# User-tian/Conan

Hardware: AMD Instinct MI355X
Metric: chunks/sec (80 ms chunk, 16 kHz), all streams summed; p50 per-chunk latency beside it (higher is better)
Workload: dtype f32 (3×bf16-limb products, f32 accumulate)

## Files before the change

### conan_amd/csrc/kernels.h

```cpp
#pragma once
#include <hip/hip_runtime.h>
#include <stdint.h>
#include <stdlib.h>

namespace cnk {

inline const char* dev_getenv(const char* name) {
#ifdef CONAN_DEV_SWITCHES
  return getenv(name);
#else
  (void)name;
  return nullptr;
#endif
}
#define HIP_CHECK(x) ::ch::hip_check((x), #x)


struct TRef {
  float* base;
  long long slot_stride;
  int C;
  int lmask;
  int rate;
  int off;
  int mode;
  int pad_;
};

constexpr int kSlotTablePad = 32;

constexpr int kMegaMaxOps = 80;
constexpr int kMegaDbgGroupWords = 512 + 4 * kMegaMaxOps;
constexpr int kMegaDbgWords = kMegaDbgGroupWords + 64;

enum Act { ACT_NONE = 0, ACT_LRELU = 1, ACT_RELU = 2, ACT_GELU = 3, ACT_TANH = 4 };

constexpr unsigned long long kSpinBudgetTicks = 5000000ull;
constexpr unsigned long long kSpinGapTicks = 100000ull;
enum WaitCode { WAIT_MEGA_BARRIER = 1, WAIT_EMF_CLUSTER = 2, WAIT_PAIR_FLAG = 3, WAIT_PAIR_MAILBOX = 4, WAIT_RETIRED_5 = 5 , WAIT_MEGA_ELECT = 6, WAIT_MEGA_DECIDED = 7, WAIT_MEGA_FLAGS = 8 };
struct SpinGuard { unsigned long long last = 0, acc = 0; unsigned it = 0; };
#if defined(__HIPCC__)
__device__ __forceinline__ bool spin_expired(SpinGuard& g, unsigned* guard, unsigned code) {
  if ((++g.it & 255u) != 0u || guard == nullptr) return false;
  if (__hip_atomic_load(guard, __ATOMIC_RELAXED, __HIP_MEMORY_SCOPE_AGENT) != 0u) return true;
  const unsigned long long now = __builtin_amdgcn_s_memrealtime();
  if (g.last != 0) { const unsigned long long d = now - g.last; g.acc += d < kSpinGapTicks ? d : kSpinGapTicks; }
  g.last = now;
  if (g.acc < kSpinBudgetTicks) return false;
  __hip_atomic_store(guard, code, __ATOMIC_RELAXED, __HIP_MEMORY_SCOPE_AGENT);
  unsigned* host = *reinterpret_cast<unsigned* const*>(guard + 2);
  if (host) __hip_atomic_store(host, code, __ATOMIC_RELAXED, __HIP_MEMORY_SCOPE_SYSTEM);
  return true;
}
#endif

struct ConvArgs {
  TRef x;
  TRef y;
  TRef res;
  TRef m1, m2;
  const float* w;
  const float* bias;
  const float* bvec;
  const int* slots;
  const int* pos;
  const int* lens;
  long long bvec_stride;
  int has_res, has_m1, has_m2;
  int Cin, Cin_pad, Cout, Cout_pad;
  int ktaps, dil, pad_left;
  int T;
  int n;
  int in_act;
  float in_slope;
  int out_act;
  float out_scale, out_slope;
  int shuffle_r;
  int Cin_alloc;
  float* y2_base;
  float y2_slope;
  const unsigned short* wl;
#ifdef CK_STAMPS
  unsigned long long* dbg;
#endif
};

struct ConvGroup {
  ConvArgs p[3];
  int tile_start[4];
  int tiles_n[3];
  int order[3];
  float* slab;
  int* counters;
  const int* assign;
  int assign_per;
  int ksplit;
  int split_from;
  int fenced;
};

enum ConvCfg { CFG_128x64 = 0, CFG_64x64 = 1, CFG_128x32 = 2, CFG_32x64_K2 = 3, CFG_32x32_K4 = 4, CFG_64x32_K2 = 5,
               CFG_64x64_KS64 = 6, CFG_128x32_KS64 = 7, NUM_CFG };
int conv_cfg_ks(int cfg);
bool conv_cfg_splitk(int cfg);
const char* conv_cfg_name(int cfg);
int conv_cfg_tm(int cfg);
int conv_cfg_tn(int cfg);
void launch_conv(const ConvGroup& g, int nprob, int cfg, hipStream_t st, int num_cu = 256);

struct ConvTallArgs {
  ConvArgs p;
  int S, nbps;
  int mtiles, ntiles;
  float* slab;
  int* counters;
};
bool conv_tall_supported(const ConvArgs& a);
bool conv_tall_plan(const ConvArgs& a, int num_cu, int plan_n, ConvTallArgs* out, long long slab_floats, int max_counters, int max_T = 32);
void launch_conv_tall(const ConvTallArgs& g, hipStream_t st);

struct ConvLimbGroup {
  ConvArgs p[3];
  int nprob;
  const int* tiles;
  const int* assign;
  int assign_per;
  int wr_max;
  float* slab; int* counters;
  long long slab_floats; int max_counters;
};
bool conv_limb_supported(const ConvArgs& a);
int conv_limb_shape(const ConvArgs* p, int nprob, int num_cu, int plan_n = 0, bool tail_split = false);
bool launch_conv_limb(const ConvLimbGroup& g, int shape, int num_cu, hipStream_t st);
int conv_limb_tail_slices(const ConvArgs& a, int shape, int num_cu);
const char* conv_limb_name(int shape);

struct RBProb {
  const float* w1; const float* w2;
  const float* b1; const float* b2;
  const unsigned short* w1l; const unsigned short* w2l;
  TRef x;
  TRef y;
  int k, dil;
};
struct RBArgs {
  RBProb p[3];
  const int* slots; const int* pos;
  const int* tiles;
  int ntiles;
  int* sched;
  int nprob, n, T;
  int tiles_per_slot;
  int order[3];
  float slope;
  int merge;
  TRef ymean;
  unsigned long long* dbg;
};
bool resblock_fused_supported(int C, int kmax, int span_max);
int resblock_fused_rows(int C, int T, int n, int ksum, int kmax, int num_cu);
bool launch_resblock_fused(const RBArgs& a, int C, int rows, int num_cu, hipStream_t st);
bool resblock_fused_can_merge(int C, int rows);
const char* resblock_fused_name(int C, int rows, bool merge = false);
const int* resblock_tiles(const RBArgs& a, int ro, int* total_out);
bool resblock_limb_supported(int C, int kmax, int span_max);
constexpr int kResblockLimbMaxSlots = 256;
int resblock_limb_rows(int C, int span_max);
bool launch_resblock_limb(const RBArgs& a, int C, int rows, int num_cu, hipStream_t st);
bool resblock_limb_can_merge(int C, int rows);
const char* resblock_limb_name(int C, int rows, bool merge = false);


struct RPProb {
  const float* w1; const float* w2;
  const float* b1; const float* b2;
  TRef x, y;
  TRef xh;
  int k, dil;
};
struct RPArgs {
  RPProb p[3];
  const int* slots; const int* pos;
  const int* tiles; int ntiles;
  int* sched;
  float* xb;
  unsigned* xflag; unsigned* mbox; unsigned* xcount;
  int nprob, n, T;
  float slope;
  unsigned* guard;
  int fault;
};
bool resblock_pair_supported(int C, int kmax, int span_max, int T);
size_t resblock_pair_xb_floats(int num_cu);
bool launch_resblock_pair(const RPArgs& a, int num_cu, hipStream_t st);
const char* resblock_pair_name(int T);

struct RowConvArgs {
  TRef x;
  TRef hist;
  TRef y, res, m1, m2, lnmask, mask_out;
  const float* w;
  const float* bias;
  const float* bvec; long long bvec_stride;
  const float* gamma; const float* beta; float eps;
  const int* slots; const int* pos;
  int ln, has_res, has_m1, has_m2, has_lnmask, has_mask_out;
  int Cin, Cout, Cout_pad, ktaps, dil, T, n;
  int out_act; float out_scale, out_slope;
  int in_lrelu; float in_slope;
  int wr_max;
  int cw;
  const float* w2;
  float* part; long long part_stride;
  int Cout2, Cout2_pad;
  const float* xp; long long xp_stride; int xparts, xp_ld;
  const float* xbias; TRef xres; int has_xres;
  TRef xm1, xm2; int has_xm1, has_xm2, xstore;
  int hid_overlay;
};
bool rowconv_supported(int Cin, int ktaps, int dil, int T);
void launch_rowconv(const RowConvArgs& a, hipStream_t st, int plan_rows = 0);
const char* rowconv_kernel_name(const RowConvArgs& a, int plan_rows = 0);
int rowconv_plan(RowConvArgs& a, int* nbx, int* nby, int* lds_floats, int plan_rows = 0);

struct LNArgs {
  TRef x, pre, y, post, m1, m2, mask_out;
  const float* gamma;
  const float* beta;
  const int* slots;
  const int* pos;
  const int* lens;
  int has_pre, has_post, has_m1, has_m2, has_mask_out;
  int T, n, C;
  float eps;
  const float* xp; long long xp_stride; int xparts, xp_ld;
  const float* xbias; TRef xres; int has_xres;
};
void launch_layernorm(const LNArgs& a, hipStream_t st);

struct CopyArgs {
  TRef x, y;
  const int* slots; const int* pos; const int* lens;
  int T, n, C;
};
void launch_copy_rows(const CopyArgs& a, hipStream_t st);

struct EmbedArgs {
  TRef y;
  const float* table; const int* idx;
  const int* slots; const int* pos;
  int T, n, C, vocab;
};
void launch_embed(const EmbedArgs& a, hipStream_t st);

struct EmfAttnArgs {
  const float* q;
  const float* kv;
  float* out;
  float* kring; float* vring;
  long long ring_slot_stride;
  const int* slots; const int* past;
  int n, R, U, D, H, LC, lmask;
  float scaling;
  int M, seg;
};
void launch_emf_attn(const EmfAttnArgs& a, hipStream_t st);

struct EmfMemArgs {
  float* ln;
  float* bank;
  const float* mems_in;
  const int* slots; const int* past;
  int n, R, U, D, M, MB, seg;
};
void launch_emf_mem_prep(const EmfMemArgs& a, hipStream_t st);
void launch_emf_seg_mean(const float* x, float* out, int n, int rows, int row0, int U, int D, hipStream_t st);
void launch_emf_mem_out(const float* x, float* out, int n, int rows, int row, int D, int tanh_on_mem, hipStream_t st);

constexpr int EMF_MAX_LAYERS = 12;
struct EmfLayerW {
  const float *wqkv, *wo, *w1, *w2;
  const float* params;
};
struct EmfFusedArgs {
  EmfLayerW layers[EMF_MAX_LAYERS];
  float* kring[EMF_MAX_LAYERS]; float* vring[EMF_MAX_LAYERS];
  long long ring_slot_stride;
  const float* chunk;
  float* out;
  float* logits;
  int* codes;
  const float* wp; const float* bp;
  const int* slots; int* past;
  int n, L, R, U, D, H, LC, lmask, F, K;
#ifdef EF_STAMPS
  unsigned long long* dbg;
#endif
  unsigned magic_per_g;
  float scaling;
  int cs;
  float* xch;
  unsigned* xflag;
  unsigned* xepoch;
  int fenced;
  unsigned* guard;
  unsigned fault;
  int M, MB, tanh_on_mem;
  float* bank_k[EMF_MAX_LAYERS]; float* bank_v[EMF_MAX_LAYERS];
  long long bank_slot_stride;
};
constexpr int EMF_MAX_CLUSTER = 8;
constexpr int EMF_MAX_CHUNKS = 16;
inline size_t emformer_cluster_xch_floats(int max_groups, int D) { return (size_t)max_groups * 2 * EMF_MAX_CHUNKS * 16 * D; }
inline size_t emformer_cluster_flag_words(int max_groups) { return (size_t)max_groups * (EMF_MAX_LAYERS * EMF_MAX_CLUSTER + 1); }
int emformer_fused_streams_per_block(const EmfFusedArgs& a);
bool emformer_fused_supported(const EmfFusedArgs& a);
void launch_emformer_fused(const EmfFusedArgs& a, hipStream_t st);

struct XAttnArgs {
  TRef q;
  TRef out;
  const float* kv;
  long long kv_slot_stride;
  const float* kmask;
  const int* slen;
  float* attn_avg;
  const int* slots; const int* pos;
  int T, n, E, H, S_max;
};
void launch_xattn(const XAttnArgs& a, hipStream_t st);

struct PitchHeadArgs {
  TRef h;
  TRef pitch_inp;
  TRef dec_inp;
  const float* gamma; const float* beta; const float* w; const float* b;
  const float* pitch_embed;
  const int* codes;
  float* uv_pred; float* f0; int* bins;
  const int* slots; const int* pos;
  int T, n, Cp, E, silent_token;
};
void launch_pitch_head(const PitchHeadArgs& a, hipStream_t st);

struct MeanActArgs { TRef x[3]; TRef y; const int* slots; const int* pos; int nsrc, T, n, C; float slope; };
void launch_mean_act(const MeanActArgs& a, hipStream_t st);
struct ConvPostArgs { TRef x[3]; TRef xmean; int nsrc; float slope; const float* w; float bias; float* wav; float* pre; const int* slots; const int* pos; int T, n, C, k;
                      int* adv_pos; int adv_delta; int* adv_ticket; };
void launch_conv_post(const ConvPostArgs& a, hipStream_t st);

enum MegaOpType { MOP_RC111 = 0, MOP_RC114 = 1, MOP_ROWLIN = 2, MOP_LN = 3, MOP_XATTN = 4, MOP_PITCH = 5, MOP_EMBED = 6, MOP_COPY32 = 7, MOP_ADVANCE = 8, MOP_FFN = 9 };
struct MegaCopy { unsigned* dst; const unsigned* src; long long n; };
struct MegaAdvance { int* pos; const int* slots; int n, delta; };
struct MegaOp {
  int type, nbx, nby;
  int barrier;
  float f0, f1;
  int pad_[2];
  union U { RowConvArgs rc; LNArgs ln; XAttnArgs xa; PitchHeadArgs ph; EmbedArgs em; MegaCopy cp; MegaAdvance adv; } u;
};
int decoder_mega_lds_floats(const MegaOp& op, int rc_lds_floats);
int decoder_mega_blocks_per_cu(int lds_bytes, bool wide_regs);
struct MegaLaunch {
  const MegaOp* prog; int nops, njobs, groups, group_size, kw4, lds_bytes;
  const int* slots; const int* pos; int n, T;
  unsigned* gbar; unsigned* bar; unsigned bar_base; unsigned long long* dbg;
  unsigned* guard;
  int wide_regs;
  int xcd; unsigned* xs; unsigned xseq, xdec_base;
};
void launch_decoder_mega(const MegaLaunch& m, hipStream_t st);

struct ArgmaxArgs { const float* x; int* idx; int rows, C; };
void launch_argmax(const ArgmaxArgs& a, hipStream_t st);

void launch_advance(int* pos, const int* slots, int n, int delta, hipStream_t st);
void launch_fill_int(int* p, const int* slots, int n, int value, hipStream_t st);
void launch_copy_int_rows(int* dst, const int* src, int n, int T, int S, hipStream_t st);
void launch_profile_mark(hipStream_t st);
void launch_scatter_int(int* dst, const int* slots, const int* src, int n, hipStream_t st);
void launch_scatter_ids(int* dst, const int* slots, const int* src, const int* lens, int n, int S_max, hipStream_t st);
void launch_gather_ids(int* dst, int* cnt, const int* src, const int* slen, const int* slots, int n, int S_max, hipStream_t st);
void launch_scatter_rows(float* dst, const float* src, const int* slots, int n, int C, hipStream_t st);
void launch_zero_slots(float* base, long long slot_stride, long long count, const int* slots, int n, hipStream_t st);
constexpr int kMelStreamFrames = 4;
struct MelStreamArgs {
  const float* wav;
  float* aring;
  float* mring;
  float* chunk;
  const int* slots;
  const float* win; const double2* tw; const float* fb; const int* lo; const int* hi;
  long long r_prev, total;
  int m, n, f0, nnew, pos, rows, real;
  int LA, LM, nm, n_fft, hop, nb, cmag;
  float eps, vmin, vmax, mag_eps;
  int natural_log;
};
inline size_t mel_stream_lds_bytes(int n_fft, int cmag) { return (size_t)n_fft * kMelStreamFrames * 8 + (size_t)n_fft * 16 + (size_t)kMelStreamFrames * cmag * 4; }
void launch_mel_stream(const MelStreamArgs& a, hipStream_t st);
void launch_mel_stream_copy(const MelStreamArgs& a, hipStream_t st);
enum RaggedField {
  kRgSlot, kRgRecvLo, kRgRecvHi, kRgTotalLo, kRgTotalHi,
  kRgM, kRgF0, kRgNnew, kRgPos, kRgRows, kRgReal,
  kRgChunk,
  kRgJob,
  kRgGroup, kRgIndex, kRgEmit,
  kRaggedWords = 16
};
struct MelRaggedArgs {
  const float* wav;
  float* aring; float* mring; float* chunk;
  const int* tab;
  const float* win; const double2* tw; const float* fb; const int* lo; const int* hi;
  int n, jobs, wstride;
  int LA, LM, nm, n_fft, hop, nb, cmag;
  float eps, vmin, vmax, mag_eps;
  int natural_log;
};
void launch_mel_ragged(const MelRaggedArgs& a, hipStream_t st);
struct WavScatterArgs {
  const int* tab; int n, seg, nm, hop;
  const int* codes_src; const float* mel_src; const float* wav_src;
  int* codes; float* mel; float* wav;
};
void launch_wav_scatter(const WavScatterArgs& a, hipStream_t st);

constexpr int kRsTile = 256;
constexpr int kRsRing = 32768;
constexpr int kRsMaxWindow = 16384;
struct RsFilter {
  const float* taps;
  const int* ph;
  int orig, nph, w, L;
};
struct RsRow {
  long long in0, out0;
  const float* taps; const int* ph;
  int slot, m, h, orig, nph, w, L, copy;
};
static_assert(sizeof(RsRow) == 16 * sizeof(int), "RsRow is uploaded as 16 ints");
struct ResampleArgs { const float* x; float* y; long long samples, nout; RsFilter f; int win; };
void launch_resample(const ResampleArgs& a, int n, hipStream_t st);
struct ResampleStreamArgs {
  const float* wav; long long wav_ld;
  float* ring;
  float* out; long long out_ld;
  const RsRow* rows; int n, tiles, win;
};
void launch_resample_stream(const ResampleStreamArgs& a, hipStream_t st);
struct RsOutRow {
  long long in0, out0;
  const float* taps; const int* ph;
  int slot, m, h, orig, nph, w, L, dst;
};
static_assert(sizeof(RsOutRow) == 16 * sizeof(int), "RsOutRow is uploaded as 16 ints");
struct ResampleOutArgs {
  const float* wav; long long wav_ld;
  float* ring; int ring_len;
  float* out; long long out_ld;
  const RsOutRow* rows; int n, tiles, win;
};
void launch_resample_out(const ResampleOutArgs& a, hipStream_t st);

struct RowMaskArgs { TRef x; TRef m; const int* lens; int T, n, C; int mode; };
void launch_rowmask(const RowMaskArgs& a, hipStream_t st);
struct WNGateArgs { TRef xin; TRef acts; const int* lens; int T, n, H; };
void launch_wn_gate(const WNGateArgs& a, hipStream_t st);
struct WNUpdateArgs { TRef rs; TRef x; TRef out; TRef m; const int* lens; int T, n, H; int last; int first; };
void launch_wn_update(const WNUpdateArgs& a, hipStream_t st);
struct PoolArgs { TRef x; TRef m; TRef y; const int* lens; int T, n, C, group; };
void launch_group_pool(const PoolArgs& a, hipStream_t st);
struct VQArgs {
  TRef x; TRef dots; TRef cat;
  const float* emb; const float* e2; const float* postable;
  int* ids;
  const int* lens; int S, n, E, M, S_max;
};
void launch_vq(const VQArgs& a, hipStream_t st);
struct KMaskArgs { TRef tok; float* kmask; long long kmask_stride; const int* slots; const int* lens; int S, n, S_max; };
void launch_kmask(const KMaskArgs& a, hipStream_t st);
struct MeanArgs { TRef x; TRef m; float* out; long long out_stride; const int* slots; const int* lens; int T, n, C; };
void launch_masked_mean(const MeanArgs& a, hipStream_t st);
struct ScaleMaskArgs { TRef x; TRef m; const int* lens; int T, n, C; };
void launch_mul_mask(const ScaleMaskArgs& a, hipStream_t st);

}
```

### conan_amd/csrc/resblock_limb.hip

```cpp
#include <algorithm>
#include <cstring>
#include <type_traits>

#include "kernels.h"

#define RL_MAX_SLOTS 256

#ifndef RL_HELPER_PRIO
#define RL_HELPER_PRIO 3
#endif
#ifndef RL_MATRIX_PRIO
#define RL_MATRIX_PRIO 0
#endif
#ifndef RL_STAMPS
#define RL_STAMPS 0
#endif

#ifdef RL_ABLATE_W
#define RL_WOFF(x) 0
#define RL_WOFF2(a_, b_) (b_)
#else
#define RL_WOFF(x) (x)
#define RL_WOFF2(a_, b_) (a_)
#endif

namespace cnk {

namespace {

typedef float f32x4 __attribute__((ext_vector_type(4)));
typedef __bf16 bf16x8 __attribute__((ext_vector_type(8)));
typedef unsigned short u16;
typedef const f32x4 __attribute__((address_space(1)))* gcf4;
typedef f32x4 __attribute__((address_space(1)))* gf4;
typedef const float __attribute__((address_space(1)))* gcf1;
typedef const int __attribute__((address_space(1)))* gci;

__device__ __forceinline__ f32x4 rl_gload(const void* p) { return *(gcf4)(p); }
__device__ __forceinline__ float4 rl_gload4(const float* p) { const f32x4 v = *(gcf4)(p); return make_float4(v[0], v[1], v[2], v[3]); }
__device__ __forceinline__ void rl_gstore4(float* p, const float4 v) { *(gf4)(p) = (f32x4){v.x, v.y, v.z, v.w}; }

typedef float f32x2 __attribute__((ext_vector_type(2)));
typedef __bf16 bf16x2 __attribute__((ext_vector_type(2)));
__device__ __forceinline__ void rl_split2(const f32x2 x, unsigned& h, unsigned& m, unsigned& l) {
  h = __builtin_bit_cast(unsigned, __builtin_convertvector(x, bf16x2));
  const f32x2 hf = {__uint_as_float(h << 16), __uint_as_float(h & 0xffff0000u)};
  const f32x2 r1 = x - hf;
  m = __builtin_bit_cast(unsigned, __builtin_convertvector(r1, bf16x2));
  const f32x2 mf = {__uint_as_float(m << 16), __uint_as_float(m & 0xffff0000u)};
  const f32x2 r2 = r1 - mf;
  l = __builtin_bit_cast(unsigned, __builtin_convertvector(r2, bf16x2));
}
__device__ __forceinline__ f32x2 rl_lrelu2(const f32x2 x, const float slope) {
  const f32x2 sx = x * slope;
  return (f32x2){__builtin_fmaxf(x[0], sx[0]), __builtin_fmaxf(x[1], sx[1])};
}

template <int C_, int NR2_, int SPAN_>
struct RLGeom {
  static constexpr int C = C_, NR2 = NR2_;
  static constexpr int NR1 = NR2 + 1;
  static constexpr int RO = 16 * NR2;
  static constexpr int XT_ROWS = 16 * NR1;
  static constexpr int MAXSPAN = SPAN_;
  static constexpr int WR_MAX = XT_ROWS + MAXSPAN;
  static constexpr int LDB = C + 16;
  static constexpr int PLW = WR_MAX * LDB;
  static constexpr int PLX = XT_ROWS * LDB;
  static constexpr int LDA = C + 4;
  static constexpr int LDS_U16 = 3 * (PLW + PLX);
  static constexpr int NCT = C / 16;
  static constexpr int NCW = C == 64 ? 1 : 2;
  static constexpr int RSPLIT = 4 / (NCT / NCW);
  static constexpr int NRW1 = (NR1 + RSPLIT - 1) / RSPLIT;
  static constexpr int NRW2 = (NR2 + RSPLIT - 1) / RSPLIT;
  static constexpr int KB = C / 32;
  static constexpr int RING = 2;
  static constexpr int C4 = C / 4;
  static constexpr int BLK = 3 * 512;
  static_assert(C % 32 == 0 && NCT % NCW == 0 && 4 % (NCT / NCW) == 0 && (KB == 1 || KB % RING == 0), "channel count");
  static_assert(RO * LDA * 4 <= 3 * PLX * 2, "accumulator image inside the xt planes");
  static_assert(LDS_U16 * 2 + 32 + 8 * RL_MAX_SLOTS <= 160 * 1024, "LDS budget");
};

template <int NCW, int RING>
__device__ __forceinline__ void rl_prefetch_w(f32x4 (&bw)[RING][NCW][3], const u16* __restrict__ wl, const long long ct_stride) {
#pragma unroll
  for (int q = 0; q < RING; ++q) {
#pragma unroll
    for (int c = 0; c < NCW; ++c)
#pragma unroll
      for (int p = 0; p < 3; ++p) bw[q][c][p] = rl_gload(wl + c * ct_stride + q * 1536 + p * 512);
    __builtin_amdgcn_sched_barrier(0);
  }
}

template <int NRW, int NCW, int LDB, int KB, int RING>
__device__ __forceinline__ void rl_gemm(const u16* __restrict__ src, const int plane, const int row0, const int tap_stride, const int k,
                                        const u16* __restrict__ wl, const long long ct_stride, const u16* __restrict__ wl_next,
                                        const long long ct_stride_next, f32x4 (&acc)[NRW][NCW], f32x4 (&bw)[RING][NCW][3], const int lane) {
  const u16* abase = src + (row0 + (lane & 15)) * LDB + 8 * (lane >> 4);
  f32x4 af[NRW][3];
#pragma unroll
  for (int r = 0; r < NRW; ++r)
#pragma unroll
    for (int p = 0; p < 3; ++p) af[r][p] = *reinterpret_cast<const f32x4*>(abase + p * plane + r * 16 * LDB);
  const int tstep = tap_stride * LDB;
  if constexpr (KB == 1) {
    static_assert(RING == 2, "ring");
    constexpr int PA[6] = {2, 1, 0, 1, 0, 0}, PB[6] = {0, 1, 2, 0, 1, 0};
    auto block = [&](const int j, auto slot_c) __attribute__((always_inline)) {
      constexpr int SL = decltype(slot_c)::value;
      const u16* anext = abase + (j + 1) * tstep;
#pragma unroll
      for (int s = 0; s < 6; ++s)
#pragma unroll
        for (int r = 0; r < NRW; ++r) {
#pragma unroll
          for (int c = 0; c < NCW; ++c)
            acc[r][c] = __builtin_amdgcn_mfma_f32_16x16x32_bf16(__builtin_bit_cast(bf16x8, bw[SL][c][PB[s]]), __builtin_bit_cast(bf16x8, af[r][PA[s]]), acc[r][c], 0, 0, 0);
#ifndef RL_ABLATE_A
          if (s == 0) af[r][2] = *reinterpret_cast<const f32x4*>(anext + 2 * plane + r * 16 * LDB);
          if (s == 3) af[r][1] = *reinterpret_cast<const f32x4*>(anext + plane + r * 16 * LDB);
          if (s == 5) af[r][0] = *reinterpret_cast<const f32x4*>(anext + r * 16 * LDB);
#endif
        }
      const bool own = j + 2 < k;
      const u16* wsrc = own ? wl + (long long)(j + 2) * 1536 : wl_next + (long long)(j + 2 - k) * 1536;
      const long long cs = own ? ct_stride : ct_stride_next;
#pragma unroll
      for (int c = 0; c < NCW; ++c)
#pragma unroll
        for (int p = 0; p < 3; ++p) bw[SL][c][p] = rl_gload(wsrc + c * cs + p * 512);
#pragma unroll
      for (int s = 0; s < 6; ++s) {
        if (s == 0 || s == 3 || s == 5) {
#pragma unroll
          for (int r = 0; r < NRW; ++r) {
            __builtin_amdgcn_sched_group_barrier(0x008, NCW, 0);
            __builtin_amdgcn_sched_group_barrier(0x100, 1, 0);
          }
        } else {
          __builtin_amdgcn_sched_group_barrier(0x008, NRW * NCW, 0);
        }
      }
      __builtin_amdgcn_sched_group_barrier(0x020, 3 * NCW, 0);
    };
    int j = 0;
    for (; j + 1 < k; j += 2) {
      block(j, std::integral_constant<int, 0>{});
      block(j + 1, std::integral_constant<int, 1>{});
    }
    if (j < k) {
      block(j, std::integral_constant<int, 0>{});
#pragma unroll
      for (int c = 0; c < NCW; ++c)
#pragma unroll
        for (int p = 0; p < 3; ++p) { const f32x4 t = bw[0][c][p]; bw[0][c][p] = bw[1][c][p]; bw[1][c][p] = t; }
    }
    return;
  }
  for (int j = 0; j < k; ++j) {
    const u16* arow = abase + j * tstep;
    const bool last = j + 1 == k;
    const u16* wnext = last ? wl_next : wl + (long long)(j + 1) * KB * 1536;
    const long long cnext = last ? ct_stride_next : ct_stride;
#pragma unroll
    for (int q = 0; q < KB; ++q) {
      const u16* anext = (q + 1 < KB) ? arow + (q + 1) * 32 : arow + tstep;
      constexpr int PA[6] = {2, 1, 0, 1, 0, 0}, PB[6] = {0, 1, 2, 0, 1, 0};
#pragma unroll
      for (int s = 0; s < 6; ++s)
#pragma unroll
        for (int r = 0; r < NRW; ++r) {
#pragma unroll
          for (int c = 0; c < NCW; ++c)
            acc[r][c] = __builtin_amdgcn_mfma_f32_16x16x32_bf16(__builtin_bit_cast(bf16x8, bw[q % RING][c][PB[s]]), __builtin_bit_cast(bf16x8, af[r][PA[s]]),
                                                                acc[r][c], 0, 0, 0);
#ifndef RL_ABLATE_A
          if (s == 0) af[r][2] = *reinterpret_cast<const f32x4*>(anext + 2 * plane + r * 16 * LDB);
          if (s == 3) af[r][1] = *reinterpret_cast<const f32x4*>(anext + plane + r * 16 * LDB);
          if (s == 5) af[r][0] = *reinterpret_cast<const f32x4*>(anext + r * 16 * LDB);
#endif
        }
      if (q + RING < KB) {
#pragma unroll
        for (int c = 0; c < NCW; ++c)
#pragma unroll
          for (int p = 0; p < 3; ++p) bw[q % RING][c][p] = rl_gload(wl + RL_WOFF(((long long)j * KB + q + RING) * 1536) + c * ct_stride + p * 512);
      } else {
#pragma unroll
        for (int c = 0; c < NCW; ++c)
#pragma unroll
          for (int p = 0; p < 3; ++p) bw[q % RING][c][p] = rl_gload(RL_WOFF2(wnext, wl) + (q + RING - KB) * 1536 + c * cnext + p * 512);
      }
#pragma unroll
      for (int s = 0; s < 6; ++s) {
        if (s == 0 || s == 3 || s == 5) {
#pragma unroll
          for (int r = 0; r < NRW; ++r) {
            __builtin_amdgcn_sched_group_barrier(0x008, NCW, 0);
            __builtin_amdgcn_sched_group_barrier(0x100, 1, 0);
          }
        } else {
          __builtin_amdgcn_sched_group_barrier(0x008, NRW * NCW, 0);
        }
      }
      __builtin_amdgcn_sched_group_barrier(0x020, 3 * NCW, 0);
      __builtin_amdgcn_sched_barrier(0);
    }
  }
}

}

#define RL_SEL(br_, f) ((br_) == 0 ? a.p[0].f : ((br_) == 1 ? a.p[1].f : a.p[2].f))

template <int C, int NR2, int SPAN, bool MERGE>
__global__ __launch_bounds__(512, 2) void resblock_limb_kernel(const RBArgs a) {
  using G = RLGeom<C, NR2, SPAN>;
  constexpr int LDB = G::LDB;
  __shared__ __attribute__((aligned(16))) u16 lds[G::LDS_U16 + 16 + 4 * RL_MAX_SLOTS];
  u16* const win = lds;
  u16* const xt = lds + 3 * G::PLW;
  float* const accimg = reinterpret_cast<float*>(xt);
  int* const meta = reinterpret_cast<int*>(lds + G::LDS_U16);
  int* const sptab = meta + 8;
  const int tid = threadIdx.x;
  const int lane = tid & 63;
  const int wave = __builtin_amdgcn_readfirstlane(tid >> 6);
  const int ntiles = a.ntiles;
  const float slope = a.slope;
  const int T = a.T;
  constexpr bool merge = MERGE;
  const int np = a.nprob;

  if (wave >= 4) {
    const int ht = tid - 256;
    __builtin_amdgcn_s_setprio(RL_HELPER_PRIO);
    auto hbar = [&]() __attribute__((always_inline)) { asm volatile("s_waitcnt lgkmcnt(0)\n\ts_barrier" ::: "memory"); };
    constexpr int NIT = (G::WR_MAX * G::C4 + 255) / 256;
    float4 wv[NIT];
    int wtotal = 0, wzr = 0;
    auto win_issue = [&](const int p, const int i, const int t0, const int slot, const int pos) __attribute__((always_inline)) {
      const int k = RL_SEL(p, k), d = RL_SEL(p, dil);
      const int wr = G::XT_ROWS + (k - 1) * d;
      const int tw0 = t0 - (k - 1) - (k - 1) * d;
      const int xmode = a.p[0].x.mode, xrate = a.p[0].x.rate;
      const float* xb = RL_SEL(p, x.base) + (long long)(xmode == 0 ? slot : i) * RL_SEL(p, x.slot_stride);
      const unsigned rbase = (xmode == 0 ? (unsigned)pos * (unsigned)xrate : 0u) + (unsigned)(RL_SEL(p, x.off) + tw0);
      const unsigned rmask = xmode == 0 ? (unsigned)RL_SEL(p, x.lmask) : 0xffffffffu;
      wtotal = wr * G::C4;
#pragma unroll
      for (int u = 0; u < NIT; ++u) {
        const int idx = ht + 256 * u;
        const int w = idx / G::C4, c4 = idx - w * G::C4;
        const unsigned row = (rbase + (unsigned)w) & rmask;
        wv[u] = idx < wtotal ? rl_gload4(xb + (long long)row * C + c4 * 4) : make_float4(0.f, 0.f, 0.f, 0.f);
      }
      const long long abs0 = (xmode == 0 ? (long long)pos * xrate : 0ll) + t0 - (k - 1);
      wzr = abs0 >= 0 ? 0 : (abs0 < -(long long)G::XT_ROWS ? G::XT_ROWS : (int)-abs0);
    };
    auto win_write = [&]() __attribute__((always_inline)) {
#pragma unroll
      for (int u = 0; u < NIT; ++u) {
        const int idx = ht + 256 * u;
        const int w = idx / G::C4, c4 = idx - w * G::C4;
        unsigned h[2], m[2], l[2];
        rl_split2(rl_lrelu2((f32x2){wv[u].x, wv[u].y}, slope), h[0], m[0], l[0]);
        rl_split2(rl_lrelu2((f32x2){wv[u].z, wv[u].w}, slope), h[1], m[1], l[1]);
        if (idx < wtotal) {
          u16* dst = win + w * LDB + c4 * 4;
          *reinterpret_cast<uint2*>(dst) = make_uint2(h[0], h[1]);
          *reinterpret_cast<uint2*>(dst + G::PLW) = make_uint2(m[0], m[1]);
          *reinterpret_cast<uint2*>(dst + 2 * G::PLW) = make_uint2(l[0], l[1]);
        }
      }
      if (ht == 0) meta[0] = wzr;
    };
    constexpr int NOUT = (G::RO * G::C4) / 256;
    static_assert((G::RO * G::C4) % 256 == 0 && 256 % G::C4 == 0, "output tile / helper threads");
    const int oc4 = ht % G::C4;
    float4 oacc[NOUT], ores[NOUT], osum[MERGE ? NOUT : 1], ob2 = make_float4(0.f, 0.f, 0.f, 0.f);
    const float* oxb = nullptr; const float* ob2p = nullptr;
    float* oyb = nullptr;
    unsigned oyr0 = 0, oym = 0, oxr0 = 0, oxm = 0;
    int ot0 = 0, op = 0, oyC = C;
#pragma unroll
    for (int u = 0; u < (MERGE ? NOUT : 1); ++u) osum[u] = make_float4(0.f, 0.f, 0.f, 0.f);
    auto out_fetch = [&](const int p, const int i, const int t0, const int slot, const int pos) __attribute__((always_inline)) {
      const int xmode = a.p[0].x.mode, xrate = a.p[0].x.rate, ymode = a.p[0].y.mode, yrate = a.p[0].y.rate;
      oxb = RL_SEL(p, x.base) + (long long)(xmode == 0 ? slot : i) * RL_SEL(p, x.slot_stride);
      oxr0 = (xmode == 0 ? (unsigned)pos * (unsigned)xrate : 0u) + (unsigned)(RL_SEL(p, x.off) + t0);
      oxm = xmode == 0 ? (unsigned)RL_SEL(p, x.lmask) : 0xffffffffu;
      if (!merge) {
        oyb = RL_SEL(p, y.base) + (long long)(ymode == 0 ? slot : i) * RL_SEL(p, y.slot_stride);
        oyr0 = (ymode == 0 ? (unsigned)pos * (unsigned)yrate : 0u) + (unsigned)(RL_SEL(p, y.off) + t0);
        oym = ymode == 0 ? (unsigned)RL_SEL(p, y.lmask) : 0xffffffffu;
      } else {
        const int mmode = a.ymean.mode;
        oyb = a.ymean.base + (long long)(mmode == 0 ? slot : i) * a.ymean.slot_stride;
        oyr0 = (mmode == 0 ? (unsigned)pos * (unsigned)a.ymean.rate : 0u) + (unsigned)(a.ymean.off + t0);
        oym = mmode == 0 ? (unsigned)a.ymean.lmask : 0xffffffffu;
        oyC = a.ymean.C;
      }
      ot0 = t0; op = p;
      ob2p = RL_SEL(p, b2) + oc4 * 4;
#pragma unroll
      for (int u = 0; u < NOUT; ++u) oacc[u] = *reinterpret_cast<const float4*>(accimg + ((ht + 256 * u) / G::C4) * G::LDA + oc4 * 4);
      ob2 = rl_gload4(ob2p);
#pragma unroll
      for (int u = 0; u < NOUT; ++u) {
        const int r = (ht + 256 * u) / G::C4;
        ores[u] = ot0 + r < T ? rl_gload4(oxb + (long long)((oxr0 + (unsigned)r) & oxm) * C + oc4 * 4) : make_float4(0.f, 0.f, 0.f, 0.f);
      }
    };
    auto out_store = [&]() __attribute__((always_inline)) {
#pragma unroll
      for (int u = 0; u < NOUT; ++u) {
        const int r = (ht + 256 * u) / G::C4;
        if (ot0 + r < T) {
          const float4 v = make_float4((oacc[u].x + ob2.x) + ores[u].x, (oacc[u].y + ob2.y) + ores[u].y, (oacc[u].z + ob2.z) + ores[u].z, (oacc[u].w + ob2.w) + ores[u].w);
          if constexpr (!MERGE) rl_gstore4(oyb + (long long)((oyr0 + (unsigned)r) & oym) * C + oc4 * 4, v);
          else {
            float4 sm = osum[MERGE ? u : 0];
            if (op == 0) sm = v; else { sm.x += v.x; sm.y += v.y; sm.z += v.z; sm.w += v.w; }
            osum[MERGE ? u : 0] = sm;
            if (op == np - 1) {
              const float dn = (float)np;
              if (np > 1) { sm.x /= dn; sm.y /= dn; sm.z /= dn; sm.w /= dn; }
              sm.x = sm.x > 0.f ? sm.x : sm.x * slope; sm.y = sm.y > 0.f ? sm.y : sm.y * slope;
              sm.z = sm.z > 0.f ? sm.z : sm.z * slope; sm.w = sm.w > 0.f ? sm.w : sm.w * slope;
              rl_gstore4(oyb + (long long)((oyr0 + (unsigned)r) & oym) * oyC + oc4 * 4, sm);
            }
          }
        }
      }
    };
#if RL_STAMPS
    const unsigned long long h_t0 = __builtin_amdgcn_s_memtime();
    unsigned long long h_t[6] = {0, 0, 0, 0, 0, 0};
#define RL_HT(i_) h_t[i_] = __builtin_amdgcn_s_memtime() - h_t0
#else
#define RL_HT(i_)
#endif
    int dv0 = 0;
    if (wave == 4 && lane == 0) dv0 = __hip_atomic_fetch_add(a.sched, 1, __ATOMIC_RELAXED, __HIP_MEMORY_SCOPE_AGENT);
    for (int e = ht; e < a.n; e += 256) {
      const int sl = a.slots ? *(gci)(a.slots + e) : e;
      sptab[2 * e] = sl; sptab[2 * e + 1] = a.pos ? *(gci)(a.pos + sl) : 0;
    }
    const int tps = a.tiles_per_slot, per_prob = a.n * tps;
    auto decode = [&](const int e, int& p, int& i, int& t0) __attribute__((always_inline)) {
      if constexpr (!MERGE) {
        const int b = e / per_prob, rem = e - b * per_prob;
        p = b == 0 ? a.order[0] : (b == 1 ? a.order[1] : a.order[2]);
        i = rem / tps; t0 = (rem - i * tps) * G::RO;
      } else {
        const int g = e / np;
        p = e - g * np; i = g / tps; t0 = (g - i * tps) * G::RO;
      }
    };
    int cur = -1, p = -1, i = 0, t0 = 0;
    if (wave == 4) {
      cur = __builtin_amdgcn_readfirstlane(dv0) * (merge ? np : 1);
      if (cur >= ntiles) cur = -1;
      if (cur >= 0) decode(cur, p, i, t0);
      if (lane == 0) { meta[1] = cur; meta[2] = p; meta[3] = 0; }
    }
    RL_HT(0);
    asm volatile("s_waitcnt lgkmcnt(0)\n\ts_barrier" ::: "memory");
    RL_HT(1);
    if (wave != 4) {
      cur = __builtin_amdgcn_readfirstlane(meta[1]);
      if (cur >= 0) decode(cur, p, i, t0);
    }
    if (cur >= 0) {
    int slot = __builtin_amdgcn_readfirstlane(sptab[2 * i]), pos = __builtin_amdgcn_readfirstlane(sptab[2 * i + 1]);
    win_issue(p, i, t0, slot, pos);
    RL_HT(2);
    int gen = 1;
    int dv = 0, dnext = -1;
    auto draw_issue = [&](const int have, const int idx_prev, const int p_prev) __attribute__((always_inline)) {
      if (wave == 4 && lane == 0 && have) {
        if (merge && p_prev != np - 1) dnext = idx_prev + 1;
        else { dnext = -1; dv = __hip_atomic_fetch_add(a.sched, 1, __ATOMIC_RELAXED, __HIP_MEMORY_SCOPE_AGENT); }
      }
    };
    auto draw_take = [&](const int have) __attribute__((always_inline)) {
      int idx = -1;
      if (!have) return idx;
      if (wave == 4) {
        const int drawn = dv * (merge ? np : 1);
        idx = __builtin_amdgcn_readfirstlane(dnext >= 0 ? dnext : drawn);
        if (idx >= ntiles) idx = -1;
        if (lane == 0) {
          meta[1] = idx;
          asm volatile("s_waitcnt lgkmcnt(0)" ::: "memory");
          __hip_atomic_store(&meta[3], gen, __ATOMIC_RELEASE, __HIP_MEMORY_SCOPE_WORKGROUP);
        }
      } else {
        while (__hip_atomic_load(&meta[3], __ATOMIC_ACQUIRE, __HIP_MEMORY_SCOPE_WORKGROUP) != gen) __builtin_amdgcn_s_sleep(4);
        idx = __builtin_amdgcn_readfirstlane(meta[1]);
      }
      ++gen;
      return idx;
    };
    const bool deep = ntiles >= 5 * (int)gridDim.x * (merge ? np : 1);
    auto stage = [&](const int e) __attribute__((always_inline)) {
      int pe, ie, te;
      decode(e, pe, ie, te);
      win_issue(pe, ie, te, __builtin_amdgcn_readfirstlane(sptab[2 * ie]), __builtin_amdgcn_readfirstlane(sptab[2 * ie + 1]));
      return pe;
    };
    int nxt = -1, pn = -1;
    if (deep) {
      draw_issue(1, cur, p);
      nxt = draw_take(1);
    }
    RL_HT(3);
    win_write();
    RL_HT(4);
    hbar();
    RL_HT(5);
#if RL_STAMPS
    if (a.dbg && blockIdx.x == 0 && wave == 4 && lane == 0) { unsigned long long* q = a.dbg + 256 * 4 + 12; for (int e = 0; e < 6; ++e) q[e] = h_t[e]; }
#endif
    bool pending = false;
    for (;;) {
      const bool have = deep ? nxt >= 0 : true;
      if (deep && nxt >= 0) pn = stage(nxt);
      draw_issue(have, deep ? nxt : cur, deep ? pn : p);
      if (pending) out_store();
      int nn = -1;
      if (!deep) {
        nxt = draw_take(have); pn = -1;
        if (nxt >= 0) pn = stage(nxt);
      }
      if (ht == 0) meta[2] = nxt >= 0 ? pn : -1;
      hbar();
      hbar();
      if (nxt >= 0) win_write();
      hbar();
      hbar();
      out_fetch(p, i, t0, slot, pos);
      pending = true;
      if (deep) nn = draw_take(have);
      if (nxt < 0) break;
      cur = nxt;
      decode(cur, p, i, t0);
      slot = __builtin_amdgcn_readfirstlane(sptab[2 * i]); pos = __builtin_amdgcn_readfirstlane(sptab[2 * i + 1]);
      nxt = nn;
    }
    if (pending) out_store();
    }
    if (ht == 0) {
      const int d = __hip_atomic_fetch_add(a.sched + 1, 1, __ATOMIC_RELAXED, __HIP_MEMORY_SCOPE_AGENT);
      if (d == (int)gridDim.x - 1) {
        __hip_atomic_store(a.sched, 0, __ATOMIC_RELAXED, __HIP_MEMORY_SCOPE_AGENT);
        __hip_atomic_store(a.sched + 1, 0, __ATOMIC_RELAXED, __HIP_MEMORY_SCOPE_AGENT);
      }
    }
    return;
  }

  if (RL_MATRIX_PRIO) __builtin_amdgcn_s_setprio(RL_MATRIX_PRIO);
  auto bar = [&]() __attribute__((always_inline)) { asm volatile("s_waitcnt lgkmcnt(0)\n\ts_barrier" ::: "memory"); };
  const int wc = wave % (4 / G::RSPLIT);
  const int wr = wave / (4 / G::RSPLIT);
  const int ct0 = wc * G::NCW;
  const int lr = lane & 15, lg = lane >> 4;
#if RL_STAMPS
  unsigned long long st_gemm = 0, st_t0 = __builtin_amdgcn_s_memtime(), st_r0 = __builtin_amdgcn_s_memrealtime(), st_bar = 0, st_b3 = 0, st_b1 = 0, st_b4 = 0, st_b2 = 0, st_e1 = 0, st_e2 = 0, st_tiles = 0, st_head = 0, st_pre = 0, st_mid = 0;
#define RL_T() __builtin_amdgcn_s_memtime()
#define RL_BAR(acc_) do { const unsigned long long q0_ = RL_T(); bar(); const unsigned long long q1_ = RL_T(); acc_ += q1_ - q0_; st_bar += q1_ - q0_; } while (0)
#define RL_GEMM(...) do { const unsigned long long s0_ = RL_T(); __VA_ARGS__; asm volatile("s_nop 0" ::"v"(acc[0][0][0])); st_gemm += RL_T() - s0_; } while (0)
#else
#define RL_BAR(acc_) bar()
#define RL_GEMM(...) __VA_ARGS__
#endif
  f32x4 bw[G::RING][G::NCW][3];
  bar();
  int p = __builtin_amdgcn_readfirstlane(meta[2]);
  if (p < 0) return;
  {
    const long long cs = (long long)(RL_SEL(p, k) + 1) * G::KB * G::BLK;
    rl_prefetch_w<G::NCW, G::RING>(bw, RL_SEL(p, w1l) + (long long)ct0 * cs + lane * 8, cs);
  }
  bar();
#if RL_STAMPS
  st_head = RL_T() - st_t0;
#endif
  while (p >= 0) {
#if RL_STAMPS
    const unsigned long long top_ = RL_T();
#endif
    const int k = RL_SEL(p, k), d = RL_SEL(p, dil);
    const u16* const w1 = RL_SEL(p, w1l);
    const u16* const w2 = RL_SEL(p, w2l);
    const float* const b1 = RL_SEL(p, b1);
    const long long ct_stride = (long long)(k + 1) * G::KB * G::BLK;
    const int zrows = __builtin_amdgcn_readfirstlane(meta[0]);
    f32x4 b1v[G::NCW];
#pragma unroll
    for (int c = 0; c < G::NCW; ++c) b1v[c] = rl_gload(b1 + (ct0 + c) * 16 + 4 * lg);
    int pn;
    {
      f32x4 acc[G::NRW1][G::NCW];
#pragma unroll
      for (int r = 0; r < G::NRW1; ++r)
#pragma unroll
        for (int c = 0; c < G::NCW; ++c) acc[r][c] = (f32x4){0.f, 0.f, 0.f, 0.f};
      const int rt0 = wr * G::NRW1;
#if RL_STAMPS
      st_pre += RL_T() - top_;
#endif
      RL_GEMM(rl_gemm<G::NRW1, G::NCW, LDB, G::KB, G::RING>(win, G::PLW, rt0 * 16, d, k, w1 + (long long)ct0 * ct_stride + lane * 8, ct_stride,
                                                           w2 + (long long)ct0 * ct_stride + lane * 8, ct_stride, acc, bw, lane));
      RL_BAR(st_b3);
#if RL_STAMPS
      const unsigned long long e1_0 = RL_T();
#endif
      auto epilogue1 = [&](auto zr_c) __attribute__((always_inline)) {
        constexpr bool ZR = decltype(zr_c)::value;
#pragma unroll
        for (int c = 0; c < G::NCW; ++c) {
          const int col = (ct0 + c) * 16 + 4 * lg;
#pragma unroll
          for (int r = 0; r < G::NRW1; ++r) {
            if (rt0 + r < G::NR1) {
              const int m = (rt0 + r) * 16 + lr;
              unsigned h[2], mm[2], l[2];
              const f32x4 v = acc[r][c] + b1v[c];
              rl_split2(rl_lrelu2((f32x2){v[0], v[1]}, slope), h[0], mm[0], l[0]);
              rl_split2(rl_lrelu2((f32x2){v[2], v[3]}, slope), h[1], mm[1], l[1]);
              const bool zr = ZR && m < zrows;
              u16* dst = xt + m * LDB + col;
              *reinterpret_cast<uint2*>(dst) = zr ? make_uint2(0u, 0u) : make_uint2(h[0], h[1]);
              *reinterpret_cast<uint2*>(dst + G::PLX) = zr ? make_uint2(0u, 0u) : make_uint2(mm[0], mm[1]);
              *reinterpret_cast<uint2*>(dst + 2 * G::PLX) = zr ? make_uint2(0u, 0u) : make_uint2(l[0], l[1]);
            }
          }
        }
      };
      if (zrows > 0) epilogue1(std::true_type{}); else epilogue1(std::false_type{});
#if RL_STAMPS
      asm volatile("s_waitcnt lgkmcnt(0)" ::: "memory"); st_e1 += RL_T() - e1_0; ++st_tiles;
#endif
    }
    RL_BAR(st_b1);
#if RL_STAMPS
    const unsigned long long mid_ = RL_T();
#endif
    pn = __builtin_amdgcn_readfirstlane(meta[2]);
    const int pnx = pn >= 0 ? pn : p;
    const long long csn = (long long)(RL_SEL(pnx, k) + 1) * G::KB * G::BLK;
    const u16* const w1n = RL_SEL(pnx, w1l) + (long long)ct0 * csn + lane * 8;
    {
      f32x4 acc[G::NRW2][G::NCW];
#pragma unroll
      for (int r = 0; r < G::NRW2; ++r)
#pragma unroll
        for (int c = 0; c < G::NCW; ++c) acc[r][c] = (f32x4){0.f, 0.f, 0.f, 0.f};
      const int rt0 = wr * G::NRW2;
#if RL_STAMPS
      st_mid += RL_T() - mid_;
#endif
      RL_GEMM(rl_gemm<G::NRW2, G::NCW, LDB, G::KB, G::RING>(xt, G::PLX, rt0 * 16, 1, k, w2 + (long long)ct0 * ct_stride + lane * 8, ct_stride,
                                                           w1n, csn, acc, bw, lane));
      RL_BAR(st_b4);
#if RL_STAMPS
      const unsigned long long e2_0 = RL_T();
#endif
#pragma unroll
      for (int c = 0; c < G::NCW; ++c) {
        const int col = (ct0 + c) * 16 + 4 * lg;
#pragma unroll
        for (int r = 0; r < G::NRW2; ++r) {
          if (rt0 + r < NR2) *reinterpret_cast<f32x4*>(accimg + ((rt0 + r) * 16 + lr) * G::LDA + col) = acc[r][c];
        }
      }
#if RL_STAMPS
      asm volatile("s_waitcnt lgkmcnt(0)" ::: "memory"); st_e2 += RL_T() - e2_0;
#endif
    }
    RL_BAR(st_b2);
    p = pn;
  }
#if RL_STAMPS
  if (a.dbg && tid == 0) {
    unsigned long long* o = a.dbg + blockIdx.x * 4;
    if (blockIdx.x == 0) { unsigned long long* q = a.dbg + 256 * 4; q[0] = st_b3; q[1] = st_b1; q[2] = st_b4; q[3] = st_b2; q[4] = st_e1; q[5] = st_e2; q[6] = st_tiles; q[7] = st_gemm; q[8] = __builtin_amdgcn_s_memtime() - st_t0; q[9] = st_head; q[10] = st_pre; q[11] = st_mid; }
    o[0] = st_gemm; o[1] = __builtin_amdgcn_s_memtime() - st_t0; o[2] = __builtin_amdgcn_s_memrealtime() - st_r0; o[3] = st_bar;
  }
#endif
}


namespace {
struct RLCand { int C, NR2, span; };
const RLCand kLimbCands[] = {{32, 10, 50}, {64, 5, 50}, {128, 2, 50}};
}

bool resblock_limb_supported(int C, int kmax, int span_max) {
  for (const RLCand& c : kLimbCands)
    if (c.C == C && span_max <= c.span) return kmax <= 16;
  return false;
}

int resblock_limb_rows(int C, int span_max) {
  int best = 0;
  for (const RLCand& c : kLimbCands)
    if (c.C == C && span_max <= c.span) best = std::max(best, 16 * c.NR2);
  return best;
}

template <int C, int NR2, int SPAN, bool MERGE = false>
static bool launch_rl(const RBArgs& ain, int num_cu, hipStream_t st) {
  RBArgs a = ain;
  const int ro = 16 * NR2;
  a.tiles_per_slot = (a.T + ro - 1) / ro;
  const int total = a.nprob * a.n * a.tiles_per_slot;
  if (total <= 0) return true;
  if (!a.sched) return false;
  for (int p = 0; p < a.nprob; ++p) if (!a.p[p].w1l || !a.p[p].w2l) return false;
  if (a.n > RL_MAX_SLOTS) return false;
  if (!(a.slope > 0.f && a.slope <= 1.f)) return false;
  for (int p = 0; p < 3; ++p) a.order[p] = p;
  std::stable_sort(a.order, a.order + a.nprob, [&](int x, int y) { return a.p[x].k > a.p[y].k; });
  const int grid = std::min(a.merge ? total / a.nprob : total, num_cu);
  a.tiles = nullptr; a.ntiles = total;
  hipLaunchKernelGGL((resblock_limb_kernel<C, NR2, SPAN, MERGE>), dim3(grid), dim3(512), 0, st, a);
  return true;
}

bool launch_resblock_limb(const RBArgs& a, int C, int rows, int num_cu, hipStream_t st) {
  const int nr2 = rows / 16;
  if (a.merge) {
    if (C == 32 && nr2 == 10) return launch_rl<32, 10, 50, true>(a, num_cu, st);
    if (C == 64 && nr2 == 5) return launch_rl<64, 5, 50, true>(a, num_cu, st);
    if (C == 128 && nr2 == 2) return launch_rl<128, 2, 50, true>(a, num_cu, st);
    return false;
  }
  if (C == 32 && nr2 == 10) return launch_rl<32, 10, 50>(a, num_cu, st);
  if (C == 64 && nr2 == 5) return launch_rl<64, 5, 50>(a, num_cu, st);
  if (C == 128 && nr2 == 2) return launch_rl<128, 2, 50>(a, num_cu, st);
  return false;
}

bool resblock_limb_can_merge(int C, int rows) { return (C == 32 && rows == 160) || (C == 64 && rows == 80) || (C == 128 && rows == 32); }

const char* resblock_limb_name(int C, int rows, bool merge) {
  static thread_local char buf[72];
  const int span = 50;
  snprintf(buf, sizeof(buf), "cnk::resblock_limb_kernel<%d, %d, %d, %s>", C, rows / 16, span, merge ? "true" : "false");
  return buf;
}

}
```

### conan_amd/csrc/streams.h

```cpp
#pragma once
#include "host_common.h"

using ch::Error;
using ch::Lin;
using ch::PackedConv;
using ch::Ring;
using cnk::ConvArgs;
using cnk::ConvGroup;
using cnk::TRef;

constexpr int kMaxBranches = 3;
constexpr int PADR = 16;

struct VocStage {
  Ring up;
  Ring upa;
  Ring xs;
  std::vector<std::vector<Ring>> xt, xo;
  std::vector<std::vector<Ring>> xa;
  int C = 0, rate = 1;
  bool fused = false;
  bool pair = false;
  std::vector<std::vector<Ring>> xh;
};

struct PinRing {
  static constexpr int N = 8;
  int* buf = nullptr;
  size_t cap = 0;
  hipEvent_t ev[N] = {};
  int next = 0, cur = 0;
  void init(size_t ints) {
    cap = ints;
    HIP_CHECK(hipHostMalloc((void**)&buf, cap * N * sizeof(int), hipHostMallocDefault));
    for (int i = 0; i < N; ++i) HIP_CHECK(hipEventCreateWithFlags(&ev[i], hipEventDisableTiming));
  }
  void upload(int* dst, const int* src, size_t n, hipStream_t st) {
    if (n > cap) throw ch::Error(CONAN_ERR_INVALID, "host table larger than the staging buffer");
    cur = next; next = (next + 1) % N;
    HIP_CHECK(hipEventSynchronize(ev[cur]));
    memcpy(buf + (size_t)cur * cap, src, n * sizeof(int));
    HIP_CHECK(hipMemcpyAsync(dst, buf + (size_t)cur * cap, n * sizeof(int), hipMemcpyHostToDevice, st));
    HIP_CHECK(hipEventRecord(ev[cur], st));
  }
  ~PinRing() {
    for (int i = 0; i < N; ++i) if (ev[i]) (void)hipEventDestroy(ev[i]);
    if (buf) (void)hipHostFree(buf);
  }
};

struct conan_streams {
  conan_ctx* ctx = nullptr;
  std::atomic<int>* live = nullptr;
  std::map<std::string, std::string> dev_plan;
  void parse_dev_plan(const char* text);
  const char* dev(const char* name) const {
    if (!dev_plan.empty()) {
      auto it = dev_plan.find(name);
      if (it != dev_plan.end()) return it->second.c_str();
    }
#ifdef CONAN_DEV_SWITCHES
    return getenv((std::string("CONAN_") + name).c_str());
#else
    return nullptr;
#endif
  }
  bool fixed_plan = false;
  bool in_style_pass = false;
  int plan_n(int n) const { return (fixed_plan && !in_style_pass) ? max_slots : n; }
  bool pipe_idle = false;
  bool shared_device = false;
  int max_slots = 0, max_frames = 0, max_ref = 0, S_max = 0;
  std::vector<void*> allocs;
  int64_t state_bytes = 0;
  std::vector<std::pair<float*, long long>> voc_state, dec_state, emf_state;

  int* d_slots = nullptr;
  int* d_ident = nullptr;
  int* d_zero = nullptr;
  int* d_lens = nullptr;
  int* d_lens2 = nullptr;
  int* d_codes = nullptr;
  float* sk_slab[3] = {nullptr, nullptr, nullptr};
  int* sk_counters[3] = {nullptr, nullptr, nullptr};
  int reserve_cus = 0;
  bool fenced = false;
  bool rb_limb = false;
  bool arith_auto = true;
  bool rb_merge = true;
  int* cp_ticket[3] = {nullptr, nullptr, nullptr};
  int* rb_sched[2] = {nullptr, nullptr};
  float* rp_xb[2] = {nullptr, nullptr};
  unsigned* rp_words[2] = {nullptr, nullptr};
  long long sk_slab_floats = 0;
  int sk_max_tiles = 0;
  std::vector<int> h_slots;
  std::vector<int> slot_seen;
  int slot_gen = 0;
  PinRing pin;
  int* pos_emf = nullptr; int* pos_dec = nullptr; int* pos_voc = nullptr;
  unsigned* d_guard = nullptr;
  unsigned* h_guard = nullptr;
  int test_fault = 0;
  void check_fault() const {
    if (!h_guard) return;
    const unsigned code = *(volatile const unsigned*)h_guard;
    if (code == 0) return;
    static const char* what[] = {"?", "decoder_mega_kernel group / grid barrier", "emformer_fused_kernel cluster exchange", "resblock_pair_kernel partner flag", "resblock_pair_kernel tile mailbox",
                                 "(retired)", "decoder_mega_kernel xcd election", "decoder_mega_kernel xcd roll call", "decoder_mega_kernel xcd flag barrier"};
    throw ch::Error(CONAN_ERR_HIP, std::string("a cross-workgroup wait gave up after its 50 ms budget (") + what[code < 9 ? code : 0] +
                                       "): results since then are invalid and this stream-set is unusable - destroy it and create a new one");
  }

  float* fe_audio = nullptr; float* fe_mel = nullptr; float* fe_chunk = nullptr;
  int fe_LA = 0, fe_LM = 0, fe_last_n = 0;
  struct FeSlot { long long recv = 0; int frames = 0, chunks = 0, phase = 0; };
  std::vector<FeSlot> fe_slot;
  static constexpr int NS = 4;
  PinRing fe_pin;
  int* rg_tab[NS] = {}; int* rg_codes[NS] = {}; float* rg_mel[NS] = {}; float* rg_wav[NS] = {};
  hipEvent_t ev_stage[NS] = {};
  long long rg_calls = 0;
  bool fe_last_ragged = false;
  void ragged_init();
  struct RsSlot { const ch::RsTable* f = nullptr; long long in = 0, out = 0; int phase = 0; };
  std::vector<RsSlot> rs_slot;
  float* rs_ring = nullptr;
  PinRing rs_pin;
  cnk::RsRow* rs_rows[NS] = {}; float* rs_wav[NS] = {};
  hipEvent_t ev_rs[NS] = {};
  long long rs_calls = 0;
  void resample_init();
  struct OrSlot { const ch::RsTable* f = nullptr; long long out = 0; int flushed = 0; };
  std::vector<OrSlot> or_slot;
  std::vector<long long> voc_samples;
  float* or_ring = nullptr; int or_ring_len = 0;
  PinRing or_pin;
  cnk::RsOutRow* or_rows[NS] = {}; float* or_wav[NS] = {};
  hipEvent_t ev_or[NS] = {};
  long long or_calls = 0, out_ld = 0;
  std::vector<int32_t> out_counts;
  void out_stage_init();
  struct OutPlan {
    bool active = false;
    std::vector<cnk::RsOutRow> rows;
    std::vector<int32_t> counts;
    std::vector<int> dst;
    float* base = nullptr; long long ld = 0;
    int tiles = 1, win = 0;
    double flops = 0;
  };
  OutPlan out_plan(const int32_t* slots, int n, int frames, float* wav_out, long long natural_ld, const std::vector<int>* dst, const std::string& who) const;
  Ring v_mel, v_pre;
  std::vector<VocStage> v_st;
  std::vector<Ring> e_k, e_v;
  std::vector<float*> e_bank;
  int e_bank_rows = 0;
  float* e_mems[2] = {nullptr, nullptr};
  Lin e_x[2], e_ln, e_q, e_kv, e_att, e_r1, e_ffn, e_h, e_r2, e_logits;
  bool emf_fused = false;
  int emf_cluster = 0;
  cnk::EmfFusedArgs emf_fused_args;
  Ring c_emb, c_pin2, c_lastr;
  std::vector<Ring> c_uvh;
  std::vector<Ring> c_lnrs;
  Lin c_pin, c_q, c_att, c_a1, c_a2, c_ff, c_uv5, c_x[2], c_h, c_post, c_mask_blk, c_mask_blk2, c_mask_out, c_mel, c_part, c_part2;
  float* c_style = nullptr;
  float* c_kv = nullptr;
  float* c_kmask = nullptr;
  int* c_slen = nullptr;
  int* c_vqids = nullptr;
  std::vector<char> has_ref;
  std::vector<char> voc_fresh;
  int sp_batch = 0;
  Lin s_mel, s_np, s_wnm, s_x[2], s_ln, s_h, s_blkm, s_wx, s_wout, s_win, s_acts, s_rs, s_ph, s_pm, s_px[2], s_pln, s_phh,
      s_pblk, s_enc, s_dots, s_cat, s_tok, s_kvtmp;
  int* s_ids = nullptr;

  float* alloc(size_t floats) {
    void* p = nullptr;
    if (floats == 0) floats = 4;
    HIP_CHECK(hipMalloc(&p, floats * sizeof(float)));
    HIP_CHECK(hipMemset(p, 0, floats * sizeof(float)));
    allocs.push_back(p);
    state_bytes += (int64_t)floats * 4;
    return (float*)p;
  }
  Ring mk_ring(int C, int rate, int hist, std::vector<std::pair<float*, long long>>* reg) {
    Ring r; r.C = C; r.rate = rate;
    r.L = ch::next_pow2(hist + max_frames * rate);
    r.slot_stride = (long long)r.L * C;
    r.base = alloc((size_t)max_slots * r.slot_stride);
    if (reg) reg->push_back({r.base, r.slot_stride});
    return r;
  }
  Lin mk_lin(int rows, int C, int nb = -1) {
    Lin l; l.rows = rows; l.C = C;
    l.base = alloc((size_t)(nb < 0 ? max_slots : nb) * rows * C);
    return l;
  }
  hipStream_t st_emf = nullptr, st_front = nullptr, st_voc = nullptr;
  hipEvent_t ev_wide[4] = {};
  hipEvent_t mark_wide = nullptr;
  bool wide_marked[4] = {false, false, false, false};
  static constexpr int NP = 4;
  hipEvent_t ev_in[NP] = {}, ev_emf[NP] = {}, ev_front[NP] = {}, ev_voc[NP] = {};
  hipEvent_t ev_fence[NP] = {};
  hipStream_t fence_stream = nullptr; bool fence_set = false;
  hipEvent_t fence_event = nullptr;
  int* codes_hand[NP] = {};
  int ws_index(hipStream_t st) const { return (st_voc && st == st_voc) ? 1 : ((st_emf && st == st_emf) ? 2 : 0); }
  float* mel_hand[NP] = {};
  long long async_steps = 0;
  std::vector<hipEvent_t> clock_ev;
  bool clock_on = false; int clock_n = 0;
  std::vector<hipEvent_t> tl_ev;
  bool tl_on = false; int tl_n = 0;
  void async_init();
  void join(hipStream_t st);

  void mega_print_stamps();
  ~conan_streams() {
    if (live) live->fetch_sub(1);
    if (mega_dbg) mega_print_stamps();
    if (st_emf) (void)hipStreamDestroy(st_emf);
    if (st_front) (void)hipStreamDestroy(st_front);
    if (st_voc) (void)hipStreamDestroy(st_voc);
    for (int i = 0; i < NP; ++i) { if (ev_in[i]) (void)hipEventDestroy(ev_in[i]); if (ev_fence[i]) (void)hipEventDestroy(ev_fence[i]); }
    for (int i = 0; i < NP; ++i) { if (ev_wide[i]) (void)hipEventDestroy(ev_wide[i]); if (ev_emf[i]) (void)hipEventDestroy(ev_emf[i]); if (ev_front[i]) (void)hipEventDestroy(ev_front[i]); if (ev_voc[i]) (void)hipEventDestroy(ev_voc[i]); }
    for (int i = 0; i < NS; ++i) if (ev_stage[i]) (void)hipEventDestroy(ev_stage[i]);
    for (int i = 0; i < NS; ++i) if (ev_rs[i]) (void)hipEventDestroy(ev_rs[i]);
    for (int i = 0; i < NS; ++i) if (ev_or[i]) (void)hipEventDestroy(ev_or[i]);
    for (void* p : allocs) (void)hipFree(p);
    if (h_guard) (void)hipHostFree(h_guard);
    for (auto& e : prof_ev) { (void)hipEventDestroy(e.first); (void)hipEventDestroy(e.second); }
    for (auto& e : clock_ev) (void)hipEventDestroy(e);
    for (auto& m : mega_cache) { if (m.copied) (void)hipEventDestroy(m.copied); if (m.pinned) (void)hipHostFree(m.pinned); if (m.dev) (void)hipFree(m.dev); }
    for (auto& e : tl_ev) (void)hipEventDestroy(e);
  }

  void build_vocoder();
  void build_emformer();
  void build_decoder();
  void set_slots(const int32_t* slots, int n, hipStream_t st);
  int pick_cfg(int M, int N, int nprob) const;
  bool prof_on = false;
  std::vector<std::pair<hipEvent_t, hipEvent_t>> prof_ev;
  size_t prof_used = 0;
  double prof_flops = 0.0;
  long long prof_launches = 0;
  struct ProfRec { std::string name; double flops; };
  std::vector<ProfRec> prof_rec;
  struct ProfKernel { std::string name; double ms, flops; long long n; };
  std::vector<ProfKernel> prof_kernels;
  void launch_group(const ConvGroup& g, int nprob, int cfg, hipStream_t st);
  bool launch_rb(const cnk::RBArgs& a, int C, hipStream_t st, const TRef* ymean = nullptr);
  void launch_rp(const cnk::RPArgs& a, hipStream_t st);
  bool use_rowconv = true;
  bool rowconv_ok(const PackedConv& pc, int dil, int T) const { return use_rowconv && pc.wf && cnk::rowconv_supported(pc.Cin, pc.k, dil, T); }
  cnk::RowConvArgs mk_rc(const PackedConv& pc, const TRef& x, const TRef& y, int n, int T, int dil = 1) const;
  void rowconv(const cnk::RowConvArgs& a, hipStream_t st);
  template <typename F> void profiled(const std::string& name, double flops, hipStream_t st, F&& launch);
  void conv(const ConvArgs& a, hipStream_t st) { ConvGroup g; g.p[0] = a; launch_group(g, 1, pick_cfg(plan_n(a.n) * a.T, a.Cout, 1), st); }
  ConvArgs mk(const PackedConv& pc, const TRef& x, const TRef& y, int n, int T, const int* pos, int dil = 1, int pad_left = -1) const;

  struct DecExtra { float* mel_out2 = nullptr; int* codes_dst = nullptr; const int* codes_src = nullptr; int codes_words = 0; };
  struct MegaProgram {
    long long key[6] = {0, 0, 0, 0, 0, 0};
    bool ok = false;
    int nops = 0, groups = 0, group_size = 0, njobs = 0, kw4 = 0, lds_bytes = 0, barriers = 0, n = 0, T = 0;
    int lds_need = 0;
    bool xcd = false;
    double flops = 0.0;
    cnk::MegaOp* dev = nullptr;
    cnk::MegaOp* pinned = nullptr;
    hipEvent_t copied = nullptr;
    long long stamp = 0;
  };
  static constexpr int kMegaMaxOps = cnk::kMegaMaxOps, kMegaEntries = 12;
  std::vector<MegaProgram> mega_cache;
  long long mega_clock = 0;
  bool use_mega = true;
  int mega_grid = 128;
  int mega_gs = 8;
  bool mega_narrow_ksplit = true;
  int mega_ffn_gs = 8;
  unsigned* mega_bar = nullptr;
  unsigned mega_bar_count = 0;
  unsigned* mega_x = nullptr;
  unsigned mega_gseq = 0;
  unsigned mega_xseq = 0, mega_xdec = 0;
  int opt_flags = 0;
  bool mega_single = true;
  unsigned long long* mega_dbg = nullptr;
  int mega_dbg_prog = -1;
  std::vector<cnk::MegaOp>* mega_rec = nullptr;
  bool mega_rec_ok = true; int mega_rec_lds = 0; double mega_rec_flops = 0.0;
  void mega_push(cnk::MegaOp& op, int lds_floats);
  bool run_mega(int n, int T, const int32_t* codes, float* mel_out, const DecExtra& ex, hipStream_t st);
  void launch_mega(MegaProgram& e, hipStream_t st);
  void decoder_ops(int n, int frames, const int32_t* codes, float* mel_out, const conan_decoder_taps& taps, hipStream_t st);
  void op_embed(const cnk::EmbedArgs& a, hipStream_t st);
  void op_ln(const cnk::LNArgs& a, hipStream_t st);
  void op_xattn(const cnk::XAttnArgs& a, hipStream_t st);
  void op_pitch(const cnk::PitchHeadArgs& a, hipStream_t st);
  void op_advance(int* pos, int n, int delta, hipStream_t st);

  void hifigan_step(int n, int frames, const float* mel_dev, float* wav_out, float* pre_tanh, hipStream_t st, const conan_hifigan_taps* taps = nullptr,
                    const OutPlan* op = nullptr);
  void emformer_step(int n, const float* chunk, float* out, float* logits, int32_t* codes, hipStream_t st);
  void decoder_step(int n, int frames, const int32_t* codes, float* mel_out, const conan_decoder_taps& taps, hipStream_t st, const DecExtra* extra = nullptr);
  void set_reference(const int32_t* slots, int n, const float* ref, const int32_t* ref_len, int max_len, hipStream_t st);
  void conv_blocks_noncausal(const std::string& name, int nblocks, int k, int C, Lin* x, Lin& ln, Lin& h, Lin& blkm, const TRef& npm,
                             const int* lens, int n, int T, int& cur, hipStream_t st);
};

template <typename F>
inline void conan_streams::profiled(const std::string& name, double flops, hipStream_t st, F&& launch) {
  if (!prof_on) { launch(); return; }
  if (prof_used == prof_ev.size()) {
    hipEvent_t a, b;
    HIP_CHECK(hipEventCreate(&a)); HIP_CHECK(hipEventCreate(&b));
    prof_ev.push_back({a, b});
  }
  auto& ev = prof_ev[prof_used++];
  HIP_CHECK(hipEventRecord(ev.first, st));
  launch();
  HIP_CHECK(hipEventRecord(ev.second, st));
  prof_flops += flops;
  prof_launches += 1;
  prof_rec.push_back({name, flops});
}
```

### conan_amd/csrc/streams.hip

```cpp
#include <climits>

#include "streams.h"


ConvArgs conan_streams::mk(const PackedConv& pc, const TRef& x, const TRef& y, int n, int T, const int* pos, int dil,
                           int pad_left) const {
  ConvArgs a;
  memset(&a, 0, sizeof(a));
  a.x = x;
  a.y = y; a.res = ch::null_ref(); a.m1 = ch::null_ref(); a.m2 = ch::null_ref();
  a.w = pc.w; a.bias = pc.bias; a.bvec = nullptr; a.slots = d_slots; a.pos = pos; a.lens = nullptr;
  a.Cin = pc.Cin; a.Cin_pad = pc.Cin_pad; a.Cin_alloc = pc.Cin_alloc; a.Cout = pc.Cout; a.Cout_pad = pc.Cout_pad;
  a.ktaps = pc.k; a.dil = dil; a.pad_left = pad_left < 0 ? (pc.k - 1) * dil : pad_left;
  a.T = T; a.n = n; a.in_act = cnk::ACT_NONE; a.in_slope = 0.f; a.out_act = cnk::ACT_NONE; a.out_scale = 1.f; a.out_slope = 0.f;
  a.shuffle_r = pc.shuffle_r;
  a.wl = reinterpret_cast<const unsigned short*>(pc.wl);
  if (x.C != pc.Cin && !(x.C > pc.Cin)) throw Error(CONAN_ERR_SHAPE, "conv input width mismatch");
  return a;
}

int conan_streams::pick_cfg(int M, int N, int nprob) const {
  const int wide[] = {cnk::CFG_64x64, cnk::CFG_32x64_K2, cnk::CFG_32x32_K4};
  const int narrow[] = {cnk::CFG_128x32, cnk::CFG_64x32_K2, cnk::CFG_32x32_K4};
  const int* order = N <= 32 ? narrow : wide;
  const int cnt = 3;
  long long need = ctx->num_cu;
  int best = order[cnt - 1];
  for (int k = 0; k < cnt; ++k) {
    int c = order[k];
    long long blocks = (long long)((M + cnk::conv_cfg_tm(c) - 1) / cnk::conv_cfg_tm(c)) * ((N + cnk::conv_cfg_tn(c) - 1) / cnk::conv_cfg_tn(c)) * nprob;
    if (blocks >= need) {
      best = c;
      if (c == cnk::CFG_64x64 && blocks < 2 * need && nprob > 1) best = cnk::CFG_64x64_KS64;
      break;
    }
  }
  return best;
}

void conan_streams::launch_group(const ConvGroup& gin, int nprob, int cfg, hipStream_t st) {
  if (mega_rec) { mega_rec_ok = false; return; }
  for (int p = 0; p < nprob; ++p) {
    const ConvArgs& a = gin.p[p];
    if ((long long)(a.x.mode == 0 ? max_slots : a.n) * a.x.slot_stride * 4 >= (1ll << 32))
      throw Error(CONAN_ERR_UNSUPPORTED, "activation tensor of 4 GiB or more: lower max_slots");
    if (a.y2_base && ((a.Cout & 3) || (a.y.C & 3) || ((a.Cout / a.shuffle_r) & 3))) throw Error(CONAN_ERR_UNSUPPORTED, "activated twin output needs channel counts that are multiples of 4");
  }
  if (rb_limb && nprob == 1 && dev("NO_TALL") == nullptr) {
    const int cus = std::max(8, ctx->num_cu - (ws_index(st) == 1 ? reserve_cus : 0));
    const int wsi = ws_index(st);
    cnk::ConvTallArgs ta;
    if (cnk::conv_tall_plan(gin.p[0], cus, fixed_plan ? plan_n(gin.p[0].n) : 0, &ta, sk_slab_floats, sk_max_tiles, dev("TALL_MAXT") ? atoi(dev("TALL_MAXT")) : 32)) {
      ta.slab = sk_slab[wsi]; ta.counters = sk_counters[wsi];
      const ConvArgs& a = gin.p[0];
      profiled("cnk::conv_tall_kernel", 2.0 * (double)a.n * a.T * a.Cout * a.ktaps * a.Cin, st, [&] { cnk::launch_conv_tall(ta, st); });
      return;
    }
  }
  if (rb_limb && nprob >= 1 && nprob <= 3) {
    bool ok = true;
    for (int p = 0; p < nprob; ++p) ok = ok && cnk::conv_limb_supported(gin.p[p]) && gin.p[p].n == gin.p[0].n && gin.p[p].T == gin.p[0].T && gin.p[p].Cout == gin.p[0].Cout;
    const int cus = std::max(8, ctx->num_cu - (ws_index(st) == 1 ? reserve_cus : 0));
    const int shape = ok ? cnk::conv_limb_shape(gin.p, nprob, cus, fixed_plan ? plan_n(gin.p[0].n) : 0, !fixed_plan) : -1;
    if (shape >= 0) {
      cnk::ConvLimbGroup lg; memset(&lg, 0, sizeof(lg));
      for (int p = 0; p < nprob; ++p) lg.p[p] = gin.p[p];
      lg.nprob = nprob;
      if (!fixed_plan && nprob == 1) {
        const int wsi = ws_index(st);
        lg.slab = sk_slab[wsi]; lg.counters = sk_counters[wsi]; lg.slab_floats = sk_slab_floats; lg.max_counters = sk_max_tiles;
      }
      double fl = 0.0;
      for (int p = 0; p < nprob; ++p) fl += 2.0 * (double)lg.p[p].n * lg.p[p].T * lg.p[p].Cout * lg.p[p].ktaps * lg.p[p].Cin;
      const bool tail = lg.slab && shape == 0 && cnk::conv_limb_tail_slices(lg.p[0], shape, cus) >= 2;
      profiled(tail ? "cnk::conv_limb_sk_kernel<4, 1, 1, 4>" : cnk::conv_limb_name(shape), fl, st, [&] {
        if (!cnk::launch_conv_limb(lg, shape, cus, st)) throw Error(CONAN_ERR_HIP, "conv_limb launch failed");
      });
      return;
    }
  }
  ConvGroup g = gin;
  for (int p = 0; p < nprob; ++p) {
    ConvArgs& a = g.p[p];
    bool ring = a.y.mode == 0 || (a.has_res && a.res.mode == 0) || (a.has_m1 && a.m1.mode == 0) || (a.has_m2 && a.m2.mode == 0) || a.bvec != nullptr;
    ring = ring || a.x.mode == 0;
    if (!ring) { a.slots = nullptr; a.pos = nullptr; }
  }
  const int wsi = ws_index(st);
  g.slab = sk_slab[wsi]; g.counters = sk_counters[wsi]; g.ksplit = 1; g.split_from = 0; g.fenced = fenced ? 1 : 0;
  const int cus_all = std::max(8, ctx->num_cu - (wsi == 1 ? reserve_cus : 0));
  if (cnk::conv_cfg_tm(cfg) != 32 && nprob == 1 && cnk::conv_cfg_splitk(cfg)) {
    static const bool off = ch::dev_getenv("CONAN_NO_TAILSPLIT") != nullptr;
    const ConvArgs& a = g.p[0];
    const int TM = cnk::conv_cfg_tm(cfg), TN = cnk::conv_cfg_tn(cfg), KS = cnk::conv_cfg_ks(cfg);
    const long long tiles = (long long)((a.n * a.T + TM - 1) / TM) * ((a.Cout + TN - 1) / TN);
    const int nks = a.ktaps * ((a.Cin_pad + KS - 1) / KS);
    const long long rem = tiles % cus_all;
    if (!off && !fixed_plan && tiles > cus_all && rem > 0 && tiles <= sk_max_tiles) {
      int S = (int)std::min<long long>(8, cus_all / rem);
      S = std::min(S, nks / 8);
      while (S > 1 && rem * S * TM * TN > sk_slab_floats) --S;
      if (S >= 2) { g.ksplit = S; g.split_from = (int)(tiles - rem); }
    }
  }
  if (cnk::conv_cfg_tm(cfg) == 32) {
    const int TM = cnk::conv_cfg_tm(cfg), TN = cnk::conv_cfg_tn(cfg);
    const int KS = cnk::conv_cfg_ks(cfg);
    long long tiles = 0;
    int nks = 0;
    for (int p = 0; p < nprob; ++p) {
      const ConvArgs& a = g.p[p];
      tiles += (long long)((plan_n(a.n) * a.T + TM - 1) / TM) * ((a.Cout + TN - 1) / TN);
      nks = std::max(nks, a.ktaps * ((a.Cin_pad + KS - 1) / KS));
    }
    int S = tiles > 0 ? (int)(ctx->num_cu / tiles) : 1;
    if (S > nks / 2) S = nks / 2;
    if (S > 16) S = 16;
    while (S > 1 && tiles * S * TM * TN > sk_slab_floats) --S;
    static const int min_saved = ch::dev_getenv("CONAN_SK_MIN") ? atoi(ch::dev_getenv("CONAN_SK_MIN")) : 12;
    if (S >= 2 && tiles <= sk_max_tiles && (nks - nks / S) * (KS / 32) >= min_saved) g.ksplit = S;
  }
  double fl = 0.0;
  for (int p = 0; p < nprob; ++p) fl += 2.0 * (double)g.p[p].n * g.p[p].T * g.p[p].Cout * g.p[p].ktaps * g.p[p].Cin;
  profiled(cnk::conv_cfg_name(cfg), fl, st, [&] { cnk::launch_conv(g, nprob, cfg, st, cus_all); });
}

cnk::RowConvArgs conan_streams::mk_rc(const PackedConv& pc, const TRef& x, const TRef& y, int n, int T, int dil) const {
  cnk::RowConvArgs a; memset(&a, 0, sizeof(a));
  a.x = x; a.hist = ch::null_ref(); a.y = y; a.res = ch::null_ref(); a.m1 = ch::null_ref(); a.m2 = ch::null_ref();
  a.lnmask = ch::null_ref(); a.mask_out = ch::null_ref();
  a.w = pc.wf; a.bias = pc.bias; a.slots = d_slots; a.pos = pos_dec;
  a.Cin = pc.Cin; a.Cout = pc.Cout; a.Cout_pad = pc.wf_cout_pad; a.ktaps = pc.k; a.dil = dil; a.T = T; a.n = n;
  a.out_act = cnk::ACT_NONE; a.out_scale = 1.f; a.out_slope = 0.f; a.eps = 1e-5f;
  return a;
}

void conan_streams::rowconv(const cnk::RowConvArgs& a, hipStream_t st) {
  const double fl = 2.0 * (double)a.n * a.T * a.Cout * a.ktaps * a.Cin;
  if (mega_rec) {
    cnk::MegaOp op; memset(&op, 0, sizeof(op));
    op.u.rc = a;
    int ldsf = 0;
    const int prows = fixed_plan ? plan_n(a.n) * a.T : 0;
    const int v = cnk::rowconv_plan(op.u.rc, &op.nbx, &op.nby, &ldsf, prows);
    op.type = v == 3 ? cnk::MOP_ROWLIN : (v == 2 ? cnk::MOP_RC114 : cnk::MOP_RC111);
    const int strips64 = (op.u.rc.Cout_pad + 63) / 64;
    if (v == 0 && !a.w2 && plan_n(a.n) * a.T > 16 && mega_narrow_ksplit && (strips64 * 4 <= mega_gs || (strips64 * 2 <= mega_gs && a.ktaps >= 3)) && (a.ktaps * (a.Cin >> 4)) % 4 == 0) {
      const int ldsk = (32 + op.u.rc.wr_max * (a.Cin + 8) + 3 * 64 * 4);
      cnk::MegaOp t = op; t.type = cnk::MOP_RC114;
      if (cnk::decoder_mega_lds_floats(t, ldsk) * 4 <= (96 + 32 * 264) * 4) {
        op.type = cnk::MOP_RC114; op.nbx = (op.u.rc.Cout_pad + 15) / 16; ldsf = ldsk;
      }
    }
    if (a.w2) {
      if ((v != 0 && v != 2) || (a.ktaps * (a.Cin >> 4)) % 8 != 0) { mega_rec_ok = false; return; }
      op.type = cnk::MOP_FFN;
      const int hc = a.Cout / mega_ffn_gs;
      op.u.rc.hid_overlay = hc == 64 ? 1 : 0;
      ldsf = op.u.rc.hid_overlay ? std::max(op.u.rc.wr_max * (a.Cin + 8), 16 * (hc + 8)) : op.u.rc.wr_max * (a.Cin + 8) + 16 * (hc + 8);
      mega_rec_flops += 2.0 * (double)a.n * a.T * a.Cout * a.Cout2;
    }
    mega_rec_flops += fl;
    mega_push(op, cnk::decoder_mega_lds_floats(op, ldsf));
    return;
  }
  const int prows = fixed_plan ? plan_n(a.n) * a.T : 0;
  profiled(cnk::rowconv_kernel_name(a, prows), fl, st, [&] { cnk::launch_rowconv(a, st, prows); });
}

bool conan_streams::launch_rb(const cnk::RBArgs& ain, int C, hipStream_t st, const TRef* ymean) {
  cnk::RBArgs a = ain;
  a.sched = rb_sched[ws_index(st) == 1 ? 1 : 0];
  int ksum = 0, kmax = 0;
  double fl = 0.0;
  for (int p = 0; p < a.nprob; ++p) { ksum += a.p[p].k; kmax = std::max(kmax, a.p[p].k); fl += 2.0 * 2.0 * (double)a.n * a.T * C * C * a.p[p].k; }
  const int cus = std::max(8, ctx->num_cu - (ws_index(st) == 1 ? reserve_cus : 0));
  int span = 0;
  bool limb = rb_limb;
  for (int p = 0; p < a.nprob; ++p) { span = std::max(span, (a.p[p].k - 1) * a.p[p].dil); limb = limb && a.p[p].w1l && a.p[p].w2l; }
  limb = limb && plan_n(a.n) <= cnk::kResblockLimbMaxSlots && cnk::resblock_limb_supported(C, kmax, span);
  const int rows = limb ? cnk::resblock_limb_rows(C, span) : cnk::resblock_fused_rows(C, a.T, plan_n(a.n), ksum, kmax, cus);
  const long long groups = (long long)plan_n(a.n) * ((a.T + rows - 1) / rows);
  const long long rounds = (groups + cus - 1) / cus;
  const bool balanced = groups * 10 >= rounds * cus * 9;
  a.merge = (ymean && rb_merge && a.nprob > 1 && groups >= cus && balanced && (limb ? cnk::resblock_limb_can_merge(C, rows) : cnk::resblock_fused_can_merge(C, rows))) ? 1 : 0;
  if (a.merge) a.ymean = *ymean;
  profiled(limb ? cnk::resblock_limb_name(C, rows, a.merge != 0) : cnk::resblock_fused_name(C, rows, a.merge != 0), fl, st, [&] {
    if (!(limb ? cnk::launch_resblock_limb(a, C, rows, cus, st) : cnk::launch_resblock_fused(a, C, rows, cus, st))) throw Error(CONAN_ERR_HIP, "fused resblock launch failed");
  });
  return a.merge != 0;
}

void conan_streams::launch_rp(const cnk::RPArgs& ain, hipStream_t st) {
  cnk::RPArgs a = ain;
  const int w = ws_index(st) == 1 ? 1 : 0;
  const int pairs = ctx->num_cu / 2;
  a.xb = rp_xb[w]; a.xflag = rp_words[w]; a.mbox = rp_words[w] + (size_t)pairs * 8; a.xcount = rp_words[w] + (size_t)pairs * 12;
  a.sched = reinterpret_cast<int*>(rp_words[w] + (size_t)pairs * 14);
  a.guard = d_guard; a.fault = test_fault == 3 ? 1 : 0;
  if (test_fault == 3) test_fault = 0;
  double fl = 0.0;
  for (int p = 0; p < a.nprob; ++p) fl += 2.0 * 2.0 * (double)a.n * a.T * 256.0 * 256.0 * a.p[p].k;
  profiled(cnk::resblock_pair_name(a.T), fl, st, [&] {
    if (!cnk::launch_resblock_pair(a, ctx->num_cu, st)) throw Error(CONAN_ERR_HIP, "resblock pair launch failed");
  });
}

void conan_streams::mega_print_stamps() {
  if (!mega_dbg || mega_dbg_prog < 0 || mega_dbg_prog >= (int)mega_cache.size()) return;
  (void)hipDeviceSynchronize();
  const MegaProgram& e = mega_cache[mega_dbg_prog];
  std::vector<unsigned long long> h(cnk::kMegaDbgWords);
  if (hipMemcpy(h.data(), mega_dbg, h.size() * 8, hipMemcpyDeviceToHost) != hipSuccess) return;
  static const char* names[] = {"rowconv<1,1,1>", "rowconv<1,1,4>", "rowlin", "layernorm", "xattn", "pitch_head", "embed", "copy32", "advance", "ffn"};
  constexpr int nnames = (int)(sizeof(names) / sizeof(names[0]));
  fprintf(stderr, "[decoder_mega] last launch: %d groups x %d workgroups, %d jobs, %d operators, %d group barriers, %.1f us in all (workgroup 0; first job per operator below)\n",
          e.groups, e.group_size, e.njobs, e.nops, e.barriers, (h[e.nops + 1] - h[0]) / 100.0);
  if (!e.xcd) {
    fprintf(stderr, "  groups on one XCD (l2 mode) / XCC masks:");
    for (int g2 = 0; g2 < e.groups && g2 < 32; ++g2) if (h[cnk::kMegaDbgGroupWords + g2]) fprintf(stderr, " %d:%llu/%02llx", g2, h[cnk::kMegaDbgGroupWords + g2] & 1ull, (h[cnk::kMegaDbgGroupWords + g2] >> 16) & 0xffull);
    fprintf(stderr, "\n");
  }
  for (int o = 0; o < e.nops; ++o) {
    const cnk::MegaOp& op = e.pinned[o];
    fprintf(stderr, "  op %2d %-15s strips %4d  barrier %d  %7.2f us", o, (op.type >= 0 && op.type < nnames) ? names[op.type] : "?", op.nbx, op.barrier, (h[o + 1] - h[o]) / 100.0);
    if (op.type <= cnk::MOP_ROWLIN) fprintf(stderr, "   Cin %4d Cout %4d k %d ln %d", op.u.rc.Cin, op.u.rc.Cout, op.u.rc.ktaps, op.u.rc.ln);
    if ((op.type == cnk::MOP_RC114 || op.type == cnk::MOP_RC111) && h[128 + o * 4]) fprintf(stderr, "   [args+warm %.2f stage %.2f strips %.2f barrier %.2f]", (h[128 + o * 4] - h[o]) / 100.0, (h[128 + o * 4 + 1] - h[128 + o * 4]) / 100.0,
                                                               (h[128 + o * 4 + 2] - h[128 + o * 4 + 1]) / 100.0, (h[o + 1] - h[128 + o * 4 + 2]) / 100.0);
    if (op.type == cnk::MOP_RC114 && h[512 + o * 4]) fprintf(stderr, " {stage: sync %.2f issue %.2f return+lds %.2f sync %.2f rest %.2f}", (h[512 + o * 4] - h[128 + o * 4]) / 100.0, (h[512 + o * 4 + 1] - h[512 + o * 4]) / 100.0,
                                                               (h[512 + o * 4 + 2] - h[512 + o * 4 + 1]) / 100.0, (h[512 + o * 4 + 3] - h[512 + o * 4 + 2]) / 100.0, (h[128 + o * 4 + 1] - h[512 + o * 4 + 3]) / 100.0);
    fprintf(stderr, "\n");
  }
}

void conan_streams::launch_mega(MegaProgram& e, hipStream_t st) {
  static const bool stamps = ch::dev_getenv("CONAN_MEGA_STAMPS") != nullptr;
  if (stamps && !mega_dbg) mega_dbg = reinterpret_cast<unsigned long long*>(alloc(2 * (size_t)cnk::kMegaDbgWords));
  if (stamps) HIP_CHECK(hipMemsetAsync(mega_dbg, 0, sizeof(unsigned long long) * cnk::kMegaDbgWords, st));
  if (stamps) mega_dbg_prog = (int)(&e - mega_cache.data());
  cnk::MegaLaunch m; memset(&m, 0, sizeof(m));
  m.prog = e.dev; m.nops = e.nops; m.njobs = e.njobs; m.groups = e.groups; m.group_size = e.group_size; m.kw4 = e.kw4; m.lds_bytes = e.lds_bytes;
  m.slots = d_slots; m.pos = pos_dec; m.n = e.n; m.T = e.T;
  m.gbar = mega_bar + 16; m.bar = mega_bar; m.bar_base = mega_bar_count; m.dbg = mega_dbg; m.guard = d_guard; m.wide_regs = rb_limb ? 1 : 0;
  m.xcd = e.xcd ? 1 : 0;
  const bool pipelined = st_front != nullptr && st == st_front;
  if (e.xcd) {
    static const bool pad_always = ch::dev_getenv("CONAN_MEGA_XCD_PAD") != nullptr;
    if (pipelined && !pad_always) m.lds_bytes = e.lds_need;
    mega_xseq = mega_xseq + 1u;
    m.xs = mega_x; m.xseq = mega_xseq; m.xdec_base = mega_xdec;
    if (test_fault == 1) { m.xseq += 7u; mega_xseq += 7u; test_fault = 0; }
    profiled("cnk::decoder_mega_kernel<4, 2>", e.flops, st, [&] { cnk::launch_decoder_mega(m, st); });
    mega_xdec += (unsigned)(e.groups * e.group_size);
    return;
  }
  if (test_fault == 1) { m.bar_base += 1u; test_fault = 0; }
  mega_gseq = mega_gseq + 1u;
  m.xs = mega_x; m.xseq = mega_gseq;
  { const bool nol2 = dev("MEGA_NOL2") != nullptr;
    const char* lay = dev("MEGA_LAYOUT");
    const bool mfast = lay && lay[0] == 'm';
    m.xdec_base = (nol2 ? 1u : 0u) | (mfast ? 2u : 0u); }
  profiled(rb_limb ? "cnk::decoder_mega_kernel<4, 3>" : "cnk::decoder_mega_kernel<6, 3>", e.flops, st, [&] { cnk::launch_decoder_mega(m, st); });
  mega_bar_count += (unsigned)(e.groups * e.group_size);
}

void conan_streams::parse_dev_plan(const char* text) {
  static const char* known[] = {"RESERVE_CUS", "ROWCONV", "RB_NOMERGE", "RB_NOLIMB", "FENCED", "DEC_MEGA", "MEGA_GRID", "FRONT_CUSTRIDE", "EMF_CUSTRIDE", "MEGA_GS",
                                "MEGA_NARROW", "MEGA_NOL2", "MEGA_LAYOUT", "FRONT_PRIO", "RB_UNFUSED", "RB_FUSED", "RB_PAIR", "RB_NOPAIR", "RP_MIN_SLOTS",
                                "UPS_CFG", "EMF_CLUSTER", "EMF_UNFUSED", "NO_TALL", "TALL_MAXT"};
  dev_plan.clear();
  if (!text) return;
  const std::string t(text);
  size_t p = 0;
  while (p < t.size()) {
    size_t q = t.find(';', p);
    if (q == std::string::npos) q = t.size();
    std::string item = t.substr(p, q - p);
    p = q + 1;
    while (!item.empty() && item.front() == ' ') item.erase(item.begin());
    while (!item.empty() && item.back() == ' ') item.pop_back();
    if (item.empty()) continue;
    const size_t eq = item.find('=');
    const std::string name = item.substr(0, eq), value = eq == std::string::npos ? "1" : item.substr(eq + 1);
    bool ok = false;
    for (const char* k : known) ok = ok || name == k;
    if (!ok) throw Error(CONAN_ERR_INVALID, "conan_streams_opts.dev_plan: unknown switch '" + name + "'");
    dev_plan[name] = value;
  }
}

void conan_streams::set_slots(const int32_t* slots, int n, hipStream_t st) {
  if (n <= 0 || n > max_slots) throw Error(CONAN_ERR_INVALID, "slot count out of range");
  bool same = (int)h_slots.size() == n;
  for (int i = 0; i < n; ++i) {
    if (slots[i] < 0 || slots[i] >= max_slots) throw Error(CONAN_ERR_INVALID, "slot index out of range");
    if (same && h_slots[i] != slots[i]) same = false;
  }
  if (same) return;
  if (++slot_gen == 0x7fffffff) { std::fill(slot_seen.begin(), slot_seen.end(), 0); slot_gen = 1; }
  for (int i = 0; i < n; ++i) {
    if (slot_seen[slots[i]] == slot_gen) throw Error(CONAN_ERR_INVALID, "duplicate slot");
    slot_seen[slots[i]] = slot_gen;
  }
  h_slots.assign(slots, slots + n);
  std::vector<int> up(h_slots); up.resize((size_t)n + cnk::kSlotTablePad, h_slots.back());
  pin.upload(d_slots, up.data(), up.size(), st);
}


void conan_streams::async_init() {
  if (st_front) return;
  {
    int lo = 0, hi = 0;
    HIP_CHECK(hipDeviceGetStreamPriorityRange(&lo, &hi));
    const char* e = dev("FRONT_PRIO");
    const int mode = e ? atoi(e) : 0;
    auto masked = [&](hipStream_t* st, const char* env) {
      const char* v = dev(env);
      const int stride = v ? atoi(v) : 0;
      if (stride < 2) { HIP_CHECK(hipStreamCreateWithFlags(st, hipStreamNonBlocking)); return; }
      std::vector<uint32_t> mask((ctx->num_cu + 31) / 32, 0u);
      for (int i = 0; i < ctx->num_cu; i += stride) mask[i / 32] |= 1u << (i % 32);
      HIP_CHECK(hipExtStreamCreateWithCUMask(st, (uint32_t)mask.size(), mask.data()));
    };
    if (mode == 0) {
      masked(&st_front, "FRONT_CUSTRIDE");
      HIP_CHECK(hipStreamCreateWithFlags(&st_voc, hipStreamNonBlocking));
      masked(&st_emf, "EMF_CUSTRIDE");
    } else {
      HIP_CHECK(hipStreamCreateWithPriority(&st_emf, hipStreamNonBlocking, mode > 0 ? hi : lo));
      HIP_CHECK(hipStreamCreateWithPriority(&st_front, hipStreamNonBlocking, mode > 0 ? hi : lo));
      HIP_CHECK(hipStreamCreateWithPriority(&st_voc, hipStreamNonBlocking, mode > 0 ? lo : hi));
    }
  }
  for (int i = 0; i < NP; ++i) {
    HIP_CHECK(hipEventCreateWithFlags(&ev_in[i], hipEventDisableTiming));
    HIP_CHECK(hipEventCreateWithFlags(&ev_fence[i], hipEventDisableTiming));
    HIP_CHECK(hipEventCreateWithFlags(&ev_emf[i], hipEventDisableTiming));
    codes_hand[i] = (int*)alloc((size_t)max_slots * max_frames);
    HIP_CHECK(hipEventCreateWithFlags(&ev_front[i], hipEventDisableTiming));
    HIP_CHECK(hipEventCreateWithFlags(&ev_voc[i], hipEventDisableTiming));
    mel_hand[i] = alloc((size_t)max_slots * max_frames * ctx->cfg.num_mels);
  }
}

void conan_streams::join(hipStream_t st) {
  if (async_steps == 0) return;
  const int last = (int)((async_steps - 1) % NP);
  HIP_CHECK(hipStreamWaitEvent(st, ev_emf[last], 0));
  HIP_CHECK(hipStreamWaitEvent(st, ev_front[last], 0));
  HIP_CHECK(hipStreamWaitEvent(st, ev_voc[last], 0));
}


void conan_streams::build_vocoder() {
  const conan_cfg& c = ctx->cfg;
  int maxk = 0;
  for (int b = 0; b < c.voc_num_resblocks; ++b) maxk = std::max(maxk, c.voc_rb_kernels[b]);
  v_mel = mk_ring(c.num_mels, 1, 6, &voc_state);
  v_pre = mk_ring(c.voc_initial_channel, 1, c.voc_up_kernels[0] - 1, &voc_state);
  int ch_ = c.voc_initial_channel, rate = 1;
  v_st.resize(c.voc_num_ups);
  for (int i = 0; i < c.voc_num_ups; ++i) {
    VocStage& s = v_st[i];
    rate *= c.voc_up_rates[i];
    ch_ /= 2;
    s.C = ch_; s.rate = rate;
    s.fused = c.voc_resblock != 2 && dev("RB_UNFUSED") == nullptr && (max_slots >= (rb_limb ? 4 : 8) || ch_ <= 32 || dev("RB_FUSED") != nullptr);
    for (int b = 0; b < c.voc_num_resblocks && s.fused; ++b)
      for (int d = 0; d < c.voc_rb_num_dil; ++d)
        s.fused = s.fused && cnk::resblock_fused_supported(ch_, c.voc_rb_kernels[b], (c.voc_rb_kernels[b] - 1) * c.voc_rb_dilations[b][d]);
    const bool limb_groups = rb_limb && max_slots >= 16 && dev("RB_PAIR") == nullptr;
    if (!s.fused && !limb_groups && c.voc_resblock != 2 && dev("RB_UNFUSED") == nullptr && dev("RB_NOPAIR") == nullptr &&
        c.voc_num_resblocks <= kMaxBranches && max_slots >= (dev("RP_MIN_SLOTS") ? atoi(dev("RP_MIN_SLOTS")) : 16) && max_frames * rate <= 32) {
      s.pair = true;
      for (int b = 0; b < c.voc_num_resblocks; ++b)
        for (int d = 0; d < c.voc_rb_num_dil; ++d)
          s.pair = s.pair && cnk::resblock_pair_supported(ch_, c.voc_rb_kernels[b], (c.voc_rb_kernels[b] - 1) * c.voc_rb_dilations[b][d], max_frames * rate);
      s.fused = s.pair;
    }
    int up_hist = (maxk - 1) * c.voc_rb_dilations[0][0];
    if (s.fused) for (int b = 0; b < c.voc_num_resblocks; ++b) up_hist = std::max(up_hist, (c.voc_rb_kernels[b] - 1) * (c.voc_rb_dilations[b][0] + 1));
    s.up = mk_ring(ch_, rate, up_hist, &voc_state);
    const int next_pad = (i + 1 < c.voc_num_ups) ? c.voc_up_kernels[i + 1] - 1 : 6;
    s.xs = mk_ring(ch_, rate, next_pad, &voc_state);
    if (!s.fused) s.upa = mk_ring(ch_, rate, (maxk - 1) * c.voc_rb_dilations[0][0], &voc_state);
    s.xt.resize(c.voc_num_resblocks); s.xo.resize(c.voc_num_resblocks); s.xa.resize(c.voc_num_resblocks);
    for (int b = 0; b < c.voc_num_resblocks; ++b)
      for (int d = 0; d < c.voc_rb_num_dil; ++d) {
        const int k = c.voc_rb_kernels[b];
        if (!s.fused) s.xt[b].push_back(mk_ring(ch_, rate, k - 1, &voc_state));
        const int h = (d + 1 < c.voc_rb_num_dil) ? (k - 1) * (c.voc_rb_dilations[b][d + 1] + (s.fused ? 1 : 0)) : next_pad;
        s.xo[b].push_back(mk_ring(ch_, rate, h, &voc_state));
        if (!s.fused && d + 1 < c.voc_rb_num_dil) s.xa[b].push_back(mk_ring(ch_, rate, h, &voc_state));
      }
    if (s.pair) {
      s.xh.resize(c.voc_num_resblocks);
      for (int b = 0; b < c.voc_num_resblocks; ++b)
        for (int d = 0; d < c.voc_rb_num_dil; ++d) s.xh[b].push_back(mk_ring(ch_, rate, c.voc_rb_kernels[b] - 1, &voc_state));
      for (int w = 0; w < 2 && !rp_xb[w]; ++w) {
        const int pairs = ctx->num_cu / 2;
        rp_xb[w] = alloc(cnk::resblock_pair_xb_floats(ctx->num_cu));
        rp_words[w] = reinterpret_cast<unsigned*>(alloc((size_t)pairs * 14 + 4));
      }
    }
  }
}

void conan_streams::out_stage_init() {
  if (or_wav[0]) return;
  const size_t S = (size_t)max_frames * ctx->hop;
  auto dev = [&](size_t bytes) { void* p = nullptr; HIP_CHECK(hipMalloc(&p, bytes)); allocs.push_back(p); return p; };
  for (int q = 0; q < NS; ++q) {
    or_rows[q] = (cnk::RsOutRow*)dev((size_t)max_slots * sizeof(cnk::RsOutRow));
    or_wav[q] = (float*)dev((size_t)max_slots * S * sizeof(float));
    HIP_CHECK(hipEventCreateWithFlags(&ev_or[q], hipEventDisableTiming));
  }
  or_pin.init((size_t)max_slots * sizeof(cnk::RsOutRow) / sizeof(int));
}

conan_streams::OutPlan conan_streams::out_plan(const int32_t* slots, int n, int frames, float* wav_out, long long natural_ld, const std::vector<int>* dst,
                                               const std::string& who) const {
  if (n < 1 || n > max_slots) throw Error(CONAN_ERR_INVALID, "slot count out of range");
  OutPlan P;
  const int T = frames * ctx->hop;
  const bool flush = frames == 0;
  P.base = wav_out; P.ld = (out_ld && !flush) ? out_ld : natural_ld;
  P.counts.assign(n, T);
  if (dst) P.dst = *dst;
  bool any = false;
  for (int i = 0; i < n && !or_slot.empty(); ++i) {
    if (slots[i] < 0 || slots[i] >= max_slots) throw Error(CONAN_ERR_INVALID, "slot index out of range");
    any = any || or_slot[slots[i]].f;
  }
  P.active = any || dst || P.ld != T;
  if (flush) P.active = false;
  if (!P.active && !flush) return P;
  P.rows.resize(n);
  for (int i = 0; i < n; ++i) {
    if (slots[i] < 0 || slots[i] >= max_slots) throw Error(CONAN_ERR_INVALID, "slot index out of range");
    cnk::RsOutRow& row = P.rows[i];
    memset(&row, 0, sizeof(row));
    row.slot = slots[i]; row.m = T; row.h = T; row.dst = dst ? (*dst)[i] : i;
    if (!or_slot.empty() && or_slot[slots[i]].f) {
      const OrSlot& o = or_slot[slots[i]];
      const ch::RsTable& t = *o.f;
      const std::string where = who + ": slot " + std::to_string(slots[i]) + " (output at " + std::to_string(t.out_rate) + " Hz): ";
      const long long in0 = voc_samples[slots[i]], I = in0 + T;
      long long J = o.out;
      if (flush) { if (!o.flushed) J = t.length(I); }
      else {
        if (o.flushed) throw Error(CONAN_ERR_STATE, where + "conan_streams_flush_output has ended the utterance; reset the slot with CONAN_MODEL_HIFIGAN first");
        J = std::max(t.ready(I), o.out);
      }
      if (I - (t.first(o.out) - 4) > or_ring_len) throw Error(CONAN_ERR_UNSUPPORTED, where + "resampler history ring too small for this configuration");
      if (J - o.out > INT_MAX) throw Error(CONAN_ERR_INVALID, where + "too many samples in one call");
      row.in0 = in0; row.out0 = o.out; row.taps = t.f.taps; row.ph = t.f.ph;
      row.h = (int)(J - o.out); row.orig = t.f.orig; row.nph = t.f.nph; row.w = t.f.w; row.L = t.f.L;
      P.active = P.active || row.h > 0;
      P.win = std::max(P.win, t.win);
      P.flops += 2.0 * row.h * t.f.L;
    } else if (flush) {
      row.h = 0;
    }
    P.counts[i] = row.h;
    if (row.h > P.ld)
      throw Error(CONAN_ERR_INVALID, who + ": slot " + std::to_string(slots[i]) + " (call row " + std::to_string(row.dst) + ") delivers " + std::to_string(row.h) +
                                         " samples, more than the row stride of wav_out_dev in force (" + std::to_string(P.ld) + (flush ? "; conan_streams_output_pending)" : "; conan_streams_set_output_ld)"));
    P.tiles = std::max(P.tiles, (std::max(row.h, row.m) + cnk::kRsTile - 1) / cnk::kRsTile);
  }
  return P;
}

void conan_streams::hifigan_step(int n, int frames, const float* mel_dev, float* wav_out, float* pre_tanh, hipStream_t st, const conan_hifigan_taps* taps,
                                 const OutPlan* op) {
  const conan_cfg& c = ctx->cfg;
  const int* pos = pos_voc;
  const float LR = 0.1f;
  const bool lookahead = c.voc_upsample == 2;
  for (int i = 0; i < n; ++i) {
    if (lookahead && !voc_fresh[h_slots[i]])
      throw Error(CONAN_ERR_STATE, "upsample 'nn' (CausalUpsampleBlock1) looks ahead of the frame it writes: slot " + std::to_string(h_slots[i]) +
                                       " needs conan_streams_reset(CONAN_MODEL_HIFIGAN) before every vocoder step (whole-utterance or windowed forward only)");
    voc_fresh[h_slots[i]] = 0;
  }
  const bool out_rows = op && op->active;
  int oq = -1;
  if (out_rows) {
    out_stage_init();
    oq = (int)(or_calls++ % NS);
    HIP_CHECK(hipStreamWaitEvent(st, ev_or[oq], 0));
    or_pin.upload(reinterpret_cast<int*>(or_rows[oq]), reinterpret_cast<const int*>(op->rows.data()), (size_t)n * sizeof(cnk::RsOutRow) / sizeof(int), st);
  }
  {
    cnk::CopyArgs ca; memset(&ca, 0, sizeof(ca));
    ca.x = ch::lin_ref(const_cast<float*>(mel_dev), frames, c.num_mels); ca.y = v_mel.ref();
    ca.slots = d_slots; ca.pos = pos; ca.lens = nullptr; ca.T = frames; ca.n = n; ca.C = c.num_mels;
    cnk::launch_copy_rows(ca, st);
  }
  {
    ConvArgs a = mk(ctx->conv("voc.conv_pre"), v_mel.ref(), v_pre.ref(), n, frames, pos);
    a.out_act = cnk::ACT_LRELU; a.out_slope = LR;
    conv(a, st);
  }
  auto tap = [&](float* dst, const Ring& r, int T) {
    if (!dst) return;
    cnk::CopyArgs ca; memset(&ca, 0, sizeof(ca));
    ca.x = r.ref(); ca.y = ch::lin_ref(dst, T, r.C); ca.slots = d_slots; ca.pos = pos; ca.T = T; ca.n = n; ca.C = r.C;
    cnk::launch_copy_rows(ca, st);
  };
  if (taps) tap(taps->conv_pre_act, v_pre, frames);
  const int NB = c.voc_num_resblocks, ND = c.voc_rb_num_dil;
  if (NB > kMaxBranches) throw Error(CONAN_ERR_UNSUPPORTED, "more than 3 resblock branches");
  int ridx = 0;
  bool last_merged = false;
  for (int i = 0; i < c.voc_num_ups; ++i) {
    VocStage& s = v_st[i];
    bool merged = false;
    const int Tin = frames * (s.rate / c.voc_up_rates[i]);
    const int T = frames * s.rate;
    {
      ConvArgs a = mk(ctx->conv("voc.ups." + std::to_string(i)), i == 0 ? v_pre.ref() : v_st[i - 1].xs.ref(), s.up.ref(), n, Tin, pos, 1,
                      lookahead ? 0 : -1);
      if (!s.fused) { a.y2_base = s.upa.base; a.y2_slope = LR; }
      {
        const std::vector<int> forced = [&] { std::vector<int> v; const char* e = dev("UPS_CFG"); if (e) { std::string t(e); size_t p = 0; while (p <= t.size()) { size_t q = t.find(',', p); if (q == std::string::npos) q = t.size(); v.push_back(atoi(t.substr(p, q - p).c_str())); p = q + 1; } } return v; }();
        if (i < (int)forced.size() && forced[i] >= 0 && forced[i] < cnk::NUM_CFG) { ConvGroup g; g.p[0] = a; launch_group(g, 1, forced[i], st); }
        else conv(a, st);
      }
      if (taps) tap(taps->ups[i], s.up, T);
    }
    for (int d = 0; d < ND && s.pair; ++d) {
      if (T > 32) throw Error(CONAN_ERR_INVALID, "more frames in a step than this stream-set was created for");
      cnk::RPArgs ra; memset(&ra, 0, sizeof(ra));
      for (int b = 0; b < NB; ++b) {
        const std::string base = "voc.rbf." + std::to_string(ridx + b);
        cnk::RPProb& pr = ra.p[b];
        pr.w1 = ctx->vec(base + ".c1." + std::to_string(d) + ".w"); pr.b1 = ctx->vec(base + ".c1." + std::to_string(d) + ".b");
        pr.w2 = ctx->vec(base + ".c2." + std::to_string(d) + ".w"); pr.b2 = ctx->vec(base + ".c2." + std::to_string(d) + ".b");
        pr.x = d == 0 ? s.up.ref() : s.xo[b][d - 1].ref();
        pr.y = s.xo[b][d].ref();
        pr.xh = s.xh[b][d].ref();
        pr.k = c.voc_rb_kernels[b]; pr.dil = c.voc_rb_dilations[b][d];
      }
      ra.slots = d_slots; ra.pos = pos; ra.nprob = NB; ra.n = n; ra.T = T; ra.slope = LR;
      launch_rp(ra, st);
      if (d + 1 == ND && mark_wide) { HIP_CHECK(hipEventRecord(mark_wide, st)); for (int q = 0; q < 4; ++q) if (ev_wide[q] == mark_wide) wide_marked[q] = true; }
    }
    for (int d = 0; d < ND && s.fused && !s.pair; ++d) {
      cnk::RBArgs ra; memset(&ra, 0, sizeof(ra));
      for (int b = 0; b < NB; ++b) {
        const std::string base = "voc.rbf." + std::to_string(ridx + b);
        cnk::RBProb& pr = ra.p[b];
        pr.w1 = ctx->vec(base + ".c1." + std::to_string(d) + ".w"); pr.b1 = ctx->vec(base + ".c1." + std::to_string(d) + ".b");
        pr.w2 = ctx->vec(base + ".c2." + std::to_string(d) + ".w"); pr.b2 = ctx->vec(base + ".c2." + std::to_string(d) + ".b");
        pr.w1l = reinterpret_cast<const unsigned short*>(ctx->vec_or_null(base + ".c1." + std::to_string(d) + ".wl"));
        pr.w2l = reinterpret_cast<const unsigned short*>(ctx->vec_or_null(base + ".c2." + std::to_string(d) + ".wl"));
        pr.x = d == 0 ? s.up.ref() : s.xo[b][d - 1].ref();
        pr.y = s.xo[b][d].ref();
        pr.k = c.voc_rb_kernels[b]; pr.dil = c.voc_rb_dilations[b][d];
      }
      ra.slots = d_slots; ra.pos = pos; ra.nprob = NB; ra.n = n; ra.T = T; ra.slope = LR;
      if (d + 1 < ND) launch_rb(ra, s.C, st);
      else { const TRef ym = s.xs.ref(); merged = launch_rb(ra, s.C, st, &ym); }
    }
    for (int d = 0; d < ND && c.voc_resblock == 2; ++d) {
      ConvGroup g1;
      for (int b = 0; b < NB; ++b) {
        const TRef xin = d == 0 ? s.up.ref() : s.xo[b][d - 1].ref();
        const TRef xin_act = d == 0 ? s.upa.ref() : s.xa[b][d - 1].ref();
        ConvArgs a1 = mk(ctx->conv("voc.rb." + std::to_string(ridx + b) + ".c." + std::to_string(d)), xin_act, s.xo[b][d].ref(), n, T, pos,
                         c.voc_rb_dilations[b][d]);
        a1.res = xin; a1.has_res = 1;
        if (d + 1 < ND) { a1.y2_base = s.xa[b][d].base; a1.y2_slope = LR; }
        g1.p[b] = a1;
      }
      launch_group(g1, NB, pick_cfg(plan_n(n) * T, s.C, NB), st);
    }
    for (int d = 0; d < ND && c.voc_resblock != 2 && !s.fused; ++d) {
      ConvGroup g1, g2;
      for (int b = 0; b < NB; ++b) {
        const TRef xin = d == 0 ? s.up.ref() : s.xo[b][d - 1].ref();
        const TRef xin_act = d == 0 ? s.upa.ref() : s.xa[b][d - 1].ref();
        std::string base = "voc.rb." + std::to_string(ridx + b);
        ConvArgs a1 = mk(ctx->conv(base + ".c1." + std::to_string(d)), xin_act, s.xt[b][d].ref(), n, T, pos, c.voc_rb_dilations[b][d]);
        a1.out_act = cnk::ACT_LRELU; a1.out_slope = LR;
        g1.p[b] = a1;
        ConvArgs a2 = mk(ctx->conv(base + ".c2." + std::to_string(d)), s.xt[b][d].ref(), s.xo[b][d].ref(), n, T, pos, 1);
        a2.res = xin; a2.has_res = 1;
        if (d + 1 < ND) { a2.y2_base = s.xa[b][d].base; a2.y2_slope = LR; }
        g2.p[b] = a2;
      }
      const int cfg = pick_cfg(plan_n(n) * T, s.C, NB);
      launch_group(g1, NB, cfg, st);
      launch_group(g2, NB, cfg, st);
    }
    const bool tap_last = taps && taps->stage_out[i] && i + 1 == c.voc_num_ups && !merged;
    last_merged = merged || tap_last;
    if ((i + 1 < c.voc_num_ups || tap_last) && !merged) {
      cnk::MeanActArgs ma; memset(&ma, 0, sizeof(ma));
      for (int b = 0; b < NB; ++b) ma.x[b] = s.xo[b][ND - 1].ref();
      ma.y = s.xs.ref(); ma.slots = d_slots; ma.pos = pos; ma.nsrc = NB; ma.T = T; ma.n = n; ma.C = s.C; ma.slope = LR;
      cnk::launch_mean_act(ma, st);
    }
    if (taps) tap(taps->stage_out[i], s.xs, T);
    ridx += NB;
  }
  {
    VocStage& s = v_st.back();
    const int T = frames * s.rate;
    cnk::ConvPostArgs a; memset(&a, 0, sizeof(a));
    if (last_merged) { a.x[0] = s.xs.ref(); a.nsrc = 1; }
    else { for (int b = 0; b < NB; ++b) a.x[b] = s.xo[b][ND - 1].ref(); a.nsrc = NB; a.xmean = s.xs.ref(); }
    a.slope = LR;
    a.w = ctx->vec("voc.conv_post.w"); a.bias = ctx->scalars.at("voc.conv_post.b");
    a.wav = out_rows ? or_wav[oq] : wav_out; a.pre = pre_tanh; a.slots = d_slots; a.pos = pos; a.T = T; a.n = n; a.C = s.C; a.k = (int)ctx->scalars.at("voc.conv_post.k");
    a.adv_pos = pos_voc; a.adv_delta = frames; a.adv_ticket = cp_ticket[ws_index(st)];
    cnk::launch_conv_post(a, st);
    if (out_rows) {
      cnk::ResampleOutArgs ra;
      ra.wav = or_wav[oq]; ra.wav_ld = T; ra.ring = or_ring; ra.ring_len = or_ring_len; ra.out = op->base; ra.out_ld = op->ld;
      ra.rows = or_rows[oq]; ra.n = n; ra.tiles = op->tiles; ra.win = op->win;
      profiled("resample_out_kernel", op->flops, st, [&] { cnk::launch_resample_out(ra, st); });
      HIP_CHECK(hipEventRecord(ev_or[oq], st));
    }
    if (!op || op->dst.empty()) out_counts.assign(n, T);
    for (int i = 0; i < n; ++i) {
      const int slot = h_slots[i];
      voc_samples[slot] += T;
      if (!op) continue;
      if (!or_slot.empty() && or_slot[slot].f && out_rows) or_slot[slot].out += op->counts[i];
      out_counts[op->dst.empty() ? i : op->dst[i]] = op->counts[i];
    }
  }
}


void conan_streams::build_emformer() {
  const conan_cfg& c = ctx->cfg;
  const int D = c.emf_input_dim, Q = c.emf_segment + c.emf_right_context;
  for (int l = 0; l < c.emf_layers; ++l) {
    Ring r; r.C = D; r.rate = 1; r.L = ch::next_pow2(c.emf_left_context + c.emf_segment); r.slot_stride = (long long)r.L * D;
    r.base = alloc((size_t)max_slots * r.slot_stride); emf_state.push_back({r.base, r.slot_stride}); e_k.push_back(r);
    Ring v = r; v.base = alloc((size_t)max_slots * r.slot_stride); emf_state.push_back({v.base, v.slot_stride}); e_v.push_back(v);
  }
  const int M = c.emf_max_memory_size, QP = Q + (M > 0 ? 1 : 0);
  e_x[0] = mk_lin(QP, D); e_x[1] = mk_lin(QP, D); e_ln = mk_lin(M + QP, D); e_q = mk_lin(QP, D); e_kv = mk_lin(M + Q, 2 * D);
  e_att = mk_lin(QP, D); e_r1 = mk_lin(QP, D); e_ffn = mk_lin(QP, D); e_h = mk_lin(QP, c.emf_ffn_dim); e_r2 = mk_lin(QP, D);
  e_logits = mk_lin(c.emf_segment, c.emf_output_dim);
  if (M > 0) {
    e_bank_rows = ch::next_pow2(M + 1);
    for (int l = 0; l < c.emf_layers; ++l) {
      float* b = alloc((size_t)max_slots * e_bank_rows * D);
      emf_state.push_back({b, (long long)e_bank_rows * D});
      e_bank.push_back(b);
    }
    e_mems[0] = alloc((size_t)max_slots * D); e_mems[1] = alloc((size_t)max_slots * D);
  }
  cnk::EmfFusedArgs& a = emf_fused_args; memset(&a, 0, sizeof(a));
  if (c.emf_layers <= cnk::EMF_MAX_LAYERS) {
    for (int l = 0; l < c.emf_layers; ++l) {
      const std::string nm = "emf." + std::to_string(l);
      cnk::EmfLayerW& w = a.layers[l];
      const ch::PackedConv &q = ctx->conv(nm + ".q"), &kv = ctx->conv(nm + ".kv"), &o = ctx->conv(nm + ".out"), &f1 = ctx->conv(nm + ".ff1"), &f2 = ctx->conv(nm + ".ff2");
      if (D % 16 || c.emf_ffn_dim % 64) return;
      w.wqkv = ctx->vec(nm + ".fqkv"); w.wo = ctx->vec(nm + ".fo"); w.w1 = ctx->vec(nm + ".f1"); w.w2 = ctx->vec(nm + ".f2");
      {
        const int F = c.emf_ffn_dim;
        float* pb = alloc((size_t)11 * D + F);
        auto put = [&](int off, const float* src, int n) { HIP_CHECK(hipMemcpy(pb + off, src, (size_t)n * sizeof(float), hipMemcpyDeviceToDevice)); };
        put(0, q.bias, D); put(D, kv.bias, 2 * D); put(3 * D, o.bias, D); put(4 * D, f2.bias, D);
        put(5 * D, ctx->vec(nm + ".ln_in.g"), D); put(6 * D, ctx->vec(nm + ".ln_in.b"), D);
        put(7 * D, ctx->vec(nm + ".ln_ff.g"), D); put(8 * D, ctx->vec(nm + ".ln_ff.b"), D);
        put(9 * D, ctx->vec(nm + ".ln_out.g"), D); put(10 * D, ctx->vec(nm + ".ln_out.b"), D);
        put(11 * D, f1.bias, F);
        w.params = pb;
      }
      a.kring[l] = e_k[l].base; a.vring[l] = e_v[l].base;
    }
    a.ring_slot_stride = e_k[0].slot_stride; a.lmask = e_k[0].L - 1;
    if (c.emf_output_dim != D) { a.wp = ctx->vec("emf.fproj"); a.bp = ctx->conv("emf.proj").bias; }
    a.slots = d_slots; a.past = pos_emf;
    a.L = c.emf_layers; a.R = c.emf_right_context; a.U = c.emf_segment; a.D = D; a.H = c.emf_heads; a.LC = c.emf_left_context;
    a.F = c.emf_ffn_dim; a.K = c.emf_output_dim; a.scaling = 1.0f / std::sqrt((float)(D / c.emf_heads));
    if (M > 0) {
      a.M = M; a.MB = e_bank_rows; a.tanh_on_mem = c.emf_tanh_on_mem; a.bank_slot_stride = (long long)e_bank_rows * D;
      for (int l = 0; l < c.emf_layers; ++l) {
        a.bank_k[l] = alloc((size_t)max_slots * e_bank_rows * D); emf_state.push_back({a.bank_k[l], a.bank_slot_stride});
        a.bank_v[l] = alloc((size_t)max_slots * e_bank_rows * D); emf_state.push_back({a.bank_v[l], a.bank_slot_stride});
      }
    }
    { const unsigned long long per_g = (unsigned long long)std::max(c.emf_left_context, 1) * (D / 4); a.magic_per_g = (unsigned)(((1ull << 32) + per_g - 1) / per_g); }
    {
      const size_t xf = cnk::emformer_cluster_xch_floats(std::min(max_slots, std::max(1, ctx->num_cu / 2)), D), fw = cnk::emformer_cluster_flag_words(max_slots);
      a.xch = alloc(xf);
      unsigned* words = reinterpret_cast<unsigned*>(alloc(fw));
      HIP_CHECK(hipMemset(words, 0, fw * sizeof(unsigned)));
      a.xflag = words; a.xepoch = words + (size_t)max_slots * cnk::EMF_MAX_LAYERS * cnk::EMF_MAX_CLUSTER;
      const char* e = dev("EMF_CLUSTER");
      emf_cluster = e ? atoi(e) : 0;
    }
    const char* off = dev("EMF_UNFUSED");
    emf_fused = cnk::emformer_fused_supported(a) && !(off && off[0] == '1');
  }
}

void conan_streams::emformer_step(int n, const float* chunk, float* out, float* logits, int32_t* codes, hipStream_t st) {
  const conan_cfg& c = ctx->cfg;
  const int D = c.emf_input_dim, R = c.emf_right_context, U = c.emf_segment, Q = R + U;
  if (emf_fused) {
    cnk::EmfFusedArgs a = emf_fused_args;
    a.chunk = chunk; a.out = out; a.logits = logits; a.codes = codes; a.n = n; a.fenced = fenced ? 1 : 0;
    a.guard = d_guard; a.fault = 0;
    {
      const int groups = (n + cnk::emformer_fused_streams_per_block(a) - 1) / cnk::emformer_fused_streams_per_block(a);
      const bool masked = dev("EMF_CUSTRIDE") != nullptr && atoi(dev("EMF_CUSTRIDE")) >= 2;
      const bool pipelined = st_emf != nullptr && st == st_emf;
      const bool alone = (!pipelined || pipe_idle) && !shared_device && live && live->load() == 1;
      const int cap = (emf_cluster > 0 || alone) ? ctx->num_cu : 64;
      a.cs = emf_cluster > 0 ? std::min(emf_cluster, (int)cnk::EMF_MAX_CLUSTER) : cnk::EMF_MAX_CLUSTER;
      while (a.cs & (a.cs - 1)) a.cs &= a.cs - 1;
      while (a.cs > 1 && groups * a.cs > cap) a.cs >>= 1;
      if (masked && st == st_emf) a.cs = 1;
      if (test_fault == 2 && a.cs > 1) { a.fault = 0x40000000u; test_fault = 0; }
    }
    const double Q = R + U + (c.emf_max_memory_size > 0 ? 1 : 0), Dd = D, F = c.emf_ffn_dim, keys = c.emf_max_memory_size + R + c.emf_left_context + U;
    const double fl = (double)n * (c.emf_layers * (2.0 * Q * Dd * (4.0 * Dd + 2.0 * F) + 4.0 * Q * keys * Dd) + 2.0 * U * Dd * c.emf_output_dim);
    profiled(D == 80 ? "cnk::emformer_fused_kernel<5, 10>" : "cnk::emformer_fused_kernel<4, 8>", fl, st, [&] { cnk::launch_emformer_fused(a, st); });
    return;
  }
  const int M = c.emf_max_memory_size, QP = Q + (M > 0 ? 1 : 0);
  {
    cnk::CopyArgs ca; memset(&ca, 0, sizeof(ca));
    ca.slots = nullptr; ca.pos = nullptr; ca.lens = nullptr; ca.n = n; ca.C = D;
    ca.x = ch::lin_ref(const_cast<float*>(chunk), Q, D, U); ca.y = e_x[0].ref(0); ca.T = R; if (R > 0) cnk::launch_copy_rows(ca, st);
    ca.x = ch::lin_ref(const_cast<float*>(chunk), Q, D, 0); ca.y = e_x[0].ref(R); ca.T = U; cnk::launch_copy_rows(ca, st);
  }
  if (M > 0) cnk::launch_emf_seg_mean(e_x[0].base, e_mems[0], n, QP, R, U, D, st);
  int cur = 0, mcur = 0;
  auto ln = [&](const TRef& x, const TRef& y, float* g, float* b, const TRef* pre) {
    cnk::LNArgs a; memset(&a, 0, sizeof(a));
    a.x = x; a.y = y; a.gamma = g; a.beta = b; a.slots = nullptr; a.pos = nullptr; a.lens = nullptr; a.T = Q; a.n = n; a.C = D; a.eps = 1e-5f;
    if (pre) { a.pre = *pre; a.has_pre = 1; }
    cnk::launch_layernorm(a, st);
  };
  for (int l = 0; l < c.emf_layers; ++l) {
    const std::string nm = "emf." + std::to_string(l);
    Lin& x = e_x[cur];
    ln(x.ref(), e_ln.ref(M), ctx->vec(nm + ".ln_in.g"), ctx->vec(nm + ".ln_in.b"), nullptr);
    if (M > 0) {
      cnk::EmfMemArgs ma; memset(&ma, 0, sizeof(ma));
      ma.ln = e_ln.base; ma.bank = e_bank[l]; ma.mems_in = e_mems[mcur]; ma.slots = d_slots; ma.past = pos_emf;
      ma.n = n; ma.R = R; ma.U = U; ma.D = D; ma.M = M; ma.MB = e_bank_rows; ma.seg = c.emf_segment;
      cnk::launch_emf_mem_prep(ma, st);
    }
    conv(mk(ctx->conv(nm + ".q"), e_ln.ref(M), e_q.ref(), n, QP, nullptr), st);
    conv(mk(ctx->conv(nm + ".kv"), e_ln.ref(0), e_kv.ref(), n, M + Q, nullptr), st);
    {
      cnk::EmfAttnArgs a; memset(&a, 0, sizeof(a));
      a.q = e_q.base; a.kv = e_kv.base; a.out = e_att.base; a.kring = e_k[l].base; a.vring = e_v[l].base;
      a.ring_slot_stride = e_k[l].slot_stride; a.slots = d_slots; a.past = pos_emf;
      a.n = n; a.R = R; a.U = U; a.D = D; a.H = c.emf_heads; a.LC = c.emf_left_context; a.lmask = e_k[l].L - 1;
      a.scaling = 1.0f / std::sqrt((float)(D / c.emf_heads));
      a.M = M; a.seg = c.emf_segment;
      cnk::launch_emf_attn(a, st);
    }
    {
      ConvArgs a = mk(ctx->conv(nm + ".out"), e_att.ref(), e_r1.ref(), n, QP, nullptr);
      a.res = x.ref(); a.has_res = 1;
      conv(a, st);
    }
    if (M > 0) {
      cnk::launch_emf_mem_out(e_r1.base, e_mems[mcur ^ 1], n, QP, Q, D, c.emf_tanh_on_mem, st);
      mcur ^= 1;
    }
    ln(e_r1.ref(), e_ffn.ref(), ctx->vec(nm + ".ln_ff.g"), ctx->vec(nm + ".ln_ff.b"), nullptr);
    { ConvArgs a = mk(ctx->conv(nm + ".ff1"), e_ffn.ref(), e_h.ref(), n, Q, nullptr); a.out_act = cnk::ACT_RELU; conv(a, st); }
    { ConvArgs a = mk(ctx->conv(nm + ".ff2"), e_h.ref(), e_r2.ref(), n, Q, nullptr); a.res = e_r1.ref(); a.has_res = 1; conv(a, st); }
    ln(e_r2.ref(), e_x[cur ^ 1].ref(), ctx->vec(nm + ".ln_out.g"), ctx->vec(nm + ".ln_out.b"), nullptr);
    cur ^= 1;
  }
  if (out) {
    cnk::CopyArgs ca; memset(&ca, 0, sizeof(ca));
    ca.n = n; ca.C = D; ca.T = U; ca.x = e_x[cur].ref(R); ca.y = ch::lin_ref(out, U, D);
    cnk::launch_copy_rows(ca, st);
  }
  if (logits || codes) {
    float* lg = logits ? logits : e_logits.base;
    const int K = c.emf_output_dim;
    if (c.emf_output_dim != D) conv(mk(ctx->conv("emf.proj"), e_x[cur].ref(R), ch::lin_ref(lg, U, K), n, U, nullptr), st);
    else { cnk::CopyArgs ca; memset(&ca, 0, sizeof(ca)); ca.n = n; ca.C = D; ca.T = U; ca.x = e_x[cur].ref(R); ca.y = ch::lin_ref(lg, U, D); cnk::launch_copy_rows(ca, st); }
    if (codes) { cnk::ArgmaxArgs a; a.x = lg; a.idx = codes; a.rows = n * U; a.C = K; cnk::launch_argmax(a, st); }
  }
  cnk::launch_advance(pos_emf, d_slots, n, U, st);
}


void conan_streams::build_decoder() {
  const conan_cfg& c = ctx->cfg;
  const int H = c.hidden_size, F = max_frames;
  c_emb = mk_ring(H, 1, c.content_kernel - 1, &dec_state);
  c_pin2 = mk_ring(H, 1, c.predictor_kernel - 1, &dec_state);
  const int n_uv = (int)ctx->scalars.at("conan.uv.n"), uvh = (int)ctx->scalars.at("conan.uv.hidden"), ffn = (int)ctx->scalars.at("conan.align.ffn");
  for (int i = 0; i + 1 < n_uv; ++i) c_uvh.push_back(mk_ring(ctx->conv("conan.uv." + std::to_string(i)).Cout, 1, c.predictor_kernel - 1, &dec_state));
  for (int b = 0; b < c.dec_num_blocks; ++b)
    for (int j = 0; j < c.dec_layers_in_block; ++j) c_lnrs.push_back(mk_ring(H, 1, (c.dec_kernel - 1) * c.dec_dilations[b], &dec_state));
  c_lastr = mk_ring(H, 1, c.dec_post_kernel - 1, &dec_state);
  c_pin = mk_lin(F, H); c_q = mk_lin(F, H); c_att = mk_lin(F, H); c_a1 = mk_lin(F, H); c_a2 = mk_lin(F, H);
  c_ff = mk_lin(F, ffn); c_uv5 = mk_lin(F, uvh); c_x[0] = mk_lin(F, H); c_x[1] = mk_lin(F, H); c_h = mk_lin(F, 2 * H);
  c_post = mk_lin(F, H); c_mask_blk = mk_lin(F, 1); c_mask_blk2 = mk_lin(F, 1); c_mask_out = mk_lin(F, 1); c_mel = mk_lin(F, c.num_mels);
  c_part = mk_lin(F, 32 * H);
  c_part2 = mk_lin(F, 16 * H);
  S_max = (max_ref + 3) / 4;
  if (S_max > 512) throw Error(CONAN_ERR_UNSUPPORTED, "max_ref_frames > 2048");
  c_style = alloc((size_t)max_slots * H);
  c_kv = alloc((size_t)max_slots * 2 * S_max * 2 * H);
  c_kmask = alloc((size_t)max_slots * S_max);
  c_slen = (int*)alloc((size_t)max_slots);
  c_vqids = (int*)alloc((size_t)max_slots * S_max);
  sp_batch = std::min(max_slots, 8);
  const int TR = max_ref + 2 * PADR, SR = S_max + 2 * PADR;
  s_mel = mk_lin(TR, c.num_mels, sp_batch); s_np = mk_lin(TR, 1, sp_batch); s_wnm = mk_lin(TR, 1, sp_batch);
  s_x[0] = mk_lin(TR, H, sp_batch); s_x[1] = mk_lin(TR, H, sp_batch); s_ln = mk_lin(TR, H, sp_batch); s_h = mk_lin(TR, 2 * H, sp_batch);
  s_blkm = mk_lin(TR, 1, sp_batch);
  const int NM = c.num_mels;
  s_wx = mk_lin(TR, NM, sp_batch); s_wout = mk_lin(TR, NM, sp_batch); s_win = mk_lin(TR, 2 * NM, sp_batch); s_acts = mk_lin(TR, NM, sp_batch);
  s_rs = mk_lin(TR, 2 * NM, sp_batch);
  s_ph = mk_lin(SR, NM, sp_batch); s_pm = mk_lin(SR, 1, sp_batch); s_px[0] = mk_lin(SR, NM, sp_batch); s_px[1] = mk_lin(SR, NM, sp_batch);
  s_pln = mk_lin(SR, NM, sp_batch); s_phh = mk_lin(SR, 2 * NM, sp_batch); s_pblk = mk_lin(SR, 1, sp_batch);
  s_enc = mk_lin(SR, H, sp_batch); s_dots = mk_lin(SR, c.nvq, sp_batch); s_cat = mk_lin(SR, 2 * H, sp_batch); s_tok = mk_lin(SR, H, sp_batch);
  s_kvtmp = mk_lin(SR, 2 * H, sp_batch);
  s_ids = (int*)alloc((size_t)sp_batch * S_max);
}
```

Baseline: 48240.

## Hand over first-conv halo rows between limb resblock tiles via flags

Adds a halo mode to the limb resblock kernel. A tile no longer recomputes the extra row block of the first convolution that overlaps its neighbour. Instead it reads the already split bf16 limb tail that the previous tile publishes in a per-slot tail buffer, and it waits on an epoch-tagged flag. This cuts the redundant first-conv GEMM work and shrinks the window LDS. In exchange it adds cross-workgroup spin waits with a timeout guard, extra global tail storage, and ordering dependencies between tiles. It is enabled by default for 128-channel stages.

```diff
diff --git a/conan_amd/csrc/kernels.h b/conan_amd/csrc/kernels.h
--- a/conan_amd/csrc/kernels.h
+++ b/conan_amd/csrc/kernels.h
@@ -37,7 +37,7 @@
 
 constexpr unsigned long long kSpinBudgetTicks = 5000000ull;
 constexpr unsigned long long kSpinGapTicks = 100000ull;
-enum WaitCode { WAIT_MEGA_BARRIER = 1, WAIT_EMF_CLUSTER = 2, WAIT_PAIR_FLAG = 3, WAIT_PAIR_MAILBOX = 4, WAIT_RETIRED_5 = 5 , WAIT_MEGA_ELECT = 6, WAIT_MEGA_DECIDED = 7, WAIT_MEGA_FLAGS = 8 };
+enum WaitCode { WAIT_MEGA_BARRIER = 1, WAIT_EMF_CLUSTER = 2, WAIT_PAIR_FLAG = 3, WAIT_PAIR_MAILBOX = 4, WAIT_RETIRED_5 = 5 , WAIT_MEGA_ELECT = 6, WAIT_MEGA_DECIDED = 7, WAIT_MEGA_FLAGS = 8, WAIT_LIMB_HALO = 9 };
 struct SpinGuard { unsigned long long last = 0, acc = 0; unsigned it = 0; };
 #if defined(__HIPCC__)
 __device__ __forceinline__ bool spin_expired(SpinGuard& g, unsigned* guard, unsigned code) {
@@ -156,6 +156,14 @@
   int merge;
   TRef ymean;
   unsigned long long* dbg;
+  int halo;
+  unsigned short* xtail[3];
+  long long xtail_stride;
+  int xtail_lmask;
+  unsigned hepoch;
+  unsigned* hflag;
+  int hflag_words;
+  unsigned* guard;
 };
 bool resblock_fused_supported(int C, int kmax, int span_max);
 int resblock_fused_rows(int C, int T, int n, int ksum, int kmax, int num_cu);
@@ -168,6 +176,7 @@
 int resblock_limb_rows(int C, int span_max);
 bool launch_resblock_limb(const RBArgs& a, int C, int rows, int num_cu, hipStream_t st);
 bool resblock_limb_can_merge(int C, int rows);
+bool resblock_limb_has_halo(int C, int rows, int kmax);
 const char* resblock_limb_name(int C, int rows, bool merge = false);
 
 
diff --git a/conan_amd/csrc/resblock_limb.hip b/conan_amd/csrc/resblock_limb.hip
--- a/conan_amd/csrc/resblock_limb.hip
+++ b/conan_amd/csrc/resblock_limb.hip
@@ -5,6 +5,7 @@
 #include "kernels.h"
 
 #define RL_MAX_SLOTS 256
+#define RL_HALO_KMAX 11
 
 #ifndef RL_HELPER_PRIO
 #define RL_HELPER_PRIO 3
@@ -56,14 +57,15 @@
   return (f32x2){__builtin_fmaxf(x[0], sx[0]), __builtin_fmaxf(x[1], sx[1])};
 }
 
-template <int C_, int NR2_, int SPAN_>
+template <int C_, int NR2_, int SPAN_, bool HALO_ = false>
 struct RLGeom {
   static constexpr int C = C_, NR2 = NR2_;
-  static constexpr int NR1 = NR2 + 1;
+  static constexpr int NR1 = HALO_ ? NR2 : NR2 + 1;
   static constexpr int RO = 16 * NR2;
-  static constexpr int XT_ROWS = 16 * NR1;
+  static constexpr int C1_ROWS = 16 * NR1;
+  static constexpr int XT_ROWS = 16 * (NR2 + 1);
   static constexpr int MAXSPAN = SPAN_;
-  static constexpr int WR_MAX = XT_ROWS + MAXSPAN;
+  static constexpr int WR_MAX = C1_ROWS + MAXSPAN;
   static constexpr int LDB = C + 16;
   static constexpr int PLW = WR_MAX * LDB;
   static constexpr int PLX = XT_ROWS * LDB;
@@ -218,382 +220,14 @@
 
 template <int C, int NR2, int SPAN, bool MERGE>
 __global__ __launch_bounds__(512, 2) void resblock_limb_kernel(const RBArgs a) {
-  using G = RLGeom<C, NR2, SPAN>;
-  constexpr int LDB = G::LDB;
-  __shared__ __attribute__((aligned(16))) u16 lds[G::LDS_U16 + 16 + 4 * RL_MAX_SLOTS];
-  u16* const win = lds;
-  u16* const xt = lds + 3 * G::PLW;
-  float* const accimg = reinterpret_cast<float*>(xt);
-  int* const meta = reinterpret_cast<int*>(lds + G::LDS_U16);
-  int* const sptab = meta + 8;
-  const int tid = threadIdx.x;
-  const int lane = tid & 63;
-  const int wave = __builtin_amdgcn_readfirstlane(tid >> 6);
-  const int ntiles = a.ntiles;
-  const float slope = a.slope;
-  const int T = a.T;
-  constexpr bool merge = MERGE;
-  const int np = a.nprob;
-
-  if (wave >= 4) {
-    const int ht = tid - 256;
-    __builtin_amdgcn_s_setprio(RL_HELPER_PRIO);
-    auto hbar = [&]() __attribute__((always_inline)) { asm volatile("s_waitcnt lgkmcnt(0)\n\ts_barrier" ::: "memory"); };
-    constexpr int NIT = (G::WR_MAX * G::C4 + 255) / 256;
-    float4 wv[NIT];
-    int wtotal = 0, wzr = 0;
-    auto win_issue = [&](const int p, const int i, const int t0, const int slot, const int pos) __attribute__((always_inline)) {
-      const int k = RL_SEL(p, k), d = RL_SEL(p, dil);
-      const int wr = G::XT_ROWS + (k - 1) * d;
-      const int tw0 = t0 - (k - 1) - (k - 1) * d;
-      const int xmode = a.p[0].x.mode, xrate = a.p[0].x.rate;
-      const float* xb = RL_SEL(p, x.base) + (long long)(xmode == 0 ? slot : i) * RL_SEL(p, x.slot_stride);
-      const unsigned rbase = (xmode == 0 ? (unsigned)pos * (unsigned)xrate : 0u) + (unsigned)(RL_SEL(p, x.off) + tw0);
-      const unsigned rmask = xmode == 0 ? (unsigned)RL_SEL(p, x.lmask) : 0xffffffffu;
-      wtotal = wr * G::C4;
-#pragma unroll
-      for (int u = 0; u < NIT; ++u) {
-        const int idx = ht + 256 * u;
-        const int w = idx / G::C4, c4 = idx - w * G::C4;
-        const unsigned row = (rbase + (unsigned)w) & rmask;
-        wv[u] = idx < wtotal ? rl_gload4(xb + (long long)row * C + c4 * 4) : make_float4(0.f, 0.f, 0.f, 0.f);
-      }
-      const long long abs0 = (xmode == 0 ? (long long)pos * xrate : 0ll) + t0 - (k - 1);
-      wzr = abs0 >= 0 ? 0 : (abs0 < -(long long)G::XT_ROWS ? G::XT_ROWS : (int)-abs0);
-    };
-    auto win_write = [&]() __attribute__((always_inline)) {
-#pragma unroll
-      for (int u = 0; u < NIT; ++u) {
-        const int idx = ht + 256 * u;
-        const int w = idx / G::C4, c4 = idx - w * G::C4;
-        unsigned h[2], m[2], l[2];
-        rl_split2(rl_lrelu2((f32x2){wv[u].x, wv[u].y}, slope), h[0], m[0], l[0]);
-        rl_split2(rl_lrelu2((f32x2){wv[u].z, wv[u].w}, slope), h[1], m[1], l[1]);
-        if (idx < wtotal) {
-          u16* dst = win + w * LDB + c4 * 4;
-          *reinterpret_cast<uint2*>(dst) = make_uint2(h[0], h[1]);
-          *reinterpret_cast<uint2*>(dst + G::PLW) = make_uint2(m[0], m[1]);
-          *reinterpret_cast<uint2*>(dst + 2 * G::PLW) = make_uint2(l[0], l[1]);
-        }
-      }
-      if (ht == 0) meta[0] = wzr;
-    };
-    constexpr int NOUT = (G::RO * G::C4) / 256;
-    static_assert((G::RO * G::C4) % 256 == 0 && 256 % G::C4 == 0, "output tile / helper threads");
-    const int oc4 = ht % G::C4;
-    float4 oacc[NOUT], ores[NOUT], osum[MERGE ? NOUT : 1], ob2 = make_float4(0.f, 0.f, 0.f, 0.f);
-    const float* oxb = nullptr; const float* ob2p = nullptr;
-    float* oyb = nullptr;
-    unsigned oyr0 = 0, oym = 0, oxr0 = 0, oxm = 0;
-    int ot0 = 0, op = 0, oyC = C;
-#pragma unroll
-    for (int u = 0; u < (MERGE ? NOUT : 1); ++u) osum[u] = make_float4(0.f, 0.f, 0.f, 0.f);
-    auto out_fetch = [&](const int p, const int i, const int t0, const int slot, const int pos) __attribute__((always_inline)) {
-      const int xmode = a.p[0].x.mode, xrate = a.p[0].x.rate, ymode = a.p[0].y.mode, yrate = a.p[0].y.rate;
-      oxb = RL_SEL(p, x.base) + (long long)(xmode == 0 ? slot : i) * RL_SEL(p, x.slot_stride);
-      oxr0 = (xmode == 0 ? (unsigned)pos * (unsigned)xrate : 0u) + (unsigned)(RL_SEL(p, x.off) + t0);
-      oxm = xmode == 0 ? (unsigned)RL_SEL(p, x.lmask) : 0xffffffffu;
-      if (!merge) {
-        oyb = RL_SEL(p, y.base) + (long long)(ymode == 0 ? slot : i) * RL_SEL(p, y.slot_stride);
-        oyr0 = (ymode == 0 ? (unsigned)pos * (unsigned)yrate : 0u) + (unsigned)(RL_SEL(p, y.off) + t0);
-        oym = ymode == 0 ? (unsigned)RL_SEL(p, y.lmask) : 0xffffffffu;
-      } else {
-        const int mmode = a.ymean.mode;
-        oyb = a.ymean.base + (long long)(mmode == 0 ? slot : i) * a.ymean.slot_stride;
-        oyr0 = (mmode == 0 ? (unsigned)pos * (unsigned)a.ymean.rate : 0u) + (unsigned)(a.ymean.off + t0);
-        oym = mmode == 0 ? (unsigned)a.ymean.lmask : 0xffffffffu;
-        oyC = a.ymean.C;
-      }
-      ot0 = t0; op = p;
-      ob2p = RL_SEL(p, b2) + oc4 * 4;
-#pragma unroll
-      for (int u = 0; u < NOUT; ++u) oacc[u] = *reinterpret_cast<const float4*>(accimg + ((ht + 256 * u) / G::C4) * G::LDA + oc4 * 4);
-      ob2 = rl_gload4(ob2p);
-#pragma unroll
-      for (int u = 0; u < NOUT; ++u) {
-        const int r = (ht + 256 * u) / G::C4;
-        ores[u] = ot0 + r < T ? rl_gload4(oxb + (long long)((oxr0 + (unsigned)r) & oxm) * C + oc4 * 4) : make_float4(0.f, 0.f, 0.f, 0.f);
-      }
-    };
-    auto out_store = [&]() __attribute__((always_inline)) {
-#pragma unroll
-      for (int u = 0; u < NOUT; ++u) {
-        const int r = (ht + 256 * u) / G::C4;
-        if (ot0 + r < T) {
-          const float4 v = make_float4((oacc[u].x + ob2.x) + ores[u].x, (oacc[u].y + ob2.y) + ores[u].y, (oacc[u].z + ob2.z) + ores[u].z, (oacc[u].w + ob2.w) + ores[u].w);
-          if constexpr (!MERGE) rl_gstore4(oyb + (long long)((oyr0 + (unsigned)r) & oym) * C + oc4 * 4, v);
-          else {
-            float4 sm = osum[MERGE ? u : 0];
-            if (op == 0) sm = v; else { sm.x += v.x; sm.y += v.y; sm.z += v.z; sm.w += v.w; }
-            osum[MERGE ? u : 0] = sm;
-            if (op == np - 1) {
-              const float dn = (float)np;
-              if (np > 1) { sm.x /= dn; sm.y /= dn; sm.z /= dn; sm.w /= dn; }
-              sm.x = sm.x > 0.f ? sm.x : sm.x * slope; sm.y = sm.y > 0.f ? sm.y : sm.y * slope;
-              sm.z = sm.z > 0.f ? sm.z : sm.z * slope; sm.w = sm.w > 0.f ? sm.w : sm.w * slope;
-              rl_gstore4(oyb + (long long)((oyr0 + (unsigned)r) & oym) * oyC + oc4 * 4, sm);
-            }
-          }
-        }
-      }
-    };
-#if RL_STAMPS
-    const unsigned long long h_t0 = __builtin_amdgcn_s_memtime();
-    unsigned long long h_t[6] = {0, 0, 0, 0, 0, 0};
-#define RL_HT(i_) h_t[i_] = __builtin_amdgcn_s_memtime() - h_t0
-#else
-#define RL_HT(i_)
-#endif
-    int dv0 = 0;
-    if (wave == 4 && lane == 0) dv0 = __hip_atomic_fetch_add(a.sched, 1, __ATOMIC_RELAXED, __HIP_MEMORY_SCOPE_AGENT);
-    for (int e = ht; e < a.n; e += 256) {
-      const int sl = a.slots ? *(gci)(a.slots + e) : e;
-      sptab[2 * e] = sl; sptab[2 * e + 1] = a.pos ? *(gci)(a.pos + sl) : 0;
-    }
-    const int tps = a.tiles_per_slot, per_prob = a.n * tps;
-    auto decode = [&](const int e, int& p, int& i, int& t0) __attribute__((always_inline)) {
-      if constexpr (!MERGE) {
-        const int b = e / per_prob, rem = e - b * per_prob;
-        p = b == 0 ? a.order[0] : (b == 1 ? a.order[1] : a.order[2]);
-        i = rem / tps; t0 = (rem - i * tps) * G::RO;
-      } else {
-        const int g = e / np;
-        p = e - g * np; i = g / tps; t0 = (g - i * tps) * G::RO;
-      }
-    };
-    int cur = -1, p = -1, i = 0, t0 = 0;
-    if (wave == 4) {
-      cur = __builtin_amdgcn_readfirstlane(dv0) * (merge ? np : 1);
-      if (cur >= ntiles) cur = -1;
-      if (cur >= 0) decode(cur, p, i, t0);
-      if (lane == 0) { meta[1] = cur; meta[2] = p; meta[3] = 0; }
-    }
-    RL_HT(0);
-    asm volatile("s_waitcnt lgkmcnt(0)\n\ts_barrier" ::: "memory");
-    RL_HT(1);
-    if (wave != 4) {
-      cur = __builtin_amdgcn_readfirstlane(meta[1]);
-      if (cur >= 0) decode(cur, p, i, t0);
-    }
-    if (cur >= 0) {
-    int slot = __builtin_amdgcn_readfirstlane(sptab[2 * i]), pos = __builtin_amdgcn_readfirstlane(sptab[2 * i + 1]);
-    win_issue(p, i, t0, slot, pos);
-    RL_HT(2);
-    int gen = 1;
-    int dv = 0, dnext = -1;
-    auto draw_issue = [&](const int have, const int idx_prev, const int p_prev) __attribute__((always_inline)) {
-      if (wave == 4 && lane == 0 && have) {
-        if (merge && p_prev != np - 1) dnext = idx_prev + 1;
-        else { dnext = -1; dv = __hip_atomic_fetch_add(a.sched, 1, __ATOMIC_RELAXED, __HIP_MEMORY_SCOPE_AGENT); }
-      }
-    };
-    auto draw_take = [&](const int have) __attribute__((always_inline)) {
-      int idx = -1;
-      if (!have) return idx;
-      if (wave == 4) {
-        const int drawn = dv * (merge ? np : 1);
-        idx = __builtin_amdgcn_readfirstlane(dnext >= 0 ? dnext : drawn);
-        if (idx >= ntiles) idx = -1;
-        if (lane == 0) {
-          meta[1] = idx;
-          asm volatile("s_waitcnt lgkmcnt(0)" ::: "memory");
-          __hip_atomic_store(&meta[3], gen, __ATOMIC_RELEASE, __HIP_MEMORY_SCOPE_WORKGROUP);
-        }
-      } else {
-        while (__hip_atomic_load(&meta[3], __ATOMIC_ACQUIRE, __HIP_MEMORY_SCOPE_WORKGROUP) != gen) __builtin_amdgcn_s_sleep(4);
-        idx = __builtin_amdgcn_readfirstlane(meta[1]);
-      }
-      ++gen;
-      return idx;
-    };
-    const bool deep = ntiles >= 5 * (int)gridDim.x * (merge ? np : 1);
-    auto stage = [&](const int e) __attribute__((always_inline)) {
-      int pe, ie, te;
-      decode(e, pe, ie, te);
-      win_issue(pe, ie, te, __builtin_amdgcn_readfirstlane(sptab[2 * ie]), __builtin_amdgcn_readfirstlane(sptab[2 * ie + 1]));
-      return pe;
-    };
-    int nxt = -1, pn = -1;
-    if (deep) {
-      draw_issue(1, cur, p);
-      nxt = draw_take(1);
-    }
-    RL_HT(3);
-    win_write();
-    RL_HT(4);
-    hbar();
-    RL_HT(5);
-#if RL_STAMPS
-    if (a.dbg && blockIdx.x == 0 && wave == 4 && lane == 0) { unsigned long long* q = a.dbg + 256 * 4 + 12; for (int e = 0; e < 6; ++e) q[e] = h_t[e]; }
-#endif
-    bool pending = false;
-    for (;;) {
-      const bool have = deep ? nxt >= 0 : true;
-      if (deep && nxt >= 0) pn = stage(nxt);
-      draw_issue(have, deep ? nxt : cur, deep ? pn : p);
-      if (pending) out_store();
-      int nn = -1;
-      if (!deep) {
-        nxt = draw_take(have); pn = -1;
-        if (nxt >= 0) pn = stage(nxt);
-      }
-      if (ht == 0) meta[2] = nxt >= 0 ? pn : -1;
-      hbar();
-      hbar();
-      if (nxt >= 0) win_write();
-      hbar();
-      hbar();
-      out_fetch(p, i, t0, slot, pos);
-      pending = true;
-      if (deep) nn = draw_take(have);
-      if (nxt < 0) break;
-      cur = nxt;
-      decode(cur, p, i, t0);
-      slot = __builtin_amdgcn_readfirstlane(sptab[2 * i]); pos = __builtin_amdgcn_readfirstlane(sptab[2 * i + 1]);
-      nxt = nn;
-    }
-    if (pending) out_store();
-    }
-    if (ht == 0) {
-      const int d = __hip_atomic_fetch_add(a.sched + 1, 1, __ATOMIC_RELAXED, __HIP_MEMORY_SCOPE_AGENT);
-      if (d == (int)gridDim.x - 1) {
-        __hip_atomic_store(a.sched, 0, __ATOMIC_RELAXED, __HIP_MEMORY_SCOPE_AGENT);
-        __hip_atomic_store(a.sched + 1, 0, __ATOMIC_RELAXED, __HIP_MEMORY_SCOPE_AGENT);
-      }
-    }
-    return;
-  }
-
-  if (RL_MATRIX_PRIO) __builtin_amdgcn_s_setprio(RL_MATRIX_PRIO);
-  auto bar = [&]() __attribute__((always_inline)) { asm volatile("s_waitcnt lgkmcnt(0)\n\ts_barrier" ::: "memory"); };
-  const int wc = wave % (4 / G::RSPLIT);
-  const int wr = wave / (4 / G::RSPLIT);
-  const int ct0 = wc * G::NCW;
-  const int lr = lane & 15, lg = lane >> 4;
-#if RL_STAMPS
-  unsigned long long st_gemm = 0, st_t0 = __builtin_amdgcn_s_memtime(), st_r0 = __builtin_amdgcn_s_memrealtime(), st_bar = 0, st_b3 = 0, st_b1 = 0, st_b4 = 0, st_b2 = 0, st_e1 = 0, st_e2 = 0, st_tiles = 0, st_head = 0, st_pre = 0, st_mid = 0;
-#define RL_T() __builtin_amdgcn_s_memtime()
-#define RL_BAR(acc_) do { const unsigned long long q0_ = RL_T(); bar(); const unsigned long long q1_ = RL_T(); acc_ += q1_ - q0_; st_bar += q1_ - q0_; } while (0)
-#define RL_GEMM(...) do { const unsigned long long s0_ = RL_T(); __VA_ARGS__; asm volatile("s_nop 0" ::"v"(acc[0][0][0])); st_gemm += RL_T() - s0_; } while (0)
-#else
-#define RL_BAR(acc_) bar()
-#define RL_GEMM(...) __VA_ARGS__
-#endif
-  f32x4 bw[G::RING][G::NCW][3];
-  bar();
-  int p = __builtin_amdgcn_readfirstlane(meta[2]);
-  if (p < 0) return;
-  {
-    const long long cs = (long long)(RL_SEL(p, k) + 1) * G::KB * G::BLK;
-    rl_prefetch_w<G::NCW, G::RING>(bw, RL_SEL(p, w1l) + (long long)ct0 * cs + lane * 8, cs);
-  }
-  bar();
-#if RL_STAMPS
-  st_head = RL_T() - st_t0;
-#endif
-  while (p >= 0) {
-#if RL_STAMPS
-    const unsigned long long top_ = RL_T();
-#endif
-    const int k = RL_SEL(p, k), d = RL_SEL(p, dil);
-    const u16* const w1 = RL_SEL(p, w1l);
-    const u16* const w2 = RL_SEL(p, w2l);
-    const float* const b1 = RL_SEL(p, b1);
-    const long long ct_stride = (long long)(k + 1) * G::KB * G::BLK;
-    const int zrows = __builtin_amdgcn_readfirstlane(meta[0]);
-    f32x4 b1v[G::NCW];
-#pragma unroll
-    for (int c = 0; c < G::NCW; ++c) b1v[c] = rl_gload(b1 + (ct0 + c) * 16 + 4 * lg);
-    int pn;
-    {
-      f32x4 acc[G::NRW1][G::NCW];
-#pragma unroll
-      for (int r = 0; r < G::NRW1; ++r)
-#pragma unroll
-        for (int c = 0; c < G::NCW; ++c) acc[r][c] = (f32x4){0.f, 0.f, 0.f, 0.f};
-      const int rt0 = wr * G::NRW1;
-#if RL_STAMPS
-      st_pre += RL_T() - top_;
-#endif
-      RL_GEMM(rl_gemm<G::NRW1, G::NCW, LDB, G::KB, G::RING>(win, G::PLW, rt0 * 16, d, k, w1 + (long long)ct0 * ct_stride + lane * 8, ct_stride,
-                                                           w2 + (long long)ct0 * ct_stride + lane * 8, ct_stride, acc, bw, lane));
-      RL_BAR(st_b3);
-#if RL_STAMPS
-      const unsigned long long e1_0 = RL_T();
-#endif
-      auto epilogue1 = [&](auto zr_c) __attribute__((always_inline)) {
-        constexpr bool ZR = decltype(zr_c)::value;
-#pragma unroll
-        for (int c = 0; c < G::NCW; ++c) {
-          const int col = (ct0 + c) * 16 + 4 * lg;
-#pragma unroll
-          for (int r = 0; r < G::NRW1; ++r) {
-            if (rt0 + r < G::NR1) {
-              const int m = (rt0 + r) * 16 + lr;
-              unsigned h[2], mm[2], l[2];
-              const f32x4 v = acc[r][c] + b1v[c];
-              rl_split2(rl_lrelu2((f32x2){v[0], v[1]}, slope), h[0], mm[0], l[0]);
-              rl_split2(rl_lrelu2((f32x2){v[2], v[3]}, slope), h[1], mm[1], l[1]);
-              const bool zr = ZR && m < zrows;
-              u16* dst = xt + m * LDB + col;
-              *reinterpret_cast<uint2*>(dst) = zr ? make_uint2(0u, 0u) : make_uint2(h[0], h[1]);
-              *reinterpret_cast<uint2*>(dst + G::PLX) = zr ? make_uint2(0u, 0u) : make_uint2(mm[0], mm[1]);
-              *reinterpret_cast<uint2*>(dst + 2 * G::PLX) = zr ? make_uint2(0u, 0u) : make_uint2(l[0], l[1]);
-            }
-          }
-        }
-      };
-      if (zrows > 0) epilogue1(std::true_type{}); else epilogue1(std::false_type{});
-#if RL_STAMPS
-      asm volatile("s_waitcnt lgkmcnt(0)" ::: "memory"); st_e1 += RL_T() - e1_0; ++st_tiles;
-#endif
-    }
-    RL_BAR(st_b1);
-#if RL_STAMPS
-    const unsigned long long mid_ = RL_T();
-#endif
-    pn = __builtin_amdgcn_readfirstlane(meta[2]);
-    const int pnx = pn >= 0 ? pn : p;
-    const long long csn = (long long)(RL_SEL(pnx, k) + 1) * G::KB * G::BLK;
-    const u16* const w1n = RL_SEL(pnx, w1l) + (long long)ct0 * csn + lane * 8;
-    {
-      f32x4 acc[G::NRW2][G::NCW];
-#pragma unroll
-      for (int r = 0; r < G::NRW2; ++r)
-#pragma unroll
-        for (int c = 0; c < G::NCW; ++c) acc[r][c] = (f32x4){0.f, 0.f, 0.f, 0.f};
-      const int rt0 = wr * G::NRW2;
-#if RL_STAMPS
-      st_mid += RL_T() - mid_;
-#endif
-      RL_GEMM(rl_gemm<G::NRW2, G::NCW, LDB, G::KB, G::RING>(xt, G::PLX, rt0 * 16, 1, k, w2 + (long long)ct0 * ct_stride + lane * 8, ct_stride,
-                                                           w1n, csn, acc, bw, lane));
-      RL_BAR(st_b4);
-#if RL_STAMPS
-      const unsigned long long e2_0 = RL_T();
-#endif
-#pragma unroll
-      for (int c = 0; c < G::NCW; ++c) {
-        const int col = (ct0 + c) * 16 + 4 * lg;
-#pragma unroll
-        for (int r = 0; r < G::NRW2; ++r) {
-          if (rt0 + r < NR2) *reinterpret_cast<f32x4*>(accimg + ((rt0 + r) * 16 + lr) * G::LDA + col) = acc[r][c];
-        }
-      }
-#if RL_STAMPS
-      asm volatile("s_waitcnt lgkmcnt(0)" ::: "memory"); st_e2 += RL_T() - e2_0;
-#endif
-    }
-    RL_BAR(st_b2);
-    p = pn;
-  }
-#if RL_STAMPS
-  if (a.dbg && tid == 0) {
-    unsigned long long* o = a.dbg + blockIdx.x * 4;
-    if (blockIdx.x == 0) { unsigned long long* q = a.dbg + 256 * 4; q[0] = st_b3; q[1] = st_b1; q[2] = st_b4; q[3] = st_b2; q[4] = st_e1; q[5] = st_e2; q[6] = st_tiles; q[7] = st_gemm; q[8] = __builtin_amdgcn_s_memtime() - st_t0; q[9] = st_head; q[10] = st_pre; q[11] = st_mid; }
-    o[0] = st_gemm; o[1] = __builtin_amdgcn_s_memtime() - st_t0; o[2] = __builtin_amdgcn_s_memrealtime() - st_r0; o[3] = st_bar;
-  }
-#endif
+  constexpr bool HALO = false;
+#include "resblock_limb_body.inc"
+}
+
+template <int C, int NR2, int SPAN, bool MERGE>
+__global__ __launch_bounds__(512, 2) void rl_halo_kernel(const RBArgs a) {
+  constexpr bool HALO = true;
+#include "resblock_limb_body.inc"
 }
 
 
@@ -630,6 +264,15 @@
   std::stable_sort(a.order, a.order + a.nprob, [&](int x, int y) { return a.p[x].k > a.p[y].k; });
   const int grid = std::min(a.merge ? total / a.nprob : total, num_cu);
   a.tiles = nullptr; a.ntiles = total;
+  if constexpr (C >= 64) {
+    if (a.halo) {
+      for (int p = 0; p < a.nprob; ++p) if (a.p[p].k > RL_HALO_KMAX) return false;
+      if (a.p[0].x.mode != 0 || !a.pos || !a.hflag || a.hepoch == 0u || (long long)total * 4 > a.hflag_words || a.xtail_lmask + 1 < a.T + 16) return false;
+      for (int p = 0; p < a.nprob; ++p) if (!a.xtail[p]) return false;
+      hipLaunchKernelGGL((rl_halo_kernel<C, NR2, SPAN, MERGE>), dim3(grid), dim3(512), 0, st, a);
+      return true;
+    }
+  } else if (a.halo) return false;
   hipLaunchKernelGGL((resblock_limb_kernel<C, NR2, SPAN, MERGE>), dim3(grid), dim3(512), 0, st, a);
   return true;
 }
@@ -648,6 +291,8 @@
   return false;
 }
 
+bool resblock_limb_has_halo(int C, int rows, int kmax) { return kmax <= RL_HALO_KMAX && ((C == 64 && rows == 80) || (C == 128 && rows == 32)); }
+
 bool resblock_limb_can_merge(int C, int rows) { return (C == 32 && rows == 160) || (C == 64 && rows == 80) || (C == 128 && rows == 32); }
 
 const char* resblock_limb_name(int C, int rows, bool merge) {
diff --git a/conan_amd/csrc/resblock_limb_body.inc b/conan_amd/csrc/resblock_limb_body.inc
--- /dev/null
+++ b/conan_amd/csrc/resblock_limb_body.inc
@@ -0,0 +1,471 @@
+  using G = RLGeom<C, NR2, SPAN, HALO>;
+  constexpr int LDB = G::LDB;
+  __shared__ __attribute__((aligned(16))) u16 lds[G::LDS_U16 + 16 + 4 * RL_MAX_SLOTS];
+  u16* const win = lds;
+  u16* const xt = lds + 3 * G::PLW;
+  float* const accimg = reinterpret_cast<float*>(xt);
+  int* const meta = reinterpret_cast<int*>(lds + G::LDS_U16);
+  int* const sptab = meta + 8;
+  const int tid = threadIdx.x;
+  const int lane = tid & 63;
+  const int wave = __builtin_amdgcn_readfirstlane(tid >> 6);
+  const int ntiles = a.ntiles;
+  const float slope = a.slope;
+  const int T = a.T;
+  constexpr bool merge = MERGE;
+  const int np = a.nprob;
+
+  if (wave >= 4) {
+    const int ht = tid - 256;
+    __builtin_amdgcn_s_setprio(RL_HELPER_PRIO);
+    auto hbar = [&]() __attribute__((always_inline)) { asm volatile("s_waitcnt lgkmcnt(0)\n\ts_barrier" ::: "memory"); };
+    constexpr int NIT = (G::WR_MAX * G::C4 + 255) / 256;
+    float4 wv[NIT];
+    int wtotal = 0, wzr = 0;
+    int wabs = 0, wvalid = 0, wslot = 0, wflag = 0;
+    auto win_issue = [&](const int p, const int i, const int t0, const int slot, const int pos) __attribute__((always_inline)) {
+      const int k = RL_SEL(p, k), d = RL_SEL(p, dil);
+      const int wr = G::C1_ROWS + (k - 1) * d;
+      const int tw0 = t0 - (HALO ? 0 : k - 1) - (k - 1) * d;
+      const int xmode = a.p[0].x.mode, xrate = a.p[0].x.rate;
+      const float* xb = RL_SEL(p, x.base) + (long long)(xmode == 0 ? slot : i) * RL_SEL(p, x.slot_stride);
+      const unsigned rbase = (xmode == 0 ? (unsigned)pos * (unsigned)xrate : 0u) + (unsigned)(RL_SEL(p, x.off) + tw0);
+      const unsigned rmask = xmode == 0 ? (unsigned)RL_SEL(p, x.lmask) : 0xffffffffu;
+      wtotal = wr * G::C4;
+#pragma unroll
+      for (int u = 0; u < NIT; ++u) {
+        const int idx = ht + 256 * u;
+        const int w = idx / G::C4, c4 = idx - w * G::C4;
+        const unsigned row = (rbase + (unsigned)w) & rmask;
+        wv[u] = idx < wtotal ? rl_gload4(xb + (long long)row * C + c4 * 4) : make_float4(0.f, 0.f, 0.f, 0.f);
+      }
+      const long long abs0 = (xmode == 0 ? (long long)pos * xrate : 0ll) + t0 - (k - 1);
+      wzr = (HALO || abs0 >= 0) ? 0 : (abs0 < -(long long)G::XT_ROWS ? G::XT_ROWS : (int)-abs0);
+      if constexpr (HALO) {
+        wabs = (int)((unsigned)pos * (unsigned)xrate + (unsigned)t0); wvalid = T - t0 < G::RO ? T - t0 : G::RO; wslot = slot;
+        wflag = (p * a.n + i) * a.tiles_per_slot + t0 / G::RO;
+      }
+    };
+    auto win_write = [&]() __attribute__((always_inline)) {
+#pragma unroll
+      for (int u = 0; u < NIT; ++u) {
+        const int idx = ht + 256 * u;
+        const int w = idx / G::C4, c4 = idx - w * G::C4;
+        unsigned h[2], m[2], l[2];
+        rl_split2(rl_lrelu2((f32x2){wv[u].x, wv[u].y}, slope), h[0], m[0], l[0]);
+        rl_split2(rl_lrelu2((f32x2){wv[u].z, wv[u].w}, slope), h[1], m[1], l[1]);
+        if (idx < wtotal) {
+          u16* dst = win + w * LDB + c4 * 4;
+          *reinterpret_cast<uint2*>(dst) = make_uint2(h[0], h[1]);
+          *reinterpret_cast<uint2*>(dst + G::PLW) = make_uint2(m[0], m[1]);
+          *reinterpret_cast<uint2*>(dst + 2 * G::PLW) = make_uint2(l[0], l[1]);
+        }
+      }
+      if (ht == 0) {
+        meta[0] = wzr;
+        if constexpr (HALO) { meta[4] = wabs; meta[5] = wvalid; meta[6] = wslot; meta[7] = wflag; }
+      }
+    };
+    constexpr int HQ = 3 * G::C4;
+    constexpr int NHIT = HALO ? ((RL_HALO_KMAX - 1) * HQ + 255) / 256 : 1;
+    unsigned long long hv[NHIT];
+    auto halo_ready = [&](const int p_, const int i_, const int t0_) __attribute__((always_inline)) {
+      const unsigned* f = a.hflag + ((long long)((p_ * a.n + i_) * a.tiles_per_slot + t0_ / G::RO - 1)) * 4;
+      unsigned v = a.hepoch;
+      if (lane < 4) v = __hip_atomic_load(f + lane, __ATOMIC_RELAXED, __HIP_MEMORY_SCOPE_AGENT);
+      return __builtin_amdgcn_ballot_w64(v != a.hepoch) == 0ull;
+    };
+    auto halo_issue = [&](const int p_, const int slot_, const int pos_, const int t0_) __attribute__((always_inline)) {
+      const int k = RL_SEL(p_, k);
+      const unsigned long long* tb = reinterpret_cast<const unsigned long long*>(p_ == 0 ? a.xtail[0] : (p_ == 1 ? a.xtail[1] : a.xtail[2])) + (long long)slot_ * a.xtail_stride;
+      const unsigned r0 = (unsigned)pos_ * (unsigned)a.p[0].x.rate + (unsigned)(t0_ - (k - 1));
+      const int total = (k - 1) * HQ;
+#pragma unroll
+      for (int u = 0; u < NHIT; ++u) {
+        const int idx = ht + 256 * u;
+        const int m = idx / HQ, q = idx - m * HQ;
+        const unsigned row = (r0 + (unsigned)m) & (unsigned)a.xtail_lmask;
+        hv[u] = idx < total ? __hip_atomic_load(tb + (row * (unsigned)HQ + (unsigned)q), __ATOMIC_RELAXED, __HIP_MEMORY_SCOPE_AGENT) : 0ull;
+      }
+    };
+    auto halo_write = [&](const int p_) __attribute__((always_inline)) {
+      const int total = (RL_SEL(p_, k) - 1) * HQ;
+#pragma unroll
+      for (int u = 0; u < NHIT; ++u) {
+        const int idx = ht + 256 * u;
+        const int m = idx / HQ, q = idx - m * HQ;
+        const int pl = q / G::C4, c4 = q - pl * G::C4;
+        if (idx < total) *reinterpret_cast<unsigned long long*>(xt + pl * G::PLX + m * LDB + c4 * 4) = hv[u];
+      }
+    };
+    constexpr int NOUT = (G::RO * G::C4) / 256;
+    static_assert((G::RO * G::C4) % 256 == 0 && 256 % G::C4 == 0, "output tile / helper threads");
+    const int oc4 = ht % G::C4;
+    float4 oacc[NOUT], ores[NOUT], osum[MERGE ? NOUT : 1], ob2 = make_float4(0.f, 0.f, 0.f, 0.f);
+    const float* oxb = nullptr; const float* ob2p = nullptr;
+    float* oyb = nullptr;
+    unsigned oyr0 = 0, oym = 0, oxr0 = 0, oxm = 0;
+    int ot0 = 0, op = 0, oyC = C;
+#pragma unroll
+    for (int u = 0; u < (MERGE ? NOUT : 1); ++u) osum[u] = make_float4(0.f, 0.f, 0.f, 0.f);
+    auto out_fetch = [&](const int p, const int i, const int t0, const int slot, const int pos) __attribute__((always_inline)) {
+      const int xmode = a.p[0].x.mode, xrate = a.p[0].x.rate, ymode = a.p[0].y.mode, yrate = a.p[0].y.rate;
+      oxb = RL_SEL(p, x.base) + (long long)(xmode == 0 ? slot : i) * RL_SEL(p, x.slot_stride);
+      oxr0 = (xmode == 0 ? (unsigned)pos * (unsigned)xrate : 0u) + (unsigned)(RL_SEL(p, x.off) + t0);
+      oxm = xmode == 0 ? (unsigned)RL_SEL(p, x.lmask) : 0xffffffffu;
+      if (!merge) {
+        oyb = RL_SEL(p, y.base) + (long long)(ymode == 0 ? slot : i) * RL_SEL(p, y.slot_stride);
+        oyr0 = (ymode == 0 ? (unsigned)pos * (unsigned)yrate : 0u) + (unsigned)(RL_SEL(p, y.off) + t0);
+        oym = ymode == 0 ? (unsigned)RL_SEL(p, y.lmask) : 0xffffffffu;
+      } else {
+        const int mmode = a.ymean.mode;
+        oyb = a.ymean.base + (long long)(mmode == 0 ? slot : i) * a.ymean.slot_stride;
+        oyr0 = (mmode == 0 ? (unsigned)pos * (unsigned)a.ymean.rate : 0u) + (unsigned)(a.ymean.off + t0);
+        oym = mmode == 0 ? (unsigned)a.ymean.lmask : 0xffffffffu;
+        oyC = a.ymean.C;
+      }
+      ot0 = t0; op = p;
+      ob2p = RL_SEL(p, b2) + oc4 * 4;
+#pragma unroll
+      for (int u = 0; u < NOUT; ++u) oacc[u] = *reinterpret_cast<const float4*>(accimg + ((ht + 256 * u) / G::C4) * G::LDA + oc4 * 4);
+      ob2 = rl_gload4(ob2p);
+#pragma unroll
+      for (int u = 0; u < NOUT; ++u) {
+        const int r = (ht + 256 * u) / G::C4;
+        ores[u] = ot0 + r < T ? rl_gload4(oxb + (long long)((oxr0 + (unsigned)r) & oxm) * C + oc4 * 4) : make_float4(0.f, 0.f, 0.f, 0.f);
+      }
+    };
+    auto out_store = [&]() __attribute__((always_inline)) {
+#pragma unroll
+      for (int u = 0; u < NOUT; ++u) {
+        const int r = (ht + 256 * u) / G::C4;
+        if (ot0 + r < T) {
+          const float4 v = make_float4((oacc[u].x + ob2.x) + ores[u].x, (oacc[u].y + ob2.y) + ores[u].y, (oacc[u].z + ob2.z) + ores[u].z, (oacc[u].w + ob2.w) + ores[u].w);
+          if constexpr (!MERGE) rl_gstore4(oyb + (long long)((oyr0 + (unsigned)r) & oym) * C + oc4 * 4, v);
+          else {
+            float4 sm = osum[MERGE ? u : 0];
+            if (op == 0) sm = v; else { sm.x += v.x; sm.y += v.y; sm.z += v.z; sm.w += v.w; }
+            osum[MERGE ? u : 0] = sm;
+            if (op == np - 1) {
+              const float dn = (float)np;
+              if (np > 1) { sm.x /= dn; sm.y /= dn; sm.z /= dn; sm.w /= dn; }
+              sm.x = sm.x > 0.f ? sm.x : sm.x * slope; sm.y = sm.y > 0.f ? sm.y : sm.y * slope;
+              sm.z = sm.z > 0.f ? sm.z : sm.z * slope; sm.w = sm.w > 0.f ? sm.w : sm.w * slope;
+              rl_gstore4(oyb + (long long)((oyr0 + (unsigned)r) & oym) * oyC + oc4 * 4, sm);
+            }
+          }
+        }
+      }
+    };
+#if RL_STAMPS
+    const unsigned long long h_t0 = __builtin_amdgcn_s_memtime();
+    unsigned long long h_t[6] = {0, 0, 0, 0, 0, 0};
+#define RL_HT(i_) h_t[i_] = __builtin_amdgcn_s_memtime() - h_t0
+#else
+#define RL_HT(i_)
+#endif
+    int dv0 = 0;
+    if (wave == 4 && lane == 0) dv0 = __hip_atomic_fetch_add(a.sched, 1, __ATOMIC_RELAXED, __HIP_MEMORY_SCOPE_AGENT);
+    for (int e = ht; e < a.n; e += 256) {
+      const int sl = a.slots ? *(gci)(a.slots + e) : e;
+      sptab[2 * e] = sl; sptab[2 * e + 1] = a.pos ? *(gci)(a.pos + sl) : 0;
+    }
+    const int tps = a.tiles_per_slot, per_prob = a.n * tps;
+    auto decode = [&](const int e, int& p, int& i, int& t0) __attribute__((always_inline)) {
+      if constexpr (!MERGE) {
+        const int b = e / per_prob, rem = e - b * per_prob;
+        p = b == 0 ? a.order[0] : (b == 1 ? a.order[1] : a.order[2]);
+        if constexpr (HALO) { const int rt = rem / a.n; i = rem - rt * a.n; t0 = rt * G::RO; }
+        else { i = rem / tps; t0 = (rem - i * tps) * G::RO; }
+      } else {
+        const int g = e / np;
+        p = e - g * np;
+        if constexpr (HALO) { const int rt = g / a.n; i = g - rt * a.n; t0 = rt * G::RO; }
+        else { i = g / tps; t0 = (g - i * tps) * G::RO; }
+      }
+    };
+    int cur = -1, p = -1, i = 0, t0 = 0;
+    if (wave == 4) {
+      cur = __builtin_amdgcn_readfirstlane(dv0) * (merge ? np : 1);
+      if (cur >= ntiles) cur = -1;
+      if (cur >= 0) decode(cur, p, i, t0);
+      if (lane == 0) { meta[1] = cur; meta[2] = p; meta[3] = 0; }
+    }
+    RL_HT(0);
+    asm volatile("s_waitcnt lgkmcnt(0)\n\ts_barrier" ::: "memory");
+    RL_HT(1);
+    if (wave != 4) {
+      cur = __builtin_amdgcn_readfirstlane(meta[1]);
+      if (cur >= 0) decode(cur, p, i, t0);
+    }
+    if (cur >= 0) {
+    int slot = __builtin_amdgcn_readfirstlane(sptab[2 * i]), pos = __builtin_amdgcn_readfirstlane(sptab[2 * i + 1]);
+    win_issue(p, i, t0, slot, pos);
+    RL_HT(2);
+    int gen = 1;
+    int dv = 0, dnext = -1;
+    auto draw_issue = [&](const int have, const int idx_prev, const int p_prev) __attribute__((always_inline)) {
+      if (wave == 4 && lane == 0 && have) {
+        if (merge && p_prev != np - 1) dnext = idx_prev + 1;
+        else { dnext = -1; dv = __hip_atomic_fetch_add(a.sched, 1, __ATOMIC_RELAXED, __HIP_MEMORY_SCOPE_AGENT); }
+      }
+    };
+    auto draw_take = [&](const int have) __attribute__((always_inline)) {
+      int idx = -1;
+      if (!have) return idx;
+      if (wave == 4) {
+        const int drawn = dv * (merge ? np : 1);
+        idx = __builtin_amdgcn_readfirstlane(dnext >= 0 ? dnext : drawn);
+        if (idx >= ntiles) idx = -1;
+        if (lane == 0) {
+          meta[1] = idx;
+          asm volatile("s_waitcnt lgkmcnt(0)" ::: "memory");
+          __hip_atomic_store(&meta[3], gen, __ATOMIC_RELEASE, __HIP_MEMORY_SCOPE_WORKGROUP);
+        }
+      } else {
+        while (__hip_atomic_load(&meta[3], __ATOMIC_ACQUIRE, __HIP_MEMORY_SCOPE_WORKGROUP) != gen) __builtin_amdgcn_s_sleep(4);
+        idx = __builtin_amdgcn_readfirstlane(meta[1]);
+      }
+      ++gen;
+      return idx;
+    };
+    const bool deep = ntiles >= 5 * (int)gridDim.x * (merge ? np : 1);
+    auto stage = [&](const int e) __attribute__((always_inline)) {
+      int pe, ie, te;
+      decode(e, pe, ie, te);
+      win_issue(pe, ie, te, __builtin_amdgcn_readfirstlane(sptab[2 * ie]), __builtin_amdgcn_readfirstlane(sptab[2 * ie + 1]));
+      return pe;
+    };
+    int nxt = -1, pn = -1;
+    if (deep) {
+      draw_issue(1, cur, p);
+      nxt = draw_take(1);
+    }
+    RL_HT(3);
+    win_write();
+    RL_HT(4);
+    hbar();
+    RL_HT(5);
+#if RL_STAMPS
+    if (a.dbg && blockIdx.x == 0 && wave == 4 && lane == 0) { unsigned long long* q = a.dbg + 256 * 4 + 12; for (int e = 0; e < 6; ++e) q[e] = h_t[e]; }
+#endif
+    bool pending = false;
+    for (;;) {
+      const bool have = deep ? nxt >= 0 : true;
+      if (deep && nxt >= 0) pn = stage(nxt);
+      draw_issue(have, deep ? nxt : cur, deep ? pn : p);
+      if (pending) out_store();
+      int nn = -1;
+      if (!deep) {
+        nxt = draw_take(have); pn = -1;
+        if (nxt >= 0) pn = stage(nxt);
+      }
+      if (ht == 0) meta[2] = nxt >= 0 ? pn : -1;
+      bool hgot = false;
+      if constexpr (HALO && !MERGE) {
+        hgot = t0 == 0 || halo_ready(p, i, t0);
+        if (hgot) halo_issue(p, slot, pos, t0);
+      }
+      hbar();
+      if constexpr (HALO) {
+        if (!hgot) {
+          if (t0 > 0) {
+            SpinGuard sg;
+            while (!halo_ready(p, i, t0)) {
+              __builtin_amdgcn_s_sleep(2);
+              if (spin_expired(sg, a.guard, WAIT_LIMB_HALO)) break;
+            }
+          }
+          halo_issue(p, slot, pos, t0);
+        }
+        halo_write(p);
+      }
+      hbar();
+      if (nxt >= 0) win_write();
+      hbar();
+      hbar();
+      out_fetch(p, i, t0, slot, pos);
+      pending = true;
+      if (deep) nn = draw_take(have);
+      if (nxt < 0) break;
+      cur = nxt;
+      decode(cur, p, i, t0);
+      slot = __builtin_amdgcn_readfirstlane(sptab[2 * i]); pos = __builtin_amdgcn_readfirstlane(sptab[2 * i + 1]);
+      nxt = nn;
+    }
+    if (pending) out_store();
+    }
+    if (ht == 0) {
+      const int d = __hip_atomic_fetch_add(a.sched + 1, 1, __ATOMIC_RELAXED, __HIP_MEMORY_SCOPE_AGENT);
+      if (d == (int)gridDim.x - 1) {
+        __hip_atomic_store(a.sched, 0, __ATOMIC_RELAXED, __HIP_MEMORY_SCOPE_AGENT);
+        __hip_atomic_store(a.sched + 1, 0, __ATOMIC_RELAXED, __HIP_MEMORY_SCOPE_AGENT);
+      }
+    }
+    return;
+  }
+
+  if (RL_MATRIX_PRIO) __builtin_amdgcn_s_setprio(RL_MATRIX_PRIO);
+  auto bar = [&]() __attribute__((always_inline)) { asm volatile("s_waitcnt lgkmcnt(0)\n\ts_barrier" ::: "memory"); };
+  const int wc = wave % (4 / G::RSPLIT);
+  const int wr = wave / (4 / G::RSPLIT);
+  const int ct0 = wc * G::NCW;
+  const int lr = lane & 15, lg = lane >> 4;
+#if RL_STAMPS
+  unsigned long long st_gemm = 0, st_t0 = __builtin_amdgcn_s_memtime(), st_r0 = __builtin_amdgcn_s_memrealtime(), st_bar = 0, st_b3 = 0, st_b1 = 0, st_b4 = 0, st_b2 = 0, st_e1 = 0, st_e2 = 0, st_tiles = 0, st_head = 0, st_pre = 0, st_mid = 0;
+#define RL_T() __builtin_amdgcn_s_memtime()
+#define RL_BAR(acc_) do { const unsigned long long q0_ = RL_T(); bar(); const unsigned long long q1_ = RL_T(); acc_ += q1_ - q0_; st_bar += q1_ - q0_; } while (0)
+#define RL_GEMM(...) do { const unsigned long long s0_ = RL_T(); __VA_ARGS__; asm volatile("s_nop 0" ::"v"(acc[0][0][0])); st_gemm += RL_T() - s0_; } while (0)
+#else
+#define RL_BAR(acc_) bar()
+#define RL_GEMM(...) __VA_ARGS__
+#endif
+  f32x4 bw[G::RING][G::NCW][3];
+  bar();
+  int p = __builtin_amdgcn_readfirstlane(meta[2]);
+  if (p < 0) return;
+  {
+    const long long cs = (long long)(RL_SEL(p, k) + 1) * G::KB * G::BLK;
+    rl_prefetch_w<G::NCW, G::RING>(bw, RL_SEL(p, w1l) + (long long)ct0 * cs + lane * 8, cs);
+  }
+  bar();
+#if RL_STAMPS
+  st_head = RL_T() - st_t0;
+#endif
+  while (p >= 0) {
+#if RL_STAMPS
+    const unsigned long long top_ = RL_T();
+#endif
+    const int k = RL_SEL(p, k), d = RL_SEL(p, dil);
+    const u16* const w1 = RL_SEL(p, w1l);
+    const u16* const w2 = RL_SEL(p, w2l);
+    const float* const b1 = RL_SEL(p, b1);
+    const long long ct_stride = (long long)(k + 1) * G::KB * G::BLK;
+    const int zrows = __builtin_amdgcn_readfirstlane(meta[0]);
+    const int tabs = HALO ? __builtin_amdgcn_readfirstlane(meta[4]) : 0, tvalid = HALO ? __builtin_amdgcn_readfirstlane(meta[5]) : 0;
+    const int tslot = HALO ? __builtin_amdgcn_readfirstlane(meta[6]) : 0, tflag = HALO ? __builtin_amdgcn_readfirstlane(meta[7]) : 0;
+    f32x4 b1v[G::NCW];
+#pragma unroll
+    for (int c = 0; c < G::NCW; ++c) b1v[c] = rl_gload(b1 + (ct0 + c) * 16 + 4 * lg);
+    int pn;
+    {
+      f32x4 acc[G::NRW1][G::NCW];
+#pragma unroll
+      for (int r = 0; r < G::NRW1; ++r)
+#pragma unroll
+        for (int c = 0; c < G::NCW; ++c) acc[r][c] = (f32x4){0.f, 0.f, 0.f, 0.f};
+      const int rt0 = wr * G::NRW1;
+#if RL_STAMPS
+      st_pre += RL_T() - top_;
+#endif
+      RL_GEMM(rl_gemm<G::NRW1, G::NCW, LDB, G::KB, G::RING>(win, G::PLW, rt0 * 16, d, k, w1 + (long long)ct0 * ct_stride + lane * 8, ct_stride,
+                                                           w2 + (long long)ct0 * ct_stride + lane * 8, ct_stride, acc, bw, lane));
+      RL_BAR(st_b3);
+#if RL_STAMPS
+      const unsigned long long e1_0 = RL_T();
+#endif
+      auto epilogue1 = [&](auto zr_c) __attribute__((always_inline)) {
+        constexpr bool ZR = decltype(zr_c)::value;
+#pragma unroll
+        for (int c = 0; c < G::NCW; ++c) {
+          const int col = (ct0 + c) * 16 + 4 * lg;
+#pragma unroll
+          for (int r = 0; r < G::NRW1; ++r) {
+            if (rt0 + r < G::NR1) {
+              const int m = (rt0 + r) * 16 + lr;
+              unsigned h[2], mm[2], l[2];
+              const f32x4 v = acc[r][c] + b1v[c];
+              rl_split2(rl_lrelu2((f32x2){v[0], v[1]}, slope), h[0], mm[0], l[0]);
+              rl_split2(rl_lrelu2((f32x2){v[2], v[3]}, slope), h[1], mm[1], l[1]);
+              const bool zr = ZR && m < zrows;
+              u16* dst = xt + m * LDB + col;
+              *reinterpret_cast<uint2*>(dst) = zr ? make_uint2(0u, 0u) : make_uint2(h[0], h[1]);
+              *reinterpret_cast<uint2*>(dst + G::PLX) = zr ? make_uint2(0u, 0u) : make_uint2(mm[0], mm[1]);
+              *reinterpret_cast<uint2*>(dst + 2 * G::PLX) = zr ? make_uint2(0u, 0u) : make_uint2(l[0], l[1]);
+            }
+          }
+        }
+      };
+      auto epilogue1h = [&]() __attribute__((always_inline)) {
+        unsigned long long* const tb = reinterpret_cast<unsigned long long*>(p == 0 ? a.xtail[0] : (p == 1 ? a.xtail[1] : a.xtail[2])) + (long long)tslot * a.xtail_stride;
+        const int tlo = tvalid - (k - 1);
+#pragma unroll
+        for (int r = G::NRW1 - 1; r >= 0; --r) {
+          if (rt0 + r < G::NR1) {
+            const int m = (rt0 + r) * 16 + lr;
+            const bool tail = m >= tlo && m < tvalid;
+            unsigned long long* const trow = tb + (long long)(((unsigned)tabs + (unsigned)m) & (unsigned)a.xtail_lmask) * (3 * G::C4);
+#pragma unroll
+            for (int c = 0; c < G::NCW; ++c) {
+              const int col = (ct0 + c) * 16 + 4 * lg;
+              unsigned h[2], mm[2], l[2];
+              const f32x4 v = acc[r][c] + b1v[c];
+              rl_split2(rl_lrelu2((f32x2){v[0], v[1]}, slope), h[0], mm[0], l[0]);
+              rl_split2(rl_lrelu2((f32x2){v[2], v[3]}, slope), h[1], mm[1], l[1]);
+              if (tail) {
+                __hip_atomic_store(trow + (col >> 2), ((unsigned long long)h[1] << 32) | h[0], __ATOMIC_RELAXED, __HIP_MEMORY_SCOPE_AGENT);
+                __hip_atomic_store(trow + G::C4 + (col >> 2), ((unsigned long long)mm[1] << 32) | mm[0], __ATOMIC_RELAXED, __HIP_MEMORY_SCOPE_AGENT);
+                __hip_atomic_store(trow + 2 * G::C4 + (col >> 2), ((unsigned long long)l[1] << 32) | l[0], __ATOMIC_RELAXED, __HIP_MEMORY_SCOPE_AGENT);
+              }
+              u16* dst = xt + (m + k - 1) * LDB + col;
+              *reinterpret_cast<uint2*>(dst) = make_uint2(h[0], h[1]);
+              *reinterpret_cast<uint2*>(dst + G::PLX) = make_uint2(mm[0], mm[1]);
+              *reinterpret_cast<uint2*>(dst + 2 * G::PLX) = make_uint2(l[0], l[1]);
+            }
+          }
+        }
+        asm volatile("s_waitcnt vmcnt(0)" ::: "memory");
+        if (lane == 0) __hip_atomic_store(a.hflag + (long long)tflag * 4 + wave, a.hepoch, __ATOMIC_RELAXED, __HIP_MEMORY_SCOPE_AGENT);
+      };
+      if constexpr (HALO) epilogue1h();
+      else if (zrows > 0) epilogue1(std::true_type{}); else epilogue1(std::false_type{});
+#if RL_STAMPS
+      asm volatile("s_waitcnt lgkmcnt(0)" ::: "memory"); st_e1 += RL_T() - e1_0; ++st_tiles;
+#endif
+    }
+    RL_BAR(st_b1);
+#if RL_STAMPS
+    const unsigned long long mid_ = RL_T();
+#endif
+    pn = __builtin_amdgcn_readfirstlane(meta[2]);
+    const int pnx = pn >= 0 ? pn : p;
+    const long long csn = (long long)(RL_SEL(pnx, k) + 1) * G::KB * G::BLK;
+    const u16* const w1n = RL_SEL(pnx, w1l) + (long long)ct0 * csn + lane * 8;
+    {
+      f32x4 acc[G::NRW2][G::NCW];
+#pragma unroll
+      for (int r = 0; r < G::NRW2; ++r)
+#pragma unroll
+        for (int c = 0; c < G::NCW; ++c) acc[r][c] = (f32x4){0.f, 0.f, 0.f, 0.f};
+      const int rt0 = wr * G::NRW2;
+#if RL_STAMPS
+      st_mid += RL_T() - mid_;
+#endif
+      RL_GEMM(rl_gemm<G::NRW2, G::NCW, LDB, G::KB, G::RING>(xt, G::PLX, rt0 * 16, 1, k, w2 + (long long)ct0 * ct_stride + lane * 8, ct_stride,
+                                                           w1n, csn, acc, bw, lane));
+      RL_BAR(st_b4);
+#if RL_STAMPS
+      const unsigned long long e2_0 = RL_T();
+#endif
+#pragma unroll
+      for (int c = 0; c < G::NCW; ++c) {
+        const int col = (ct0 + c) * 16 + 4 * lg;
+#pragma unroll
+        for (int r = 0; r < G::NRW2; ++r) {
+          if (rt0 + r < NR2) *reinterpret_cast<f32x4*>(accimg + ((rt0 + r) * 16 + lr) * G::LDA + col) = acc[r][c];
+        }
+      }
+#if RL_STAMPS
+      asm volatile("s_waitcnt lgkmcnt(0)" ::: "memory"); st_e2 += RL_T() - e2_0;
+#endif
+    }
+    RL_BAR(st_b2);
+    p = pn;
+  }
+#if RL_STAMPS
+  if (a.dbg && tid == 0) {
+    unsigned long long* o = a.dbg + blockIdx.x * 4;
+    if (blockIdx.x == 0) { unsigned long long* q = a.dbg + 256 * 4; q[0] = st_b3; q[1] = st_b1; q[2] = st_b4; q[3] = st_b2; q[4] = st_e1; q[5] = st_e2; q[6] = st_tiles; q[7] = st_gemm; q[8] = __builtin_amdgcn_s_memtime() - st_t0; q[9] = st_head; q[10] = st_pre; q[11] = st_mid; }
+    o[0] = st_gemm; o[1] = __builtin_amdgcn_s_memtime() - st_t0; o[2] = __builtin_amdgcn_s_memrealtime() - st_r0; o[3] = st_bar;
+  }
+#endif
diff --git a/conan_amd/csrc/streams.h b/conan_amd/csrc/streams.h
--- a/conan_amd/csrc/streams.h
+++ b/conan_amd/csrc/streams.h
@@ -22,6 +22,8 @@
   bool fused = false;
   bool pair = false;
   std::vector<std::vector<Ring>> xh;
+  std::vector<std::vector<unsigned short*>> xtail;
+  int tail_L = 0;
 };
 
 struct PinRing {
@@ -90,6 +92,9 @@
   bool rb_merge = true;
   int* cp_ticket[3] = {nullptr, nullptr, nullptr};
   int* rb_sched[2] = {nullptr, nullptr};
+  unsigned* rb_hflag[2] = {nullptr, nullptr};
+  int rb_hflag_words = 0;
+  unsigned rb_epoch = 0;
   float* rp_xb[2] = {nullptr, nullptr};
   unsigned* rp_words[2] = {nullptr, nullptr};
   long long sk_slab_floats = 0;
@@ -107,8 +112,9 @@
     const unsigned code = *(volatile const unsigned*)h_guard;
     if (code == 0) return;
     static const char* what[] = {"?", "decoder_mega_kernel group / grid barrier", "emformer_fused_kernel cluster exchange", "resblock_pair_kernel partner flag", "resblock_pair_kernel tile mailbox",
-                                 "(retired)", "decoder_mega_kernel xcd election", "decoder_mega_kernel xcd roll call", "decoder_mega_kernel xcd flag barrier"};
-    throw ch::Error(CONAN_ERR_HIP, std::string("a cross-workgroup wait gave up after its 50 ms budget (") + what[code < 9 ? code : 0] +
+                                 "(retired)", "decoder_mega_kernel xcd election", "decoder_mega_kernel xcd roll call", "decoder_mega_kernel xcd flag barrier",
+                                 "resblock_limb halo hand-over flag"};
+    throw ch::Error(CONAN_ERR_HIP, std::string("a cross-workgroup wait gave up after its 50 ms budget (") + what[code < 10 ? code : 0] +
                                        "): results since then are invalid and this stream-set is unusable - destroy it and create a new one");
   }
 
@@ -254,7 +260,7 @@
   struct ProfKernel { std::string name; double ms, flops; long long n; };
   std::vector<ProfKernel> prof_kernels;
   void launch_group(const ConvGroup& g, int nprob, int cfg, hipStream_t st);
-  bool launch_rb(const cnk::RBArgs& a, int C, hipStream_t st, const TRef* ymean = nullptr);
+  bool launch_rb(const cnk::RBArgs& a, int C, hipStream_t st, const TRef* ymean = nullptr, unsigned short* const* tails = nullptr, int tail_L = 0);
   void launch_rp(const cnk::RPArgs& a, hipStream_t st);
   bool use_rowconv = true;
   bool rowconv_ok(const PackedConv& pc, int dil, int T) const { return use_rowconv && pc.wf && cnk::rowconv_supported(pc.Cin, pc.k, dil, T); }
diff --git a/conan_amd/csrc/streams.hip b/conan_amd/csrc/streams.hip
--- a/conan_amd/csrc/streams.hip
+++ b/conan_amd/csrc/streams.hip
@@ -168,7 +168,7 @@
   profiled(cnk::rowconv_kernel_name(a, prows), fl, st, [&] { cnk::launch_rowconv(a, st, prows); });
 }
 
-bool conan_streams::launch_rb(const cnk::RBArgs& ain, int C, hipStream_t st, const TRef* ymean) {
+bool conan_streams::launch_rb(const cnk::RBArgs& ain, int C, hipStream_t st, const TRef* ymean, unsigned short* const* tails, int tail_L) {
   cnk::RBArgs a = ain;
   a.sched = rb_sched[ws_index(st) == 1 ? 1 : 0];
   int ksum = 0, kmax = 0;
@@ -185,6 +185,14 @@
   const bool balanced = groups * 10 >= rounds * cus * 9;
   a.merge = (ymean && rb_merge && a.nprob > 1 && groups >= cus && balanced && (limb ? cnk::resblock_limb_can_merge(C, rows) : cnk::resblock_fused_can_merge(C, rows))) ? 1 : 0;
   if (a.merge) a.ymean = *ymean;
+  if (limb && tails && a.p[0].x.mode == 0 && cnk::resblock_limb_has_halo(C, rows, kmax) && a.T + 16 <= tail_L &&
+      (long long)a.nprob * a.n * ((a.T + rows - 1) / rows) * 4 <= rb_hflag_words) {
+    a.halo = 1;
+    for (int p = 0; p < a.nprob; ++p) a.xtail[p] = tails[p];
+    a.xtail_stride = (long long)tail_L * (3 * C / 4); a.xtail_lmask = tail_L - 1;
+    if (++rb_epoch == 0u) rb_epoch = 1u;
+    a.hepoch = rb_epoch; a.hflag = rb_hflag[ws_index(st) == 1 ? 1 : 0]; a.hflag_words = rb_hflag_words; a.guard = d_guard;
+  }
   profiled(limb ? cnk::resblock_limb_name(C, rows, a.merge != 0) : cnk::resblock_fused_name(C, rows, a.merge != 0), fl, st, [&] {
     if (!(limb ? cnk::launch_resblock_limb(a, C, rows, cus, st) : cnk::launch_resblock_fused(a, C, rows, cus, st))) throw Error(CONAN_ERR_HIP, "fused resblock launch failed");
   });
@@ -268,7 +276,7 @@
 void conan_streams::parse_dev_plan(const char* text) {
   static const char* known[] = {"RESERVE_CUS", "ROWCONV", "RB_NOMERGE", "RB_NOLIMB", "FENCED", "DEC_MEGA", "MEGA_GRID", "FRONT_CUSTRIDE", "EMF_CUSTRIDE", "MEGA_GS",
                                 "MEGA_NARROW", "MEGA_NOL2", "MEGA_LAYOUT", "FRONT_PRIO", "RB_UNFUSED", "RB_FUSED", "RB_PAIR", "RB_NOPAIR", "RP_MIN_SLOTS",
-                                "UPS_CFG", "EMF_CLUSTER", "EMF_UNFUSED", "NO_TALL", "TALL_MAXT"};
+                                "UPS_CFG", "EMF_CLUSTER", "EMF_UNFUSED", "NO_TALL", "TALL_MAXT", "RB_HALO"};
   dev_plan.clear();
   if (!text) return;
   const std::string t(text);
@@ -286,6 +294,16 @@
     bool ok = false;
     for (const char* k : known) ok = ok || name == k;
     if (!ok) throw Error(CONAN_ERR_INVALID, "conan_streams_opts.dev_plan: unknown switch '" + name + "'");
+    if (name == "RB_HALO") {
+      size_t a = 0;
+      while (a <= value.size()) {
+        size_t b = value.find(',', a);
+        if (b == std::string::npos) b = value.size();
+        const std::string w = value.substr(a, b - a);
+        if (w != "0" && w != "64" && w != "128") throw Error(CONAN_ERR_INVALID, "conan_streams_opts.dev_plan: RB_HALO takes a list of 128, 64 or 0, got '" + value + "'");
+        a = b + 1;
+      }
+    }
     dev_plan[name] = value;
   }
 }
@@ -395,6 +413,28 @@
         s.xo[b].push_back(mk_ring(ch_, rate, h, &voc_state));
         if (!s.fused && d + 1 < c.voc_rb_num_dil) s.xa[b].push_back(mk_ring(ch_, rate, h, &voc_state));
       }
+    {
+      int kmax_ = 0;
+      for (int b = 0; b < c.voc_num_resblocks; ++b) kmax_ = std::max(kmax_, c.voc_rb_kernels[b]);
+      bool want = ch_ == 128;
+      if (const char* e = dev("RB_HALO")) { const std::string t = std::string(",") + e + ","; want = t.find("," + std::to_string(ch_) + ",") != std::string::npos; }
+      int span_ = 0;
+      for (int b = 0; b < c.voc_num_resblocks; ++b) for (int d = 0; d < c.voc_rb_num_dil; ++d) span_ = std::max(span_, (c.voc_rb_kernels[b] - 1) * c.voc_rb_dilations[b][d]);
+      const int rows_ = cnk::resblock_limb_rows(ch_, span_);
+      if (want && rb_limb && s.fused && !s.pair && rows_ > 0 && cnk::resblock_limb_has_halo(ch_, rows_, kmax_)) {
+        s.tail_L = ch::next_pow2(max_frames * rate + 16);
+        const size_t per_slot = (size_t)s.tail_L * (3 * ch_ / 2);
+        s.xtail.resize(c.voc_num_resblocks);
+        for (int b = 0; b < c.voc_num_resblocks; ++b)
+          for (int d = 0; d < c.voc_rb_num_dil; ++d) {
+            float* t = alloc((size_t)max_slots * per_slot);
+            voc_state.push_back({t, (long long)per_slot});
+            s.xtail[b].push_back(reinterpret_cast<unsigned short*>(t));
+          }
+        const int words = c.voc_num_resblocks * max_slots * ((max_frames * rate + rows_ - 1) / rows_) * 4;
+        rb_hflag_words = std::max(rb_hflag_words, words);
+      }
+    }
     if (s.pair) {
       s.xh.resize(c.voc_num_resblocks);
       for (int b = 0; b < c.voc_num_resblocks; ++b)
@@ -406,6 +446,7 @@
       }
     }
   }
+  for (int w = 0; w < 2 && rb_hflag_words > 0; ++w) rb_hflag[w] = reinterpret_cast<unsigned*>(alloc((size_t)rb_hflag_words));
 }
 
 void conan_streams::out_stage_init() {
@@ -562,8 +603,11 @@
         pr.k = c.voc_rb_kernels[b]; pr.dil = c.voc_rb_dilations[b][d];
       }
       ra.slots = d_slots; ra.pos = pos; ra.nprob = NB; ra.n = n; ra.T = T; ra.slope = LR;
-      if (d + 1 < ND) launch_rb(ra, s.C, st);
-      else { const TRef ym = s.xs.ref(); merged = launch_rb(ra, s.C, st, &ym); }
+      unsigned short* tails[kMaxBranches] = {nullptr, nullptr, nullptr};
+      if (!s.xtail.empty()) for (int b = 0; b < NB; ++b) tails[b] = s.xtail[b][d];
+      unsigned short* const* tl = s.xtail.empty() ? nullptr : tails;
+      if (d + 1 < ND) launch_rb(ra, s.C, st, nullptr, tl, s.tail_L);
+      else { const TRef ym = s.xs.ref(); merged = launch_rb(ra, s.C, st, &ym, tl, s.tail_L); }
     }
     for (int d = 0; d < ND && c.voc_resblock == 2; ++d) {
       ConvGroup g1;
```

Measured after the change: 48520 (median of 6 runs). No clear change (+0.6%).
